# xuanvinh1997/llm-fp8

Measured on AMD Instinct MI355X. Metric: train tokens/sec + FP8 GEMM % of MFMA peak, Llama-3.2-3B seq512 b16, higher is better.
Workload: dtype fp8 (E4M3/E5M2 operands, fp32 accumulate, bf16 activations); 1 GPU; llama-3.2-3b (28 layers) full fine-tuning step, batch 16/GPU x seq 512, fp8_scenario=default (te_llama counterpart, lm_head FP8 under the outer recipe), random-init weights, synthetic tokens; route=fused, global_batch=16, seq_len=512, parallelism=single

## Files before the change

include/mi_fp8.h:

```cpp
#ifndef MI_FP8_H
#define MI_FP8_H

#include <stdint.h>

#ifdef __cplusplus
extern "C" {
#endif

#define MI_FMT_E4M3 0
#define MI_FMT_E5M2 1

#define MI_OK 0
#define MI_ERR_ARG (-1)
#define MI_ERR_SHAPE (-2)
#define MI_ERR_HIP (-3)

#define MI_OUT_BF16 0
#define MI_OUT_F32 1

#define MI_AMAX_ALGO_MAX 0
#define MI_AMAX_ALGO_MOST_RECENT 1

#define MI_ABI_VERSION 5
int mi_abi_version(void);
const char* mi_last_error(void);
int mi_device_supported(void);

int mi_cast_amax(const void* x_bf16, void* y_fp8, void* yT_fp8, const float* scale, float* amax,
                 int64_t rows, int64_t cols, int64_t ld_y, int64_t ld_yT, int fmt, void* stream);
int mi_transpose_u8(const void* y, void* yT, int64_t rows, int64_t cols, int64_t ld_y, int64_t ld_yT, void* stream);
int mi_cast_amax_colsum(const void* x_bf16, void* y_fp8, void* yT_fp8, const float* scale, float* amax,
                        float* colsum_partial, int64_t rows, int64_t cols, int64_t ld_y, int64_t ld_yT, int fmt, void* stream);
int mi_colsum_finish(const float* partial, int64_t P, int64_t C, void* out, int out_dtype, void* stream);
int mi_colsum_finish_multi(const void* const* partials, const int64_t* P, const int64_t* C, void* const* outs,
                           const int* out_dtypes, int n, void* stream);

int mi_scale_update(float* amax_history, float* scale, float* scale_inv, const float* fp8_max,
                    int H, int S, int64_t ld, int margin, int algo, void* stream);

int mi_gemm_fp8(const void* A, const void* B, void* D, const float* sa_inv, const float* sb_inv,
                const void* bias_bf16, int64_t M, int64_t N, int64_t K, int64_t lda, int64_t ldb,
                int64_t ldd, int fmt_a, int fmt_b, int out_dtype, int algo, void* stream);

int mi_gemm_fp8_clock(const void* A, const void* B, void* D, const float* sa_inv, const float* sb_inv, int64_t M, int64_t N,
                      int64_t K, int64_t lda, int64_t ldb, int64_t ldd, int algo, unsigned long long* stamps, void* stream);

typedef struct mi_gemm_problem {
  const void* A;
  const void* B;
  void* D;
  const float* sa_inv;
  const float* sb_inv;
  int64_t M, N, K, lda, ldb, ldd;
} mi_gemm_problem;
int mi_gemm_fp8_grouped(const mi_gemm_problem* problems, int n, int fmt_a, int fmt_b, int tile_cfg, void* stream);

int64_t mi_gemm_workspace_bytes(void);
int mi_gemm_set_workspace(void* workspace, int64_t bytes);

int mi_mxfp8_quantize(const void* x_bf16, void* y_row, void* s_row, void* y_colT, void* s_colT,
                      int64_t rows, int64_t cols, int fmt, void* stream);

int mi_mxfp8_quantize_ex(const void* x_bf16, void* y_row, void* s_row, void* y_colT, void* s_colT, float* colsum,
                         int64_t rows, int64_t cols, int64_t ld_rows, int fmt, void* stream);
int mi_mxfp8_norm_quantize(const void* x_bf16, const float* rstd, const void* gamma_bf16, void* y_row, void* s_row,
                           void* y_colT, void* s_colT, int64_t rows, int64_t cols, int fmt, void* stream);
int mi_mxfp8_swiglu_quantize(const void* h_bf16, void* y_row, void* s_row, void* y_colT, void* s_colT, int64_t rows,
                             int64_t F, int fmt, void* stream);
int mi_mxfp8_dswiglu_quantize(const void* h_bf16, const void* dact_bf16, void* y_row, void* s_row, void* y_colT,
                              void* s_colT, float* colsum, int64_t rows, int64_t F, int fmt, void* stream);
int mi_mxfp8_rope_bwd_quantize(const void* dq_bf16, const void* dk_bf16, const void* dv_bf16, const float* cos_tab,
                               const float* sin_tab, void* y_row, void* s_row, void* y_colT, void* s_colT, int64_t rows,
                               int64_t seq, int n_q_heads, int n_kv_heads, int head_dim, int fmt, void* stream);

int mi_gemm_mxfp8(const void* A, const void* SA, const void* B, const void* SB, void* D,
                  const void* bias_bf16, int64_t M, int64_t N, int64_t K, int fmt_a, int fmt_b,
                  int out_dtype, int algo, void* stream);

typedef struct mi_gemm_mx_problem {
  const void* A;
  const void* SA;
  const void* B;
  const void* SB;
  void* D;
  int64_t M, N, K;
} mi_gemm_mx_problem;
int mi_gemm_mxfp8_grouped(const mi_gemm_mx_problem* problems, int n, int fmt_a, int fmt_b, int tile_cfg, void* stream);

int mi_rope_qkv(void* fused_bf16, void* q_bf16, void* k_bf16, void* v_bf16, const float* cos_tab,
                const float* sin_tab, int64_t rows, int64_t seq, int n_q_heads, int n_kv_heads, int head_dim,
                int backward, void* stream);
int mi_rope_qkv_bwd_cast(const void* dq_bf16, const void* dk_bf16, const void* dv_bf16, const float* cos_tab, const float* sin_tab,
                         void* y_fp8, void* yT_fp8, const float* scale, float* amax, int64_t rows, int64_t seq, int n_q_heads,
                         int n_kv_heads, int head_dim, int fmt, void* stream);

int mi_swiglu_cast(const void* h_bf16, void* y_fp8, void* yT_fp8, const float* scale, float* amax,
                   int64_t rows, int64_t F, int fmt, void* stream);

int mi_dswiglu_cast(const void* h_bf16, const void* dact_bf16, void* y_fp8, void* yT_fp8, const float* scale,
                    float* amax, float* colsum, int64_t rows, int64_t F, int fmt, void* stream);
int mi_swiglu_cast_bias(const void* h_bf16, const void* bias_bf16, void* y_fp8, void* yT_fp8, const float* scale, float* amax,
                        int64_t rows, int64_t F, int fmt, void* stream);
int mi_dswiglu_cast_bias(const void* h_bf16, const void* bias_bf16, const void* dact_bf16, void* y_fp8, void* yT_fp8,
                         const float* scale, float* amax, float* colsum, int64_t rows, int64_t F, int fmt, void* stream);

int mi_rmsnorm_stats(const void* x_bf16, float* rstd, int64_t rows, int64_t cols, float eps, void* stream);
int mi_add_rmsnorm_stats(const void* a_bf16, const void* b_bf16, void* out_bf16, float* rstd, int64_t rows, int64_t cols,
                         float eps, void* stream);
int mi_add_bias_rmsnorm_stats(const void* a_bf16, const void* b_bf16, const void* bias_bf16, void* out_bf16, float* rstd,
                              int64_t rows, int64_t cols, float eps, void* stream);
int mi_norm_cast(const void* x_bf16, const float* rstd, const void* gamma_bf16, void* y_fp8, void* yT_fp8,
                 const float* scale, float* amax, int64_t rows, int64_t cols, int fmt, void* stream);
int mi_rmsnorm_bwd(const void* dy_bf16, const void* x_bf16, const float* rstd, const void* gamma_bf16,
                   const void* dres_bf16, void* dx_bf16, float* dgamma_partial, int n_partials, int64_t rows,
                   int64_t cols, void* stream);

int mi_ce_forward(const void* logits_bf16, const int64_t* labels, float* lse, float* loss_rows, int64_t rows,
                  int64_t cols, void* stream);
int mi_ce_backward(const void* logits_bf16, const int64_t* labels, const float* lse, const float* gscale,
                   void* dlogits_bf16, int64_t rows, int64_t cols, void* stream);
int mi_ce_backward_cast(const void* logits_bf16, const int64_t* labels, const float* lse, const float* gscale, void* y_fp8,
                        void* yT_fp8, const float* scale, float* amax, int64_t rows, int64_t cols, int fmt, void* stream);

int mi_sumsq_bf16(const void* g_bf16, int64_t n, float* partial, int n_partials, void* stream);
int mi_sumsq_bf16_multi(const int64_t* table, int n_tensors, const int32_t* chunks, int n_chunks, int chunk_elems,
                        double* partial, void* stream);
int mi_adamw_bf16_multi(const int64_t* table, int n_tensors, const int32_t* chunks, int n_chunks, int chunk_elems,
                        const float* grad_scale, float lr, float beta1, float beta2, float eps, float weight_decay,
                        int64_t step, void* stream);
int mi_adamw_cast_bf16_multi(const int64_t* table, int n_tensors, const int32_t* chunks, int n_chunks, int chunk_elems,
                             const float* grad_scale, float lr, float beta1, float beta2, float eps, float weight_decay,
                             int64_t step, void* stream);
int mi_adamw_mxcast_bf16_multi(const int64_t* table, int n_tensors, const int32_t* chunks, int n_chunks, int chunk_elems,
                               const float* grad_scale, float lr, float beta1, float beta2, float eps, float weight_decay,
                               int64_t step, void* stream);

int mi_embedding_grad_add(void* grad_bf16, const void* dy_bf16, const int64_t* sorted_ids, const int64_t* perm, int64_t tokens,
                          int64_t hidden, int64_t vocab, float alpha, int64_t padding_idx, void* stream);
int mi_adamw_bf16(void* p_bf16, const void* g_bf16, void* exp_avg_bf16, void* exp_avg_sq_bf16, int64_t n,
                  const float* grad_scale, float lr, float beta1, float beta2, float eps, float weight_decay,
                  int64_t step, void* stream);

int mi_attn_fwd(const void* q, const void* k, const void* v, void* o, float* lse, int B, int S, int H, int G, int D,
                int64_t q_ts, int64_t k_ts, int64_t v_ts, int64_t o_ts, float scale, int causal, void* stream);
#ifdef MI_DIAG
int mi_attn_fwd_diag(const void* q, const void* k, const void* v, void* o, float* lse, unsigned long long* dbg, int B, int S,
                     int H, int G, int D, int64_t q_ts, int64_t k_ts, int64_t v_ts, int64_t o_ts, float scale, void* stream);
#endif
int mi_attn_bwd(const void* q, const void* k, const void* v, const void* o, const void* dout, const float* lse,
                float* delta, void* dq, void* dk, void* dv, int B, int S, int H, int G, int D, int64_t q_ts,
                int64_t k_ts, int64_t v_ts, int64_t o_ts, int64_t do_ts, int64_t dq_ts, int64_t dk_ts, int64_t dv_ts,
                float scale, int causal, void* stream);

#ifdef __cplusplus
}
#endif
#endif
```

llm_fp8_amd/_lib.py:

```python
from __future__ import annotations

import ctypes
import os

_HERE = os.path.dirname(os.path.abspath(__file__))
LIB_PATH = os.environ.get("LLM_FP8_AMD_LIB") or os.path.join(_HERE, "libmi_fp8.so")
LAB_LIB_PATH = os.path.join(os.path.dirname(_HERE), "tools", "bin", "libmi_fp8_lab.so")

MI_FMT_E4M3 = 0
MI_FMT_E5M2 = 1
ABI_VERSION = 5

_c_i64 = ctypes.c_int64
_c_int = ctypes.c_int
_p = ctypes.c_void_p

class GemmProblem(ctypes.Structure):
    _fields_ = [("A", ctypes.c_void_p), ("B", ctypes.c_void_p), ("D", ctypes.c_void_p), ("sa_inv", ctypes.c_void_p),
                ("sb_inv", ctypes.c_void_p), ("M", ctypes.c_int64), ("N", ctypes.c_int64), ("K", ctypes.c_int64),
                ("lda", ctypes.c_int64), ("ldb", ctypes.c_int64), ("ldd", ctypes.c_int64)]


class GemmMxProblem(ctypes.Structure):
    _fields_ = [("A", ctypes.c_void_p), ("SA", ctypes.c_void_p), ("B", ctypes.c_void_p), ("SB", ctypes.c_void_p),
                ("D", ctypes.c_void_p), ("M", ctypes.c_int64), ("N", ctypes.c_int64), ("K", ctypes.c_int64)]

SIGNATURES = {
    "mi_abi_version": [],
    "mi_last_error": [],
    "mi_device_supported": [],
    "mi_cast_amax": [_p, _p, _p, _p, _p, _c_i64, _c_i64, _c_i64, _c_i64, _c_int, _p],
    "mi_transpose_u8": [_p, _p, _c_i64, _c_i64, _c_i64, _c_i64, _p],
    "mi_scale_update": [_p, _p, _p, _p, _c_int, _c_int, _c_i64, _c_int, _c_int, _p],
    "mi_gemm_fp8_grouped": [_p, _c_int, _c_int, _c_int, _c_int, _p],
    "mi_gemm_mxfp8_grouped": [_p, _c_int, _c_int, _c_int, _c_int, _p],
    "mi_gemm_fp8": [_p, _p, _p, _p, _p, _p, _c_i64, _c_i64, _c_i64, _c_i64, _c_i64, _c_i64,
                    _c_int, _c_int, _c_int, _c_int, _p],
    "mi_mxfp8_quantize": [_p, _p, _p, _p, _p, _c_i64, _c_i64, _c_int, _p],
    "mi_mxfp8_quantize_ex": [_p, _p, _p, _p, _p, _p, _c_i64, _c_i64, _c_i64, _c_int, _p],
    "mi_mxfp8_rope_bwd_quantize": [_p, _p, _p, _p, _p, _p, _p, _p, _p, _c_i64, _c_i64, _c_int, _c_int, _c_int, _c_int, _p],
    "mi_rope_qkv": [_p, _p, _p, _p, _p, _p, _c_i64, _c_i64, _c_int, _c_int, _c_int, _c_int, _p],
    "mi_rope_qkv_bwd_cast": [_p, _p, _p, _p, _p, _p, _p, _p, _p, _c_i64, _c_i64, _c_int, _c_int, _c_int, _c_int, _p],
    "mi_swiglu_cast": [_p, _p, _p, _p, _p, _c_i64, _c_i64, _c_int, _p],
    "mi_dswiglu_cast": [_p, _p, _p, _p, _p, _p, _p, _c_i64, _c_i64, _c_int, _p],
    "mi_rmsnorm_stats": [_p, _p, _c_i64, _c_i64, ctypes.c_float, _p],
    "mi_norm_cast": [_p, _p, _p, _p, _p, _p, _p, _c_i64, _c_i64, _c_int, _p],
    "mi_rmsnorm_bwd": [_p, _p, _p, _p, _p, _p, _p, _c_int, _c_i64, _c_i64, _p],
    "mi_ce_forward": [_p, _p, _p, _p, _c_i64, _c_i64, _p],
    "mi_ce_backward": [_p, _p, _p, _p, _p, _c_i64, _c_i64, _p],
    "mi_ce_backward_cast": [_p, _p, _p, _p, _p, _p, _p, _p, _c_i64, _c_i64, _c_int, _p],
    "mi_sumsq_bf16": [_p, _c_i64, _p, _c_int, _p],
    "mi_sumsq_bf16_multi": [_p, _c_int, _p, _c_int, _c_int, _p, _p],
    "mi_adamw_bf16_multi": [_p, _c_int, _p, _c_int, _c_int, _p, ctypes.c_float, ctypes.c_float, ctypes.c_float, ctypes.c_float,
                            ctypes.c_float, _c_i64, _p],
    "mi_adamw_cast_bf16_multi": [_p, _c_int, _p, _c_int, _c_int, _p, ctypes.c_float, ctypes.c_float, ctypes.c_float, ctypes.c_float,
                                 ctypes.c_float, _c_i64, _p],
    "mi_adamw_mxcast_bf16_multi": [_p, _c_int, _p, _c_int, _c_int, _p, ctypes.c_float, ctypes.c_float, ctypes.c_float, ctypes.c_float,
                                   ctypes.c_float, _c_i64, _p],
    "mi_embedding_grad_add": [_p, _p, _p, _p, _c_i64, _c_i64, _c_i64, ctypes.c_float, _c_i64, _p],
    "mi_adamw_bf16": [_p, _p, _p, _p, _c_i64, _p, ctypes.c_float, ctypes.c_float, ctypes.c_float, ctypes.c_float,
                      ctypes.c_float, _c_i64, _p],
    "mi_add_rmsnorm_stats": [_p, _p, _p, _p, _c_i64, _c_i64, ctypes.c_float, _p],
    "mi_cast_amax_colsum": [_p, _p, _p, _p, _p, _p, _c_i64, _c_i64, _c_i64, _c_i64, _c_int, _p],
    "mi_colsum_finish": [_p, _c_i64, _c_i64, _p, _c_int, _p],
    "mi_colsum_finish_multi": [_p, _p, _p, _p, _p, _c_int, _p],
    "mi_gemm_workspace_bytes": [],
    "mi_gemm_set_workspace": [_p, _c_i64],
    "mi_attn_fwd": [_p, _p, _p, _p, _p, _c_int, _c_int, _c_int, _c_int, _c_int, _c_i64, _c_i64, _c_i64, _c_i64, ctypes.c_float,
                    _c_int, _p],
    "mi_attn_bwd": [_p] * 10 + [_c_int] * 5 + [_c_i64] * 8 + [ctypes.c_float, _c_int, _p],
    "mi_mxfp8_norm_quantize": [_p, _p, _p, _p, _p, _p, _p, _c_i64, _c_i64, _c_int, _p],
    "mi_mxfp8_swiglu_quantize": [_p, _p, _p, _p, _p, _c_i64, _c_i64, _c_int, _p],
    "mi_mxfp8_dswiglu_quantize": [_p, _p, _p, _p, _p, _p, _p, _c_i64, _c_i64, _c_int, _p],
    "mi_gemm_mxfp8": [_p, _p, _p, _p, _p, _p, _c_i64, _c_i64, _c_i64, _c_int, _c_int, _c_int, _c_int, _p],
    "mi_swiglu_cast_bias": [_p, _p, _p, _p, _p, _p, _c_i64, _c_i64, _c_int, _p],
    "mi_dswiglu_cast_bias": [_p, _p, _p, _p, _p, _p, _p, _p, _c_i64, _c_i64, _c_int, _p],
    "mi_add_bias_rmsnorm_stats": [_p, _p, _p, _p, _p, _c_i64, _c_i64, ctypes.c_float, _p],
    "mi_gemm_fp8_clock": [_p, _p, _p, _p, _p, _c_i64, _c_i64, _c_i64, _c_i64, _c_i64, _c_i64, _c_int, _p, _p],
}
LAB_SIGNATURES = {
    "mi_attn_fwd_diag": [_p, _p, _p, _p, _p, _p, _c_int, _c_int, _c_int, _c_int, _c_int, _c_i64, _c_i64, _c_i64, _c_i64, ctypes.c_float, _p],
}

_lib = None


def _bind(path: str, signatures) -> ctypes.CDLL:
    lib = ctypes.CDLL(path)
    for name, argtypes in signatures.items():
        fn = getattr(lib, name)
        fn.argtypes = argtypes
        fn.restype = ctypes.c_char_p if name == "mi_last_error" else (_c_i64 if name == "mi_gemm_workspace_bytes" else _c_int)
    v = lib.mi_abi_version()
    if v != ABI_VERSION:
        raise ImportError(f"{os.path.basename(path)} ABI version {v} != expected {ABI_VERSION}; rebuild it")
    return lib


def load() -> ctypes.CDLL:
    global _lib
    if _lib is not None:
        return _lib
    if not os.path.exists(LIB_PATH):
        raise ImportError(
            f"{LIB_PATH} not found: the HIP extension is not built. Run "
            "`python -c 'import __graft_entry__ as g; g.build()'` or `make -C llm_fp8_amd/csrc`. "
            "llm_fp8_amd has no CPU/PyTorch fallback for the FP8 path.")
    _lib = _bind(LIB_PATH, SIGNATURES)
    return _lib


def use_lab_library() -> ctypes.CDLL:
    global _lib
    if _lib is not None and getattr(_lib, "_mi_is_lab", False):
        return _lib
    if _lib is not None:
        raise RuntimeError("use_lab_library(): the product library is already loaded in this process")
    if not os.path.exists(LAB_LIB_PATH):
        raise ImportError(f"{LAB_LIB_PATH} not found: run `make -C llm_fp8_amd/csrc lab`")
    _lib = _bind(LAB_LIB_PATH, {**SIGNATURES, **LAB_SIGNATURES})
    _lib._mi_is_lab = True
    return _lib


def check(rc: int, what: str = "") -> None:
    if rc != 0:
        msg = load().mi_last_error().decode("utf-8", "replace")
        raise RuntimeError(f"libmi_fp8 {what} failed (rc={rc}): {msg}")
```

llm_fp8_amd/csrc/mi_attn.hip:

```cpp
#include "mi_common.h"

namespace mi {

typedef __bf16 bf8 __attribute__((ext_vector_type(8)));
typedef short s4v __attribute__((ext_vector_type(4)));
typedef short s8v __attribute__((ext_vector_type(8)));
typedef float f16v __attribute__((ext_vector_type(16)));
typedef __attribute__((address_space(3))) s4v lds_s4v;

template <int D>
__device__ __forceinline__ int tile_off(int row, int ch) {
  if (D == 128) return 256 * row + 16 * (ch ^ (((row & 3) << 2) | ((row >> 2) & 3)));
  return 128 * row + 16 * (ch ^ (((row & 1) << 2) | ((row >> 1) & 3)));
}

__device__ __forceinline__ bf8 as_bf8(v4i v) { return __builtin_bit_cast(bf8, v); }

template <int D>
__device__ __forceinline__ bf8 row_frag(const char* tile, int r0, int t, int lane) {
  const int r = lane & 31, h = lane >> 5;
  return as_bf8(*reinterpret_cast<const v4i*>(tile + tile_off<D>(r0 + r, 2 * t + h)));
}

template <int D>
__device__ __forceinline__ bf8 tr_frag(const char* tile, int r0, int c0, int lane) {
  const int i16 = lane & 15, qq = i16 >> 2, pp = i16 & 3, half = (lane >> 4) & 1, h = lane >> 5;
  const int ch = (c0 >> 3) + 2 * half + (pp >> 1);
  const int rb = r0 + 4 * h + qq;
  const s4v lo = __builtin_amdgcn_ds_read_tr16_b64_v4i16((lds_s4v*)(tile + tile_off<D>(rb, ch) + 8 * (pp & 1)));
  const s4v hi = __builtin_amdgcn_ds_read_tr16_b64_v4i16((lds_s4v*)(tile + tile_off<D>(rb + 8, ch) + 8 * (pp & 1)));
  s8v v;
  v[0] = lo[0]; v[1] = lo[1]; v[2] = lo[2]; v[3] = lo[3]; v[4] = hi[0]; v[5] = hi[1]; v[6] = hi[2]; v[7] = hi[3];
  return __builtin_bit_cast(bf8, v);
}

__device__ __forceinline__ bf8 acc_frag(const f16v& a, int s) {
  v4i v;
#pragma unroll
  for (int j = 0; j < 4; ++j) v[j] = (int)pack_bf16x2(a[8 * s + 2 * j], a[8 * s + 2 * j + 1]);
  return as_bf8(v);
}

__device__ __forceinline__ int acc_row(int reg, int h) { return (reg & 3) + 8 * (reg >> 2) + 4 * h; }

__device__ __forceinline__ void retire(bf8& f) {
  v4i tmp = __builtin_bit_cast(v4i, f);
  asm volatile("" : "+v"(tmp));
  f = as_bf8(tmp);
}
__device__ __forceinline__ void retire(float& f) { asm volatile("" : "+v"(f)); }

constexpr int ATT_QB = 128;
constexpr int ATT_KB = 64;

typedef __amdgpu_buffer_rsrc_t rsrc_t;
#define MI_LDS_PTR(p) ((__attribute__((address_space(3))) void*)(p))
template <int D>
__device__ __forceinline__ void dma_voffsets(int* voff, int64_t tok_stride, int tid) {
  const int lane = tid & 63, w = tid >> 6;
#pragma unroll
  for (int i = 0; i < D / 32; ++i) {
    const int p = (4 * i + w) * 1024 + 16 * lane;
    const int row = p / (2 * D), slot = (p % (2 * D)) / 16;
    const int ch = D == 128 ? slot ^ (((row & 3) << 2) | ((row >> 2) & 3)) : slot ^ (((row & 1) << 2) | ((row >> 1) & 3));
    voff[i] = (int)((int64_t)row * tok_stride * 2) + 16 * ch;
  }
}
template <int D>
__device__ __forceinline__ void stage_dma(rsrc_t rs, const int* voff, int soff, char* tile, int w) {
#pragma unroll
  for (int i = 0; i < D / 32; ++i)
    __builtin_amdgcn_raw_ptr_buffer_load_lds(rs, MI_LDS_PTR(tile + (4 * i + w) * 1024), 16, voff[i], soff, 0, 0);
}
template <int D>
__device__ __forceinline__ void stage_dma_checked(rsrc_t rs, const int* voff, int adv, char* tile, int w) {
#pragma unroll
  for (int i = 0; i < D / 32; ++i)
    __builtin_amdgcn_raw_ptr_buffer_load_lds(rs, MI_LDS_PTR(tile + (4 * i + w) * 1024), 16, (int)((u32)voff[i] + (u32)adv), 0, 0, 0);
}
template <int D, bool TAIL>
__device__ __forceinline__ void stage_tile(rsrc_t rs, const int* voff, int adv, char* tile, int w) {
  if (TAIL) stage_dma_checked<D>(rs, voff, adv, tile, w);
  else stage_dma<D>(rs, voff, adv, tile, w);
}
__device__ __forceinline__ void dma_wait_all() { asm volatile("s_waitcnt vmcnt(0)" ::: "memory"); }

template <int D, bool CAUSAL, bool DIAG = false, bool TAIL = false>
__global__ __launch_bounds__(256, 2) void attn_fwd_kernel(const uint16_t* __restrict__ q, const uint16_t* __restrict__ k,
                                                          const uint16_t* __restrict__ v, uint16_t* __restrict__ o,
                                                          float* __restrict__ lse, int S, int H, int G, int64_t q_ts,
                                                          int64_t k_ts, int64_t v_ts, int64_t o_ts, float c,
                                                          unsigned long long* __restrict__ dbg = nullptr) {
  constexpr int TILE = ATT_KB * D * 2;
  constexpr int KT = D / 16, DB = D / 32;
  __shared__ __attribute__((aligned(16))) char lds[4 * TILE];
  const int tid = threadIdx.x, lane = tid & 63, w = tid >> 6, r = lane & 31, h = lane >> 5;
  const int qb = gridDim.x - 1 - blockIdx.x, head = blockIdx.y, b = blockIdx.z, g = head / (H / G);
  const int q_first = qb * ATT_QB + w * 32;
  const int qrow = q_first + r;
  int ntiles = CAUSAL ? (qb * ATT_QB + ATT_QB) / ATT_KB : S / ATT_KB;
  if (TAIL) {
    const int stiles = (S + ATT_KB - 1) / ATT_KB;
    ntiles = CAUSAL ? min(ntiles, stiles) : stiles;
  }
  const uint16_t* kbase = k + (int64_t)b * S * k_ts + (int64_t)g * D;
  const uint16_t* vbase = v + (int64_t)b * S * v_ts + (int64_t)g * D;

  bf8 qf[KT];
  {
    const uint16_t* qp = q + ((int64_t)b * S + (TAIL ? min(qrow, S - 1) : qrow)) * q_ts + (int64_t)head * D + 8 * h;
#pragma unroll
    for (int t = 0; t < KT; ++t) qf[t] = as_bf8(*reinterpret_cast<const v4i*>(qp + 16 * t));
  }
#pragma unroll
  for (int t = 0; t < KT; ++t) retire(qf[t]);
  f16v oacc[DB];
#pragma unroll
  for (int d = 0; d < DB; ++d)
#pragma unroll
    for (int i = 0; i < 16; ++i) oacc[d][i] = 0.0f;
  float m = -1.0e30f, l = 0.0f;

  const rsrc_t rsK = __builtin_amdgcn_make_buffer_rsrc((void*)kbase, 0, (int)((((int64_t)S - 1) * k_ts + D) * 2), 0x00020000);
  const rsrc_t rsV = __builtin_amdgcn_make_buffer_rsrc((void*)vbase, 0, (int)((((int64_t)S - 1) * v_ts + D) * 2), 0x00020000);
  int kvo[D / 32], vvo[D / 32];
  dma_voffsets<D>(kvo, k_ts, tid);
  dma_voffsets<D>(vvo, v_ts, tid);
  stage_tile<D, TAIL>(rsK, kvo, 0, lds, w);
  stage_tile<D, TAIL>(rsV, vvo, 0, lds + 2 * TILE, w);
  dma_wait_all();
  __syncthreads();

  unsigned long long tsum[5] = {0, 0, 0, 0, 0}, t_prev = 0;
#define MI_STAMP(k)                                                                       \
  if (DIAG) {                                                                             \
    __builtin_amdgcn_sched_barrier(0);                                                    \
    unsigned long long tn_;                                                               \
    asm volatile("s_memtime %0\n\ts_waitcnt lgkmcnt(0)" : "=s"(tn_)::"memory");          \
    if ((k) >= 0) tsum[(k) < 0 ? 0 : (k)] += tn_ - t_prev;                                  \
    t_prev = tn_;                                                                         \
    __builtin_amdgcn_sched_barrier(0);                                                    \
  }
  MI_STAMP(-1)
  for (int j = 0; j < ntiles; ++j) {
    const char* kt = lds + (j & 1) * TILE;
    const char* vt = lds + (2 + (j & 1)) * TILE;
    const bool more = j + 1 < ntiles;
    if (more) {
      stage_tile<D, TAIL>(rsK, kvo, (int)((int64_t)(j + 1) * ATT_KB * k_ts * 2), lds + ((j + 1) & 1) * TILE, w);
      stage_tile<D, TAIL>(rsV, vvo, (int)((int64_t)(j + 1) * ATT_KB * v_ts * 2), lds + (2 + ((j + 1) & 1)) * TILE, w);
    }
    const int key0 = j * ATT_KB;
    if ((!TAIL || q_first < S) && (!CAUSAL || key0 <= q_first + 31)) {
      f16v sacc[2];
#pragma unroll
      for (int kb = 0; kb < 2; ++kb) {
#pragma unroll
        for (int i = 0; i < 16; ++i) sacc[kb][i] = 0.0f;
        bf8 ka = row_frag<D>(kt, 32 * kb, 0, lane);
#pragma unroll
        for (int t = 0; t < KT; ++t) {
          bf8 kn = ka;
          if (t + 1 < KT) kn = row_frag<D>(kt, 32 * kb, t + 1, lane);
          __builtin_amdgcn_sched_barrier(0);
          sacc[kb] = __builtin_amdgcn_mfma_f32_32x32x16_bf16(ka, qf[t], sacc[kb], 0, 0, 0);
          __builtin_amdgcn_sched_barrier(0);
          ka = kn;
        }
      }
      if (DIAG) {
        asm volatile("" : "+v"(sacc[0][0]), "+v"(sacc[1][15]));
      }
      MI_STAMP(0)
      if (CAUSAL && key0 + ATT_KB - 1 > q_first) {
#pragma unroll
        for (int kb = 0; kb < 2; ++kb)
#pragma unroll
          for (int i = 0; i < 16; ++i)
            if (key0 + 32 * kb + acc_row(i, h) > qrow) sacc[kb][i] = -INFINITY;
      }
      if (TAIL && !CAUSAL && key0 + ATT_KB > S) {
#pragma unroll
        for (int kb = 0; kb < 2; ++kb)
#pragma unroll
          for (int i = 0; i < 16; ++i)
            if (key0 + 32 * kb + acc_row(i, h) >= S) sacc[kb][i] = -INFINITY;
      }
      float mx = sacc[0][0];
#pragma unroll
      for (int kb = 0; kb < 2; ++kb)
#pragma unroll
        for (int i = 0; i < 16; ++i) mx = fmaxf(mx, sacc[kb][i]);
      mx = fmaxf(mx, __shfl_xor(mx, 32));
      const float m_new = fmaxf(m, mx);
      const float alpha = __builtin_amdgcn_exp2f((m - m_new) * c);
      const float mc = m_new * c;
      m = m_new;
      float psum = 0.0f;
#pragma unroll
      for (int kb = 0; kb < 2; ++kb)
#pragma unroll
        for (int i = 0; i < 16; ++i) {
          const float p = __builtin_amdgcn_exp2f(__builtin_fmaf(sacc[kb][i], c, -mc));
          sacc[kb][i] = p;
          psum += p;
        }
      l = l * alpha + psum;
#pragma unroll
      for (int d = 0; d < DB; ++d) oacc[d] = oacc[d] * alpha;
      if (DIAG) {
        asm volatile("" : "+v"(oacc[0][0]), "+v"(sacc[1][15]), "+v"(l));
      }
      MI_STAMP(1)
#pragma unroll
      for (int kb = 0; kb < 2; ++kb)
#pragma unroll
        for (int s = 0; s < 2; ++s) {
          const bf8 pf = acc_frag(sacc[kb], s);
          bf8 fa = tr_frag<D>(vt, 32 * kb + 16 * s, 0, lane);
#pragma unroll
          for (int d = 0; d < DB; ++d) {
            bf8 fn = fa;
            if (d + 1 < DB) fn = tr_frag<D>(vt, 32 * kb + 16 * s, 32 * (d + 1), lane);
            __builtin_amdgcn_sched_barrier(0);
            oacc[d] = __builtin_amdgcn_mfma_f32_32x32x16_bf16(fa, pf, oacc[d], 0, 0, 0);
            __builtin_amdgcn_sched_barrier(0);
            fa = fn;
          }
        }
    }
    if (DIAG) {
      asm volatile("" : "+v"(oacc[0][0]), "+v"(oacc[DB - 1][15]));
    }
    MI_STAMP(2)
    dma_wait_all();
    MI_STAMP(3)
    __syncthreads();
    MI_STAMP(4)
  }
  if (DIAG && dbg != nullptr && lane == 0) {
    unsigned long long* dp = dbg + ((((int64_t)b * H + head) * gridDim.x + qb) * 4 + w) * 8;
    for (int i2 = 0; i2 < 5; ++i2) dp[i2] = tsum[i2];
    dp[5] = (unsigned long long)ntiles;
  }
#undef MI_STAMP

  l += __shfl_xor(l, 32);
  const float inv = 1.0f / l;
  if (h == 0 && (!TAIL || qrow < S)) lse[((int64_t)b * H + head) * S + qrow] = m * c + __builtin_amdgcn_logf(l);
  char* ot = lds + w * (32 * D * 2);
#pragma unroll
  for (int d = 0; d < DB; ++d)
#pragma unroll
    for (int i = 0; i < 4; ++i) {
      const int ch = 4 * d + i;
      uint2 pk;
      pk.x = pack_bf16x2(oacc[d][4 * i] * inv, oacc[d][4 * i + 1] * inv);
      pk.y = pack_bf16x2(oacc[d][4 * i + 2] * inv, oacc[d][4 * i + 3] * inv);
      *reinterpret_cast<uint2*>(ot + r * (D * 2) + 16 * (ch ^ (r & (D / 8 - 1))) + 8 * h) = pk;
    }
  __builtin_amdgcn_s_waitcnt(0xc07f);
  __builtin_amdgcn_wave_barrier();
  constexpr int CPR = D / 8;
#pragma unroll
  for (int it = 0; it < 32 * CPR / 64; ++it) {
    const int idx = it * 64 + lane, row = idx / CPR, ch = idx % CPR;
    const v4i val = *reinterpret_cast<const v4i*>(ot + row * (D * 2) + 16 * (ch ^ (row & (CPR - 1))));
    if (!TAIL || q_first + row < S) *reinterpret_cast<v4i*>(o + ((int64_t)b * S + q_first + row) * o_ts + (int64_t)head * D + ch * 8) = val;
  }
}


template <int D, bool TAIL = false>
__device__ __forceinline__ void store_rows_from_accT(const f16v (&acc)[D / 32], float mul, char* slice, uint16_t* out,
                                                     int64_t row_stride, int lane, int nrows = 32) {
  const int r = lane & 31, h = lane >> 5;
  constexpr int CPR = D / 8;
#pragma unroll
  for (int d = 0; d < D / 32; ++d)
#pragma unroll
    for (int i = 0; i < 4; ++i) {
      const int ch = 4 * d + i;
      uint2 pk;
      pk.x = pack_bf16x2(acc[d][4 * i] * mul, acc[d][4 * i + 1] * mul);
      pk.y = pack_bf16x2(acc[d][4 * i + 2] * mul, acc[d][4 * i + 3] * mul);
      *reinterpret_cast<uint2*>(slice + r * (D * 2) + 16 * (ch ^ (r & (CPR - 1))) + 8 * h) = pk;
    }
  __builtin_amdgcn_s_waitcnt(0xc07f);
  __builtin_amdgcn_wave_barrier();
#pragma unroll
  for (int it = 0; it < 32 * CPR / 64; ++it) {
    const int idx = it * 64 + lane, row = idx / CPR, ch = idx % CPR;
    const v4i val = *reinterpret_cast<const v4i*>(slice + row * (D * 2) + 16 * (ch ^ (row & (CPR - 1))));
    if (!TAIL || row < nrows) *reinterpret_cast<v4i*>(out + (int64_t)row * row_stride + ch * 8) = val;
  }
}

template <int D, bool CAUSAL, bool TAIL = false>
__global__ __launch_bounds__(256, 2) void attn_bwd_dq_kernel(const uint16_t* __restrict__ q, const uint16_t* __restrict__ k,
                                                             const uint16_t* __restrict__ v, const uint16_t* __restrict__ o,
                                                             const uint16_t* __restrict__ dout, const float* __restrict__ lse,
                                                             float* __restrict__ delta, uint16_t* __restrict__ dq, int S,
                                                             int H, int G, int64_t q_ts, int64_t k_ts, int64_t v_ts,
                                                             int64_t o_ts, int64_t do_ts, int64_t dq_ts, float c, float scale) {
  constexpr int TILE = ATT_KB * D * 2;
  constexpr int KT = D / 16, DB = D / 32;
  __shared__ __attribute__((aligned(16))) char lds[4 * TILE];
  const int tid = threadIdx.x, lane = tid & 63, w = tid >> 6, r = lane & 31, h = lane >> 5;
  const int qb = gridDim.x - 1 - blockIdx.x, head = blockIdx.y, b = blockIdx.z, g = head / (H / G);
  const int q_first = qb * ATT_QB + w * 32;
  const int qrow = q_first + r;
  int ntiles = CAUSAL ? (qb * ATT_QB + ATT_QB) / ATT_KB : S / ATT_KB;
  if (TAIL) {
    const int stiles = (S + ATT_KB - 1) / ATT_KB;
    ntiles = CAUSAL ? min(ntiles, stiles) : stiles;
  }
  const uint16_t* kbase = k + (int64_t)b * S * k_ts + (int64_t)g * D;
  const uint16_t* vbase = v + (int64_t)b * S * v_ts + (int64_t)g * D;

  bf8 qf[KT], dof[KT];
  float dl = 0.0f;
  {
    const int lrow = TAIL ? min(qrow, S - 1) : qrow;
    const uint16_t* qp = q + ((int64_t)b * S + lrow) * q_ts + (int64_t)head * D + 8 * h;
    const uint16_t* dp = dout + ((int64_t)b * S + lrow) * do_ts + (int64_t)head * D + 8 * h;
    const uint16_t* op = o + ((int64_t)b * S + lrow) * o_ts + (int64_t)head * D + 8 * h;
#pragma unroll
    for (int t = 0; t < KT; ++t) {
      qf[t] = as_bf8(*reinterpret_cast<const v4i*>(qp + 16 * t));
      const v4i dv4 = *reinterpret_cast<const v4i*>(dp + 16 * t);
      const v4i ov4 = *reinterpret_cast<const v4i*>(op + 16 * t);
      dof[t] = as_bf8(dv4);
#pragma unroll
      for (int j = 0; j < 4; ++j) {
        const u32 a = (u32)dv4[j], bb = (u32)ov4[j];
        dl += __uint_as_float(a << 16) * __uint_as_float(bb << 16) + __uint_as_float(a & 0xFFFF0000u) * __uint_as_float(bb & 0xFFFF0000u);
      }
    }
  }
  dl += __shfl_xor(dl, 32);
  const int64_t stat = ((int64_t)b * H + head) * S + qrow;
  if (h == 0 && (!TAIL || qrow < S)) delta[stat] = dl;
  float my_lse = lse[TAIL ? ((int64_t)b * H + head) * S + min(qrow, S - 1) : stat];
#pragma unroll
  for (int t = 0; t < KT; ++t) {
    retire(qf[t]);
    retire(dof[t]);
  }
  retire(my_lse);
  retire(dl);

  f16v acc[DB];
#pragma unroll
  for (int d = 0; d < DB; ++d)
#pragma unroll
    for (int i = 0; i < 16; ++i) acc[d][i] = 0.0f;

  const rsrc_t rsK = __builtin_amdgcn_make_buffer_rsrc((void*)kbase, 0, (int)((((int64_t)S - 1) * k_ts + D) * 2), 0x00020000);
  const rsrc_t rsV = __builtin_amdgcn_make_buffer_rsrc((void*)vbase, 0, (int)((((int64_t)S - 1) * v_ts + D) * 2), 0x00020000);
  int kvo[D / 32], vvo[D / 32];
  dma_voffsets<D>(kvo, k_ts, tid);
  dma_voffsets<D>(vvo, v_ts, tid);
  stage_tile<D, TAIL>(rsK, kvo, 0, lds, w);
  stage_tile<D, TAIL>(rsV, vvo, 0, lds + 2 * TILE, w);
  dma_wait_all();
  __syncthreads();

  for (int j = 0; j < ntiles; ++j) {
    const char* kt = lds + (j & 1) * TILE;
    const char* vt = lds + (2 + (j & 1)) * TILE;
    const bool more = j + 1 < ntiles;
    if (more) {
      stage_tile<D, TAIL>(rsK, kvo, (int)((int64_t)(j + 1) * ATT_KB * k_ts * 2), lds + ((j + 1) & 1) * TILE, w);
      stage_tile<D, TAIL>(rsV, vvo, (int)((int64_t)(j + 1) * ATT_KB * v_ts * 2), lds + (2 + ((j + 1) & 1)) * TILE, w);
    }
    const int key0 = j * ATT_KB;
    auto block = [&](const int kb) {
      f16v sacc, pacc;
#pragma unroll
      for (int i = 0; i < 16; ++i) { sacc[i] = 0.0f; pacc[i] = 0.0f; }
      constexpr int PF = 1;
      bf8 kr[KT], vr[KT];
#pragma unroll
      for (int t = 0; t < PF; ++t) {
        kr[t] = row_frag<D>(kt, 32 * kb, t, lane);
        vr[t] = row_frag<D>(vt, 32 * kb, t, lane);
      }
#pragma unroll
      for (int t = 0; t < KT; ++t) {
        if (t + PF < KT) {
          kr[t + PF] = row_frag<D>(kt, 32 * kb, t + PF, lane);
          vr[t + PF] = row_frag<D>(vt, 32 * kb, t + PF, lane);
        }
        __builtin_amdgcn_sched_barrier(0);
        sacc = __builtin_amdgcn_mfma_f32_32x32x16_bf16(kr[t], qf[t], sacc, 0, 0, 0);
        pacc = __builtin_amdgcn_mfma_f32_32x32x16_bf16(vr[t], dof[t], pacc, 0, 0, 0);
        __builtin_amdgcn_sched_barrier(0);
      }
      const bool diag = CAUSAL && key0 + 32 * kb + 31 > q_first;
#pragma unroll
      for (int i = 0; i < 16; ++i) {
        float p = __builtin_amdgcn_exp2f(__builtin_fmaf(sacc[i], c, -my_lse));
        if (diag && key0 + 32 * kb + acc_row(i, h) > qrow) p = 0.0f;
        if (TAIL && !CAUSAL && key0 + 32 * kb + acc_row(i, h) >= S) p = 0.0f;
        sacc[i] = p * (pacc[i] - dl);
      }
#pragma unroll
      for (int s = 0; s < 2; ++s) {
        const bf8 dsf = acc_frag(sacc, s);
        bf8 fa = tr_frag<D>(kt, 32 * kb + 16 * s, 0, lane);
#pragma unroll
        for (int d = 0; d < DB; ++d) {
          bf8 fn = fa;
          if (d + 1 < DB) fn = tr_frag<D>(kt, 32 * kb + 16 * s, 32 * (d + 1), lane);
          __builtin_amdgcn_sched_barrier(0);
          acc[d] = __builtin_amdgcn_mfma_f32_32x32x16_bf16(fa, dsf, acc[d], 0, 0, 0);
          __builtin_amdgcn_sched_barrier(0);
          fa = fn;
        }
      }
    };
    if ((!TAIL || q_first < S) && (!CAUSAL || key0 <= q_first + 31)) block(0);
    if ((!TAIL || (q_first < S && key0 + 32 < S)) && (!CAUSAL || key0 + 32 <= q_first + 31)) block(1);
    dma_wait_all();
    __syncthreads();
  }
  store_rows_from_accT<D, TAIL>(acc, scale, lds + w * (32 * D * 2), dq + ((int64_t)b * S + q_first) * dq_ts + (int64_t)head * D, dq_ts, lane,
                                S - q_first);
}

template <int D, bool CAUSAL, bool TAIL = false>
__global__ __launch_bounds__(256, D == 128 ? 1 : 2) void attn_bwd_dkdv_kernel(const uint16_t* __restrict__ q, const uint16_t* __restrict__ k,
                                                               const uint16_t* __restrict__ v, const uint16_t* __restrict__ dout,
                                                               const float* __restrict__ lse, const float* __restrict__ delta,
                                                               uint16_t* __restrict__ dk, uint16_t* __restrict__ dv, int S, int H,
                                                               int G, int B, int64_t q_ts, int64_t k_ts, int64_t v_ts,
                                                               int64_t do_ts, int64_t dk_ts, int64_t dv_ts, float c, float scale) {
  constexpr int SL = 32 * D * 2;
  constexpr int KT = D / 16, DB = D / 32;
  constexpr int BUF = 2 * SL + 256;
  __shared__ __attribute__((aligned(16))) char lds[(2 * BUF > 4 * SL) ? 2 * BUF : 4 * SL];
  const int tid = threadIdx.x, lane = tid & 63, w = tid >> 6, r = lane & 31, h = lane >> 5;
  const int lin = blockIdx.x, nkb = TAIL ? (S + 127) / 128 : S / 128;
  const int kbi = CAUSAL ? lin / (G * B) : nkb - 1 - lin / (G * B);
  const int g = (lin / B) % G, b = lin % B;
  const int rep = H / G;
  const int key_first = kbi * 128 + w * 32;
  const int key = key_first + r;

  bf8 kf[KT], vf[KT];
  {
    const int lkey = TAIL ? min(key, S - 1) : key;
    const uint16_t* kp = k + ((int64_t)b * S + lkey) * k_ts + (int64_t)g * D + 8 * h;
    const uint16_t* vp = v + ((int64_t)b * S + lkey) * v_ts + (int64_t)g * D + 8 * h;
#pragma unroll
    for (int t = 0; t < KT; ++t) {
      kf[t] = as_bf8(*reinterpret_cast<const v4i*>(kp + 16 * t));
      vf[t] = as_bf8(*reinterpret_cast<const v4i*>(vp + 16 * t));
    }
  }
#pragma unroll
  for (int t = 0; t < KT; ++t) {
    retire(kf[t]);
    retire(vf[t]);
  }
  f16v dka[DB], dva[DB];
#pragma unroll
  for (int d = 0; d < DB; ++d)
#pragma unroll
    for (int i = 0; i < 16; ++i) { dka[d][i] = 0.0f; dva[d][i] = 0.0f; }

  const int sl0 = CAUSAL ? (kbi * 128) / 32 : 0;
  const int nsl = (TAIL ? (S + 31) / 32 : S / 32) - sl0;
  const int nsteps = rep * nsl;
  v4i qreg[2], dreg[2];
  float sreg = 0.0f;
  auto load_step = [&](int step) {
    const int head = g * rep + step / nsl, q0 = (sl0 + step % nsl) * 32;
    const uint16_t* qp = q + ((int64_t)b * S + q0) * q_ts + (int64_t)head * D;
    const uint16_t* dp = dout + ((int64_t)b * S + q0) * do_ts + (int64_t)head * D;
#pragma unroll
    for (int i = 0; i < 2; ++i) {
      const int cidx = tid + 256 * i, row = cidx / (D / 8), ch = cidx % (D / 8);
      if (D == 128 || cidx < 32 * (D / 8)) {
        if (TAIL && q0 + row >= S) {
          qreg[i] = v4i{0, 0, 0, 0};
          dreg[i] = v4i{0, 0, 0, 0};
        } else {
          qreg[i] = *reinterpret_cast<const v4i*>(qp + (int64_t)row * q_ts + ch * 8);
          dreg[i] = *reinterpret_cast<const v4i*>(dp + (int64_t)row * do_ts + ch * 8);
        }
      }
    }
    if (tid < 64) {
      if (TAIL && q0 + (tid & 31) >= S) sreg = 0.0f;
      else sreg = (tid < 32 ? lse : delta)[((int64_t)b * H + head) * S + q0 + (tid & 31)];
    }
  };
  auto store_step = [&](char* buf) {
#pragma unroll
    for (int i = 0; i < 2; ++i) {
      const int cidx = tid + 256 * i, row = cidx / (D / 8), ch = cidx % (D / 8);
      if (D == 128 || cidx < 32 * (D / 8)) {
        *reinterpret_cast<v4i*>(buf + tile_off<D>(row, ch)) = qreg[i];
        *reinterpret_cast<v4i*>(buf + SL + tile_off<D>(row, ch)) = dreg[i];
      }
    }
    if (tid < 64) reinterpret_cast<float*>(buf + 2 * SL)[tid] = sreg;
  };
  load_step(0);
  store_step(lds);
  __syncthreads();

  for (int step = 0; step < nsteps; ++step) {
    const char* buf = lds + (step & 1) * BUF;
    const bool more = step + 1 < nsteps;
    if (more) load_step(step + 1);
    const int q0 = (sl0 + step % nsl) * 32;
    if ((!TAIL || key_first < S) && (!CAUSAL || q0 + 31 >= key_first)) {
      const char* qt = buf;
      const char* dt = buf + SL;
      const float* st = reinterpret_cast<const float*>(buf + 2 * SL);
      f16v sacc, pacc;
#pragma unroll
      for (int i = 0; i < 16; ++i) { sacc[i] = 0.0f; pacc[i] = 0.0f; }
#pragma unroll
      for (int t = 0; t < KT; ++t) {
        sacc = __builtin_amdgcn_mfma_f32_32x32x16_bf16(row_frag<D>(qt, 0, t, lane), kf[t], sacc, 0, 0, 0);
        pacc = __builtin_amdgcn_mfma_f32_32x32x16_bf16(row_frag<D>(dt, 0, t, lane), vf[t], pacc, 0, 0, 0);
      }
      const bool diag = CAUSAL && q0 < key_first + 31;
      f16v dsacc;
#pragma unroll
      for (int a = 0; a < 4; ++a) {
        const v4f ls = *reinterpret_cast<const v4f*>(st + 8 * a + 4 * h);
        const v4f dl = *reinterpret_cast<const v4f*>(st + 32 + 8 * a + 4 * h);
#pragma unroll
        for (int e = 0; e < 4; ++e) {
          const int i = 4 * a + e;
          float p = __builtin_amdgcn_exp2f(__builtin_fmaf(sacc[i], c, -ls[e]));
          if (diag && key > q0 + acc_row(i, h)) p = 0.0f;
          if (TAIL && q0 + acc_row(i, h) >= S) p = 0.0f;
          sacc[i] = p;
          dsacc[i] = p * (pacc[i] - dl[e]);
        }
      }
#pragma unroll
      for (int s = 0; s < 2; ++s) {
        const bf8 pf = acc_frag(sacc, s), dsf = acc_frag(dsacc, s);
#pragma unroll
        for (int d = 0; d < DB; ++d) {
          dva[d] = __builtin_amdgcn_mfma_f32_32x32x16_bf16(tr_frag<D>(dt, 16 * s, 32 * d, lane), pf, dva[d], 0, 0, 0);
          dka[d] = __builtin_amdgcn_mfma_f32_32x32x16_bf16(tr_frag<D>(qt, 16 * s, 32 * d, lane), dsf, dka[d], 0, 0, 0);
        }
      }
    }
    if (D == 128) {
#pragma unroll
      for (int d = 0; d < DB; ++d) asm volatile("" : "+a"(dka[d]), "+a"(dva[d]));
    }
    if (more) store_step(lds + ((step + 1) & 1) * BUF);
    __syncthreads();
  }
  char* slice = lds + w * SL;
  store_rows_from_accT<D, TAIL>(dka, scale, slice, dk + ((int64_t)b * S + key_first) * dk_ts + (int64_t)g * D, dk_ts, lane, S - key_first);
  __builtin_amdgcn_wave_barrier();
  store_rows_from_accT<D, TAIL>(dva, 1.0f, slice, dv + ((int64_t)b * S + key_first) * dv_ts + (int64_t)g * D, dv_ts, lane, S - key_first);
}

}

extern "C" int mi_attn_fwd(const void* q, const void* k, const void* v, void* o, float* lse, int B, int S, int H, int G,
                           int D, int64_t q_ts, int64_t k_ts, int64_t v_ts, int64_t o_ts, float scale, int causal,
                           void* stream) {
  MI_CHECK_ARG(q && k && v && o && lse, "mi_attn_fwd: null pointer");
  MI_CHECK_ARG(B >= 1 && H >= 1 && G >= 1 && H % G == 0, "mi_attn_fwd: bad B/H/G (%d, %d, %d)", B, H, G);
  MI_CHECK_ARG(D == 128 || D == 64, "mi_attn_fwd: head_dim %d not supported (64, 128)", D);
  MI_CHECK_ARG(S >= 128 && S % 16 == 0, "mi_attn_fwd: seq %d must be a multiple of 16 and at least 128", S);
  MI_CHECK_ARG(q_ts % 8 == 0 && k_ts % 8 == 0 && v_ts % 8 == 0 && o_ts % 8 == 0, "mi_attn_fwd: token strides must be multiples of 8");
  MI_CHECK_ARG((int64_t)S * k_ts * 2 < (1LL << 31) && (int64_t)S * v_ts * 2 < (1LL << 31) && ((uintptr_t)k % 16) == 0 && ((uintptr_t)v % 16) == 0,
               "mi_attn_fwd: one batch of K / V must span < 2 GiB and be 16-byte aligned (32-bit buffer offsets of the LDS DMA)");
  MI_CHECK_ARG(((uintptr_t)q % 16) == 0 && ((uintptr_t)o % 16) == 0, "mi_attn_fwd: q and o must be 16-byte aligned (16-byte row accesses)");
  MI_CHECK_ARG(H <= 65535 && B <= 65535, "mi_attn_fwd: grid too large");
  const float c = scale * 1.4426950408889634f;
  const bool tail = S % mi::ATT_QB != 0;
  dim3 grid((S + mi::ATT_QB - 1) / mi::ATT_QB, H, B), block(256);
  hipStream_t st = (hipStream_t)stream;
#define MI_ATTN_FWD_T(DD, CC, TT)                                                                                      \
  hipLaunchKernelGGL((mi::attn_fwd_kernel<DD, CC, false, TT>), grid, block, 0, st, (const uint16_t*)q, (const uint16_t*)k, \
                     (const uint16_t*)v, (uint16_t*)o, lse, S, H, G, q_ts, k_ts, v_ts, o_ts, c, (unsigned long long*)nullptr)
#define MI_ATTN_FWD(DD, CC)                                                                                            \
  do {                                                                                                                 \
    if (tail) MI_ATTN_FWD_T(DD, CC, true); else MI_ATTN_FWD_T(DD, CC, false);                                          \
  } while (0)
  if (D == 128) {
    if (causal) MI_ATTN_FWD(128, true); else MI_ATTN_FWD(128, false);
  } else {
    if (causal) MI_ATTN_FWD(64, true); else MI_ATTN_FWD(64, false);
  }
#undef MI_ATTN_FWD_T
#undef MI_ATTN_FWD
  MI_CHECK_LAUNCH("mi_attn_fwd launch");
  return MI_OK;
}

#ifdef MI_DIAG
extern "C" int mi_attn_fwd_diag(const void* q, const void* k, const void* v, void* o, float* lse, unsigned long long* dbg, int B,
                                int S, int H, int G, int D, int64_t q_ts, int64_t k_ts, int64_t v_ts, int64_t o_ts, float scale,
                                void* stream) {
  MI_CHECK_ARG(q && k && v && o && lse && dbg, "mi_attn_fwd_diag: null pointer");
  MI_CHECK_ARG(D == 128 && S % 128 == 0 && H % G == 0, "mi_attn_fwd_diag: unsupported shape");
  dim3 grid(S / mi::ATT_QB, H, B), block(256);
  hipLaunchKernelGGL((mi::attn_fwd_kernel<128, true, true>), grid, block, 0, (hipStream_t)stream, (const uint16_t*)q,
                     (const uint16_t*)k, (const uint16_t*)v, (uint16_t*)o, lse, S, H, G, q_ts, k_ts, v_ts, o_ts,
                     scale * 1.4426950408889634f, dbg);
  MI_CHECK_LAUNCH("mi_attn_fwd_diag launch");
  return MI_OK;
}
#endif

extern "C" int mi_attn_bwd(const void* q, const void* k, const void* v, const void* o, const void* dout, const float* lse,
                           float* delta, void* dq, void* dk, void* dv, int B, int S, int H, int G, int D, int64_t q_ts,
                           int64_t k_ts, int64_t v_ts, int64_t o_ts, int64_t do_ts, int64_t dq_ts, int64_t dk_ts,
                           int64_t dv_ts, float scale, int causal, void* stream) {
  MI_CHECK_ARG(q && k && v && o && dout && lse && delta && dq && dk && dv, "mi_attn_bwd: null pointer");
  MI_CHECK_ARG(B >= 1 && H >= 1 && G >= 1 && H % G == 0, "mi_attn_bwd: bad B/H/G (%d, %d, %d)", B, H, G);
  MI_CHECK_ARG(D == 128 || D == 64, "mi_attn_bwd: head_dim %d not supported (64, 128)", D);
  MI_CHECK_ARG(S >= 128 && S % 16 == 0, "mi_attn_bwd: seq %d must be a multiple of 16 and at least 128", S);
  MI_CHECK_ARG((q_ts | k_ts | v_ts | o_ts | do_ts | dq_ts | dk_ts | dv_ts) % 8 == 0, "mi_attn_bwd: token strides must be multiples of 8");
  MI_CHECK_ARG((int64_t)S * k_ts * 2 < (1LL << 31) && (int64_t)S * v_ts * 2 < (1LL << 31) && ((uintptr_t)k % 16) == 0 && ((uintptr_t)v % 16) == 0,
               "mi_attn_bwd: one batch of K / V must span < 2 GiB and be 16-byte aligned (32-bit buffer offsets of the LDS DMA)");
  MI_CHECK_ARG((((uintptr_t)q | (uintptr_t)o | (uintptr_t)dout | (uintptr_t)dq | (uintptr_t)dk | (uintptr_t)dv) % 16) == 0,
               "mi_attn_bwd: q, o, dout, dq, dk and dv must be 16-byte aligned (16-byte row accesses)");
  MI_CHECK_ARG(H <= 65535 && B <= 65535, "mi_attn_bwd: grid too large");
  const float c = scale * 1.4426950408889634f;
  hipStream_t st = (hipStream_t)stream;
  const bool tail = S % mi::ATT_QB != 0;
  const int nblk = (S + mi::ATT_QB - 1) / mi::ATT_QB;
  dim3 grid_q(nblk, H, B), grid_kv((unsigned)((int64_t)nblk * G * B)), block(256);
#define MI_ATTN_BWD_T(DD, CC, TT)                                                                                      \
  do {                                                                                                                 \
    hipLaunchKernelGGL((mi::attn_bwd_dq_kernel<DD, CC, TT>), grid_q, block, 0, st, (const uint16_t*)q, (const uint16_t*)k, \
                       (const uint16_t*)v, (const uint16_t*)o, (const uint16_t*)dout, lse, delta, (uint16_t*)dq, S, H,  \
                       G, q_ts, k_ts, v_ts, o_ts, do_ts, dq_ts, c, scale);                                               \
    hipLaunchKernelGGL((mi::attn_bwd_dkdv_kernel<DD, CC, TT>), grid_kv, block, 0, st, (const uint16_t*)q,                \
                       (const uint16_t*)k, (const uint16_t*)v, (const uint16_t*)dout, lse, delta, (uint16_t*)dk,        \
                       (uint16_t*)dv, S, H, G, B, q_ts, k_ts, v_ts, do_ts, dk_ts, dv_ts, c, scale);                      \
  } while (0)
#define MI_ATTN_BWD(DD, CC)                                                                                            \
  do {                                                                                                                 \
    if (tail) MI_ATTN_BWD_T(DD, CC, true); else MI_ATTN_BWD_T(DD, CC, false);                                          \
  } while (0)
  if (D == 128) {
    if (causal) MI_ATTN_BWD(128, true); else MI_ATTN_BWD(128, false);
  } else {
    if (causal) MI_ATTN_BWD(64, true); else MI_ATTN_BWD(64, false);
  }
#undef MI_ATTN_BWD
#undef MI_ATTN_BWD_T
  MI_CHECK_LAUNCH("mi_attn_bwd launch");
  return MI_OK;
}
```

llm_fp8_amd/csrc/mi_fused.hip:

```cpp
#include "mi_common.h"

namespace mi {

template <int DIR>
__global__ __launch_bounds__(256) void rope_qkv_kernel(uint16_t* __restrict__ fused, uint16_t* __restrict__ q,
                                                       uint16_t* __restrict__ k, uint16_t* __restrict__ v,
                                                       const float* __restrict__ cosT, const float* __restrict__ sinT,
                                                       int rows, int seq, int nq, int nk, int D) {
  const int half = D >> 1;
  const int vph = half >> 3;
  const int W = (nq + 2 * nk) * D;
  const int rot_items = (nq + nk) * vph;
  const int cpy_items = (nk * D) >> 3;
  const int per_row = rot_items + cpy_items;
  const int64_t items = (int64_t)rows * per_row;
  const float sgn = DIR == 0 ? 1.0f : -1.0f;
  for (int64_t it = (int64_t)blockIdx.x * blockDim.x + threadIdx.x; it < items; it += (int64_t)gridDim.x * blockDim.x) {
    const int64_t r = it / per_row;
    const int w = (int)(it - r * per_row);
    uint16_t* frow = fused + r * W;
    if (w < rot_items) {
      const int hd = w / vph, vv = w - hd * vph;
      uint16_t* sep = hd < nq ? q + (r * nq + hd) * D : k + (r * nk + (hd - nq)) * D;
      uint16_t* f1 = frow + hd * D + vv * 8;
      uint16_t* s1 = sep + vv * 8;
      const uint16_t* in1 = DIR == 0 ? f1 : s1;
      uint16_t* out1 = DIR == 0 ? s1 : f1;
      const v4i a = *reinterpret_cast<const v4i*>(in1), b = *reinterpret_cast<const v4i*>(in1 + half);
      const int pos = (int)(r % seq);
      const float* cp = cosT + (int64_t)pos * half + vv * 8;
      const float* sp = sinT + (int64_t)pos * half + vv * 8;
      float c[8], sn[8];
      *reinterpret_cast<v4f*>(c) = *reinterpret_cast<const v4f*>(cp);
      *reinterpret_cast<v4f*>(c + 4) = *reinterpret_cast<const v4f*>(cp + 4);
      *reinterpret_cast<v4f*>(sn) = *reinterpret_cast<const v4f*>(sp);
      *reinterpret_cast<v4f*>(sn + 4) = *reinterpret_cast<const v4f*>(sp + 4);
      v4i o1, o2;
#pragma unroll
      for (int j = 0; j < 4; ++j) {
        const u32 wa = (u32)a[j], wb = (u32)b[j];
        const float x1l = __uint_as_float(wa << 16), x1h = __uint_as_float(wa & 0xFFFF0000u);
        const float x2l = __uint_as_float(wb << 16), x2h = __uint_as_float(wb & 0xFFFF0000u);
        const float cl = c[2 * j], ch = c[2 * j + 1], sl = sgn * sn[2 * j], sh = sgn * sn[2 * j + 1];
        o1[j] = (int)pack_bf16x2(x1l * cl - x2l * sl, x1h * ch - x2h * sh);
        o2[j] = (int)pack_bf16x2(x2l * cl + x1l * sl, x2h * ch + x1h * sh);
      }
      *reinterpret_cast<v4i*>(out1) = o1;
      *reinterpret_cast<v4i*>(out1 + half) = o2;
    } else {
      const int cv = w - rot_items;
      uint16_t* fp = frow + (nq + nk) * D + cv * 8;
      uint16_t* sp2 = v + r * (int64_t)(nk * D) + cv * 8;
      if (DIR == 0) *reinterpret_cast<v4i*>(sp2) = *reinterpret_cast<const v4i*>(fp);
      else *reinterpret_cast<v4i*>(fp) = *reinterpret_cast<const v4i*>(sp2);
    }
  }
}

template <int FMT, bool WRITE_Y, bool WRITE_T>
__global__ __launch_bounds__(256) void rope_bwd_cast_kernel(const uint16_t* __restrict__ dq, const uint16_t* __restrict__ dk,
                                                            const uint16_t* __restrict__ dv, const float* __restrict__ cosT,
                                                            const float* __restrict__ sinT, uint8_t* __restrict__ y,
                                                            uint8_t* __restrict__ yT, const float* __restrict__ scale_p,
                                                            float* amax_out, int rows, int seq, int nq, int nk) {
  constexpr int D = 128, half = 64;
  __shared__ float s_amax[4];
  const int tid = threadIdx.x, lane = tid & 63, wave = tid >> 6;
  const int W = (nq + 2 * nk) * D;
  const int units = (nq + nk) + 2 * nk;
  const int64_t u_all = (int64_t)blockIdx.x * 4 + wave;
  const int rb = (int)(u_all / units), u = (int)(u_all % units);
  const int r0 = rb * 64 + (lane >> 3) * 8, lc = (lane & 7) * 8;
  const float scale = *scale_p;
  float amax = 0.0f;
  auto emit = [&](const float (&f)[8][8], int c0) {
    u32 lo[8], hi[8];
#pragma unroll
    for (int i = 0; i < 8; ++i) {
#pragma unroll
      for (int j = 0; j < 8; ++j) amax = fmaxf(amax, (f[i][j] != f[i][j]) ? 0.0f : fabsf(f[i][j]));
      lo[i] = cvt4_fp8<FMT>(f[i][0] * scale, f[i][1] * scale, f[i][2] * scale, f[i][3] * scale);
      hi[i] = cvt4_fp8<FMT>(f[i][4] * scale, f[i][5] * scale, f[i][6] * scale, f[i][7] * scale);
    }
    if (WRITE_Y) {
      uint8_t* dst = y + (int64_t)r0 * W + c0;
#pragma unroll
      for (int i = 0; i < 8; ++i) mi::st8<MI_NT_Y>(dst + (int64_t)i * W, lo[i], hi[i]);
    }
    if (WRITE_T) {
      u32 a[4], b[4], c[4], d[4];
      transpose4x4(lo[0], lo[1], lo[2], lo[3], a[0], a[1], a[2], a[3]);
      transpose4x4(lo[4], lo[5], lo[6], lo[7], b[0], b[1], b[2], b[3]);
      transpose4x4(hi[0], hi[1], hi[2], hi[3], c[0], c[1], c[2], c[3]);
      transpose4x4(hi[4], hi[5], hi[6], hi[7], d[0], d[1], d[2], d[3]);
      uint8_t* dst = yT + (int64_t)c0 * rows + r0;
#pragma unroll
      for (int j = 0; j < 4; ++j) {
        mi::st8<MI_NT_YT>(dst + (int64_t)j * rows, a[j], b[j]);
        mi::st8<MI_NT_YT>(dst + (int64_t)(j + 4) * rows, c[j], d[j]);
      }
    }
  };
  auto bf16_round = [](float v) { return __uint_as_float(float_to_bf16_bits(v) << 16); };
  if (r0 < rows) {
    if (u < nq + nk) {
      const int hd = u;
      const uint16_t* src = hd < nq ? dq + ((int64_t)r0 * nq + hd) * D : dk + ((int64_t)r0 * nk + (hd - nq)) * D;
      const int64_t rstride = (int64_t)(hd < nq ? nq : nk) * D;
      float f1[8][8], f2[8][8];
#pragma unroll
      for (int i = 0; i < 8; ++i) {
        const v4i a = *reinterpret_cast<const v4i*>(src + i * rstride + lc);
        const v4i b = *reinterpret_cast<const v4i*>(src + i * rstride + half + lc);
        const int pos = (r0 + i) % seq;
        float c[8], sn[8];
        *reinterpret_cast<v4f*>(c) = *reinterpret_cast<const v4f*>(cosT + (int64_t)pos * half + lc);
        *reinterpret_cast<v4f*>(c + 4) = *reinterpret_cast<const v4f*>(cosT + (int64_t)pos * half + lc + 4);
        *reinterpret_cast<v4f*>(sn) = *reinterpret_cast<const v4f*>(sinT + (int64_t)pos * half + lc);
        *reinterpret_cast<v4f*>(sn + 4) = *reinterpret_cast<const v4f*>(sinT + (int64_t)pos * half + lc + 4);
#pragma unroll
        for (int j = 0; j < 4; ++j) {
          const u32 wa = (u32)a[j], wb = (u32)b[j];
          const float x1l = __uint_as_float(wa << 16), x1h = __uint_as_float(wa & 0xFFFF0000u);
          const float x2l = __uint_as_float(wb << 16), x2h = __uint_as_float(wb & 0xFFFF0000u);
          const float cl = c[2 * j], ch = c[2 * j + 1], sl = -1.0f * sn[2 * j], sh = -1.0f * sn[2 * j + 1];
          f1[i][2 * j] = bf16_round(x1l * cl - x2l * sl);
          f1[i][2 * j + 1] = bf16_round(x1h * ch - x2h * sh);
          f2[i][2 * j] = bf16_round(x2l * cl + x1l * sl);
          f2[i][2 * j + 1] = bf16_round(x2h * ch + x1h * sh);
        }
      }
      emit(f1, hd * D + lc);
      emit(f2, hd * D + half + lc);
    } else {
      const int tc = u - (nq + nk);
      float f[8][8];
#pragma unroll
      for (int i = 0; i < 8; ++i) {
        const v4i a = *reinterpret_cast<const v4i*>(dv + (int64_t)(r0 + i) * (nk * D) + tc * 64 + lc);
#pragma unroll
        for (int j = 0; j < 4; ++j) {
          f[i][2 * j] = __uint_as_float((u32)a[j] << 16);
          f[i][2 * j + 1] = __uint_as_float((u32)a[j] & 0xFFFF0000u);
        }
      }
      emit(f, (nq + nk) * D + tc * 64 + lc);
    }
  }
  if (amax_out != nullptr) {
    amax = wave_max(amax);
    if (lane == 0) s_amax[wave] = amax;
    __syncthreads();
    if (tid == 0) {
      const float m = fmaxf(fmaxf(s_amax[0], s_amax[1]), fmaxf(s_amax[2], s_amax[3]));
      if (m > 0.0f && m > __builtin_nontemporal_load(amax_out)) atomicMax(reinterpret_cast<unsigned int*>(amax_out), __float_as_uint(m));
    }
  }
}

__device__ __forceinline__ float sigmoidf_(float g) { return 1.0f / (1.0f + __expf(-g)); }

template <int FMT, int MODE, bool WRITE_Y, bool WRITE_T>
__global__ __launch_bounds__(256) void swiglu_cast_kernel(const uint16_t* __restrict__ h, const uint16_t* __restrict__ d,
                                                          uint8_t* __restrict__ y, uint8_t* __restrict__ yT,
                                                          const float* __restrict__ scale_p, float* amax_out,
                                                          float* __restrict__ colsum, int rows, int F, int tiles_c,
                                                          const uint16_t* __restrict__ bias) {
  __shared__ float s_amax[4];
  __shared__ float s_col[MODE == 1 ? 2 : 1][2][128];
  constexpr int NOUT = MODE == 0 ? 1 : 2;
  const int ocols = MODE == 0 ? F : 2 * F;
  const int tid = threadIdx.x, lane = tid & 63, wave = tid >> 6;
  const int tile_r = blockIdx.x / tiles_c, tile_c = blockIdx.x % tiles_c;
  const int r0 = tile_r * 128 + (wave >> 1) * 64 + (lane >> 3) * 8;
  const int cg = tile_c * 128 + (wave & 1) * 64 + (lane & 7) * 8;
  const float scale = *scale_p;
  float amax = 0.0f;
  float csum[NOUT][8];
#pragma unroll
  for (int o = 0; o < NOUT; ++o)
#pragma unroll
    for (int j = 0; j < 8; ++j) csum[o][j] = 0.0f;
  const bool active = (r0 < rows) && (cg < F);
  if (active) {
    u32 lo[NOUT][8], hi[NOUT][8];
    float bg[8] = {0.f, 0.f, 0.f, 0.f, 0.f, 0.f, 0.f, 0.f}, bu[8] = {0.f, 0.f, 0.f, 0.f, 0.f, 0.f, 0.f, 0.f};
    if (bias != nullptr) {
      const v4i vg = *reinterpret_cast<const v4i*>(bias + cg), vu = *reinterpret_cast<const v4i*>(bias + F + cg);
#pragma unroll
      for (int j = 0; j < 4; ++j) {
        bg[2 * j] = __uint_as_float((u32)vg[j] << 16);
        bg[2 * j + 1] = __uint_as_float((u32)vg[j] & 0xFFFF0000u);
        bu[2 * j] = __uint_as_float((u32)vu[j] << 16);
        bu[2 * j + 1] = __uint_as_float((u32)vu[j] & 0xFFFF0000u);
      }
    }
#pragma unroll
    for (int pass = 0; pass < 2; ++pass) {
      v4i gv[4], uv[4], dv[4];
#pragma unroll
      for (int i = 0; i < 4; ++i) {
        const int64_t r = r0 + 4 * pass + i;
        gv[i] = __builtin_nontemporal_load(reinterpret_cast<const v4i*>(h + r * 2 * F + cg));
        uv[i] = __builtin_nontemporal_load(reinterpret_cast<const v4i*>(h + r * 2 * F + F + cg));
        dv[i] = MODE == 1 ? __builtin_nontemporal_load(reinterpret_cast<const v4i*>(d + r * F + cg)) : (v4i){0, 0, 0, 0};
      }
#pragma unroll
      for (int i = 0; i < 4; ++i) {
        float f[NOUT][8];
#pragma unroll
        for (int j = 0; j < 4; ++j) {
          const u32 wg = (u32)gv[i][j], wu = (u32)uv[i][j], wd = (u32)dv[i][j];
          float g2[2] = {__uint_as_float(wg << 16), __uint_as_float(wg & 0xFFFF0000u)};
          float u2[2] = {__uint_as_float(wu << 16), __uint_as_float(wu & 0xFFFF0000u)};
          const float d2[2] = {__uint_as_float(wd << 16), __uint_as_float(wd & 0xFFFF0000u)};
          if (bias != nullptr) {
            g2[0] += bg[2 * j];
            g2[1] += bg[2 * j + 1];
            u2[0] += bu[2 * j];
            u2[1] += bu[2 * j + 1];
          }
#pragma unroll
          for (int e = 0; e < 2; ++e) {
            const float sg = sigmoidf_(g2[e]);
            if (MODE == 0) {
              f[0][2 * j + e] = g2[e] * sg * u2[e];
            } else {
              f[0][2 * j + e] = d2[e] * u2[e] * (sg * (1.0f + g2[e] * (1.0f - sg)));
              f[NOUT - 1][2 * j + e] = d2[e] * (g2[e] * sg);
            }
          }
        }
#pragma unroll
        for (int o = 0; o < NOUT; ++o) {
#pragma unroll
          for (int j = 0; j < 8; ++j) {
            amax = fmaxf(amax, (f[o][j] != f[o][j]) ? 0.0f : fabsf(f[o][j]));
            if (MODE == 1) csum[o][j] += f[o][j];
          }
          lo[o][4 * pass + i] = cvt4_fp8<FMT>(f[o][0] * scale, f[o][1] * scale, f[o][2] * scale, f[o][3] * scale);
          hi[o][4 * pass + i] = cvt4_fp8<FMT>(f[o][4] * scale, f[o][5] * scale, f[o][6] * scale, f[o][7] * scale);
        }
      }
      if (MODE == 1) __builtin_amdgcn_sched_barrier(0);
    }
#pragma unroll
    for (int o = 0; o < NOUT; ++o) {
      const int c0 = cg + o * F;
      if (WRITE_Y) {
        uint8_t* dst = y + (int64_t)r0 * ocols + c0;
#pragma unroll
        for (int i = 0; i < 8; ++i) mi::st8<MI_NT_Y>(dst + (int64_t)i * ocols, lo[o][i], hi[o][i]);
      }
      if (WRITE_T) {
        u32 a[4], b[4], c[4], dd[4];
        transpose4x4(lo[o][0], lo[o][1], lo[o][2], lo[o][3], a[0], a[1], a[2], a[3]);
        transpose4x4(lo[o][4], lo[o][5], lo[o][6], lo[o][7], b[0], b[1], b[2], b[3]);
        transpose4x4(hi[o][0], hi[o][1], hi[o][2], hi[o][3], c[0], c[1], c[2], c[3]);
        transpose4x4(hi[o][4], hi[o][5], hi[o][6], hi[o][7], dd[0], dd[1], dd[2], dd[3]);
        uint8_t* dst = yT + (int64_t)c0 * rows + r0;
#pragma unroll
        for (int j = 0; j < 4; ++j) {
          mi::st8<MI_NT_YT>(dst + (int64_t)j * rows, a[j], b[j]);
          mi::st8<MI_NT_YT>(dst + (int64_t)(j + 4) * rows, c[j], dd[j]);
        }
      }
    }
  }
  if (MODE == 1 && colsum != nullptr) {
#pragma unroll
    for (int o = 0; o < NOUT; ++o)
#pragma unroll
      for (int j = 0; j < 8; ++j) {
        float v = csum[o][j];
        v += __shfl_xor(v, 8);
        v += __shfl_xor(v, 16);
        v += __shfl_xor(v, 32);
        if ((lane >> 3) == 0) s_col[o][wave >> 1][(wave & 1) * 64 + (lane & 7) * 8 + j] = v;
      }
    __syncthreads();
    const int c = tile_c * 128 + (tid & 127), o = tid >> 7;
    if (c < F) colsum[(int64_t)tile_r * ocols + o * F + c] = s_col[MODE == 1 ? o : 0][0][tid & 127] + s_col[MODE == 1 ? o : 0][1][tid & 127];
  }
  if (amax_out != nullptr) {
    amax = wave_max(amax);
    if (lane == 0) s_amax[wave] = amax;
    __syncthreads();
    if (tid == 0) {
      float m = fmaxf(fmaxf(s_amax[0], s_amax[1]), fmaxf(s_amax[2], s_amax[3]));
      if (m > 0.0f && m > __builtin_nontemporal_load(amax_out)) atomicMax(reinterpret_cast<unsigned int*>(amax_out), __float_as_uint(m));
    }
  }
}

template <int FMT, int MODE>
static int launch_swiglu(const void* h, const void* d, void* y, void* yT, const float* scale, float* amax, float* colsum,
                         int64_t rows, int64_t F, hipStream_t st, const void* bias = nullptr) {
  const int64_t ocols = MODE == 0 ? F : 2 * F;
  (void)ocols;
  const int tiles_r = (int)((rows + 127) / 128), tiles_c = (int)((F + 127) / 128);
  dim3 grid((unsigned)(tiles_r * tiles_c)), block(256);
  const uint16_t *hp = (const uint16_t*)h, *dp = (const uint16_t*)d, *bp = (const uint16_t*)bias;
  uint8_t *yp = (uint8_t*)y, *tp = (uint8_t*)yT;
  if (y && yT)
    hipLaunchKernelGGL((swiglu_cast_kernel<FMT, MODE, true, true>), grid, block, 0, st, hp, dp, yp, tp, scale, amax, colsum, (int)rows, (int)F, tiles_c, bp);
  else if (y)
    hipLaunchKernelGGL((swiglu_cast_kernel<FMT, MODE, true, false>), grid, block, 0, st, hp, dp, yp, tp, scale, amax, colsum, (int)rows, (int)F, tiles_c, bp);
  else
    hipLaunchKernelGGL((swiglu_cast_kernel<FMT, MODE, false, true>), grid, block, 0, st, hp, dp, yp, tp, scale, amax, colsum, (int)rows, (int)F, tiles_c, bp);
  MI_CHECK_LAUNCH("mi_swiglu_cast launch");
  return MI_OK;
}

__global__ __launch_bounds__(256) void rmsnorm_stats_kernel(const uint16_t* __restrict__ x, float* __restrict__ rstd, int rows,
                                                            int cols, float eps) {
  const int lane = threadIdx.x & 63;
  const int row = blockIdx.x * 4 + (threadIdx.x >> 6);
  if (row >= rows) return;
  const uint16_t* xr = x + (int64_t)row * cols;
  float acc = 0.0f;
  for (int c = lane * 8; c < cols; c += 512) {
    const v4i v = *reinterpret_cast<const v4i*>(xr + c);
#pragma unroll
    for (int j = 0; j < 4; ++j) {
      const u32 w = (u32)v[j];
      const float a = __uint_as_float(w << 16), b = __uint_as_float(w & 0xFFFF0000u);
      acc += a * a + b * b;
    }
  }
#pragma unroll
  for (int o = 32; o >= 1; o >>= 1) acc += __shfl_xor(acc, o);
  if (lane == 0) rstd[row] = rsqrtf(acc / (float)cols + eps);
}

template <int FMT, bool WRITE_Y, bool WRITE_T>
__global__ __launch_bounds__(256) void norm_cast_kernel(const uint16_t* __restrict__ x, const float* __restrict__ rstd,
                                                        const uint16_t* __restrict__ gamma, uint8_t* __restrict__ y,
                                                        uint8_t* __restrict__ yT, const float* __restrict__ scale_p,
                                                        float* amax_out, int rows, int cols, int tiles_c) {
  __shared__ float s_amax[4];
  const int tid = threadIdx.x, lane = tid & 63, wave = tid >> 6;
  const int ntiles = ((rows + 63) / 64) * tiles_c;
  const int stride = gridDim.x * 4;
  const int lr = (lane >> 3) * 8, lc = (lane & 7) * 8;
  const float scale = *scale_p;
  float amax = 0.0f;
  int t = blockIdx.x * 4 + wave;
  v4i nxt[8], nxt_g;
  v4f nxt_r[2];
  auto load_tile = [&](int tt, v4i (&raw)[8], v4i& gv, v4f (&rs)[2]) {
    const int r0 = (tt / tiles_c) * 64 + lr, c0 = (tt % tiles_c) * 64 + lc;
    if (r0 < rows && c0 < cols) {
      const uint16_t* src = x + (int64_t)r0 * cols + c0;
#pragma unroll
      for (int i = 0; i < 8; ++i) raw[i] = __builtin_nontemporal_load(reinterpret_cast<const v4i*>(src + (int64_t)i * cols));
      gv = *reinterpret_cast<const v4i*>(gamma + c0);
      rs[0] = *reinterpret_cast<const v4f*>(rstd + r0);
      rs[1] = *reinterpret_cast<const v4f*>(rstd + r0 + 4);
    } else {
#pragma unroll
      for (int i = 0; i < 8; ++i) raw[i] = (v4i){0, 0, 0, 0};
      gv = (v4i){0, 0, 0, 0};
      rs[0] = rs[1] = (v4f){0.f, 0.f, 0.f, 0.f};
    }
  };
  if (t < ntiles) load_tile(t, nxt, nxt_g, nxt_r);
  while (t < ntiles) {
    v4i raw[8];
#pragma unroll
    for (int i = 0; i < 8; ++i) raw[i] = nxt[i];
    const v4i gv = nxt_g;
    const v4f rs0 = nxt_r[0], rs1 = nxt_r[1];
    const int tn = t + stride;
    if (tn < ntiles) load_tile(tn, nxt, nxt_g, nxt_r);
    const int r0 = (t / tiles_c) * 64 + lr, c0 = (t % tiles_c) * 64 + lc;
    if ((r0 < rows) && (c0 < cols)) {
      float g[8];
#pragma unroll
      for (int j = 0; j < 4; ++j) {
        g[2 * j] = __uint_as_float((u32)gv[j] << 16);
        g[2 * j + 1] = __uint_as_float((u32)gv[j] & 0xFFFF0000u);
      }
      u32 lo[8], hi[8];
#pragma unroll
      for (int i = 0; i < 8; ++i) {
        const float rs = i < 4 ? rs0[i] : rs1[i - 4];
        float f[8];
#pragma unroll
        for (int j = 0; j < 4; ++j) {
          const u32 w = (u32)raw[i][j];
          f[2 * j] = (__uint_as_float(w << 16) * rs) * g[2 * j];
          f[2 * j + 1] = (__uint_as_float(w & 0xFFFF0000u) * rs) * g[2 * j + 1];
        }
#pragma unroll
        for (int j = 0; j < 8; ++j) amax = fmaxf(amax, (f[j] != f[j]) ? 0.0f : fabsf(f[j]));
        lo[i] = cvt4_fp8<FMT>(f[0] * scale, f[1] * scale, f[2] * scale, f[3] * scale);
        hi[i] = cvt4_fp8<FMT>(f[4] * scale, f[5] * scale, f[6] * scale, f[7] * scale);
      }
      if (WRITE_Y) {
        uint8_t* dst = y + (int64_t)r0 * cols + c0;
#pragma unroll
        for (int i = 0; i < 8; ++i) mi::st8<MI_NT_Y>(dst + (int64_t)i * cols, lo[i], hi[i]);
      }
      if (WRITE_T) {
        u32 a[4], b[4], c[4], d[4];
        transpose4x4(lo[0], lo[1], lo[2], lo[3], a[0], a[1], a[2], a[3]);
        transpose4x4(lo[4], lo[5], lo[6], lo[7], b[0], b[1], b[2], b[3]);
        transpose4x4(hi[0], hi[1], hi[2], hi[3], c[0], c[1], c[2], c[3]);
        transpose4x4(hi[4], hi[5], hi[6], hi[7], d[0], d[1], d[2], d[3]);
        uint8_t* dst = yT + (int64_t)c0 * rows + r0;
#pragma unroll
        for (int j = 0; j < 4; ++j) {
          mi::st8<MI_NT_YT>(dst + (int64_t)j * rows, a[j], b[j]);
          mi::st8<MI_NT_YT>(dst + (int64_t)(j + 4) * rows, c[j], d[j]);
        }
      }
    }
    t = tn;
  }
  if (amax_out != nullptr) {
    amax = wave_max(amax);
    if (lane == 0) s_amax[wave] = amax;
    __syncthreads();
    if (tid == 0) {
      float m = fmaxf(fmaxf(s_amax[0], s_amax[1]), fmaxf(s_amax[2], s_amax[3]));
      if (m > 0.0f && m > __builtin_nontemporal_load(amax_out)) atomicMax(reinterpret_cast<unsigned int*>(amax_out), __float_as_uint(m));
    }
  }
}

constexpr int kNormMaxVec = 16;
template <int NVEC, int WPR>
__global__ __launch_bounds__(256) void rmsnorm_bwd_kernel(const uint16_t* __restrict__ dy, const uint16_t* __restrict__ x,
                                                          const float* __restrict__ rstd, const uint16_t* __restrict__ gamma,
                                                          const uint16_t* __restrict__ dres, uint16_t* __restrict__ dx,
                                                          float* __restrict__ dgp, int rows, int rows_per_block) {
  static_assert(NVEC % WPR == 0 && (WPR == 1 || WPR == 2 || WPR == 4), "row split");
  extern __shared__ float s_dg[];
  __shared__ float s_dot[2][4];
  constexpr int cols = NVEC * 512;
  constexpr int NV = NVEC / WPR, R = 4 / WPR;
  const int lane = threadIdx.x & 63, wave = threadIdx.x >> 6;
  const int slot = wave / WPR, part = wave % WPR;
  const int col0 = part * NV * 512 + lane * 8;
  v4i gq[NV];
  float dgacc[NV][8];
#pragma unroll
  for (int v = 0; v < NV; ++v) {
    gq[v] = *reinterpret_cast<const v4i*>(gamma + col0 + v * 512);
#pragma unroll
    for (int j = 0; j < 8; ++j) dgacc[v][j] = 0.0f;
  }
  const int row_begin = blockIdx.x * rows_per_block;
  const int row_end = min(rows, row_begin + rows_per_block);
  const int iters = (row_end - row_begin + R - 1) / R;
  for (int it = 0; it < iters; ++it) {
    const int row = row_begin + it * R + slot;
    const bool valid = row < row_end;
    const float rs = valid ? rstd[row] : 0.0f;
    v4i dq[NV], xq[NV];
    float dot = 0.0f;
#pragma unroll
    for (int v = 0; v < NV; ++v) {
      dq[v] = (v4i){0, 0, 0, 0};
      xq[v] = (v4i){0, 0, 0, 0};
      if (valid) {
        const int64_t off = (int64_t)row * cols + col0 + v * 512;
        dq[v] = *reinterpret_cast<const v4i*>(dy + off);
        xq[v] = *reinterpret_cast<const v4i*>(x + off);
      }
    }
#pragma unroll
    for (int v = 0; v < NV; ++v)
#pragma unroll
      for (int j = 0; j < 4; ++j) {
        const float d0 = __uint_as_float((u32)dq[v][j] << 16), d1 = __uint_as_float((u32)dq[v][j] & 0xFFFF0000u);
        const float x0 = __uint_as_float((u32)xq[v][j] << 16) * rs, x1 = __uint_as_float((u32)xq[v][j] & 0xFFFF0000u) * rs;
        const float g0 = __uint_as_float((u32)gq[v][j] << 16), g1 = __uint_as_float((u32)gq[v][j] & 0xFFFF0000u);
        dgacc[v][2 * j] += d0 * x0;
        dgacc[v][2 * j + 1] += d1 * x1;
        dot += (d0 * g0) * x0 + (d1 * g1) * x1;
      }
#pragma unroll
    for (int o = 32; o >= 1; o >>= 1) dot += __shfl_xor(dot, o);
    if (WPR > 1) {
      if (lane == 0) s_dot[it & 1][wave] = dot;
      __syncthreads();
      dot = s_dot[it & 1][slot * WPR];
#pragma unroll
      for (int q = 1; q < WPR; ++q) dot += s_dot[it & 1][slot * WPR + q];
    }
    const float c = dot / (float)cols;
    if (valid) {
#pragma unroll
      for (int v = 0; v < NV; ++v) {
        const int64_t off = (int64_t)row * cols + col0 + v * 512;
        v4i rv = {0, 0, 0, 0};
        if (dres) rv = *reinterpret_cast<const v4i*>(dres + off);
        v4i ov;
#pragma unroll
        for (int j = 0; j < 4; ++j) {
          const float d0 = __uint_as_float((u32)dq[v][j] << 16), d1 = __uint_as_float((u32)dq[v][j] & 0xFFFF0000u);
          const float x0 = __uint_as_float((u32)xq[v][j] << 16) * rs, x1 = __uint_as_float((u32)xq[v][j] & 0xFFFF0000u) * rs;
          const float g0 = __uint_as_float((u32)gq[v][j] << 16), g1 = __uint_as_float((u32)gq[v][j] & 0xFFFF0000u);
          float o0 = rs * (d0 * g0 - x0 * c), o1 = rs * (d1 * g1 - x1 * c);
          if (dres) {
            o0 += __uint_as_float((u32)rv[j] << 16);
            o1 += __uint_as_float((u32)rv[j] & 0xFFFF0000u);
          }
          ov[j] = (int)pack_bf16x2(o0, o1);
        }
        *reinterpret_cast<v4i*>(dx + off) = ov;
      }
    }
  }
#pragma unroll
  for (int v = 0; v < NV; ++v)
#pragma unroll
    for (int j = 0; j < 8; ++j) s_dg[slot * cols + col0 + v * 512 + j] = dgacc[v][j];
  __syncthreads();
  for (int c = threadIdx.x; c < cols; c += 256) {
    float a = s_dg[c];
#pragma unroll
    for (int q = 1; q < R; ++q) a += s_dg[q * cols + c];
    dgp[(int64_t)blockIdx.x * cols + c] = a;
  }
}

__global__ __launch_bounds__(256) void ce_fwd_kernel(const uint16_t* __restrict__ x, const int64_t* __restrict__ labels,
                                                     float* __restrict__ lse, float* __restrict__ loss, int cols) {
  __shared__ float s_m[4], s_s[4];
  const int row = blockIdx.x, tid = threadIdx.x;
  const uint16_t* xr = x + (int64_t)row * cols;
  float m = -INFINITY, ssum = 0.0f;
  for (int c = tid * 8; c < cols; c += 2048) {
    const v4i v = *reinterpret_cast<const v4i*>(xr + c);
    float f[8];
#pragma unroll
    for (int j = 0; j < 4; ++j) {
      f[2 * j] = __uint_as_float((u32)v[j] << 16);
      f[2 * j + 1] = __uint_as_float((u32)v[j] & 0xFFFF0000u);
    }
    float vm = f[0];
#pragma unroll
    for (int j = 1; j < 8; ++j) vm = fmaxf(vm, f[j]);
    const float nm = fmaxf(m, vm);
    float add = 0.0f;
#pragma unroll
    for (int j = 0; j < 8; ++j) add += __expf(f[j] - nm);
    ssum = (nm == -INFINITY) ? 0.0f : ssum * __expf(m - nm) + add;
    m = nm;
  }
#pragma unroll
  for (int o = 32; o >= 1; o >>= 1) {
    const float om = __shfl_xor(m, o), os = __shfl_xor(ssum, o);
    const float nm = fmaxf(m, om);
    ssum = (nm == -INFINITY) ? 0.0f : ssum * __expf(m - nm) + os * __expf(om - nm);
    m = nm;
  }
  if ((tid & 63) == 0) { s_m[tid >> 6] = m; s_s[tid >> 6] = ssum; }
  __syncthreads();
  if (tid == 0) {
    float M = s_m[0], S = s_s[0];
#pragma unroll
    for (int w = 1; w < 4; ++w) {
      const float nm = fmaxf(M, s_m[w]);
      S = (nm == -INFINITY) ? 0.0f : S * __expf(M - nm) + s_s[w] * __expf(s_m[w] - nm);
      M = nm;
    }
    const float l = M + __logf(S);
    lse[row] = l;
    const int64_t lab = labels[row];
    loss[row] = (lab >= 0 && lab < cols) ? l - bf16_bits_to_float(xr[lab]) : 0.0f;
  }
}

__global__ __launch_bounds__(256) void ce_bwd_kernel(const uint16_t* __restrict__ x, const int64_t* __restrict__ labels,
                                                     const float* __restrict__ lse, const float* __restrict__ gscale,
                                                     uint16_t* __restrict__ dx, int cols) {
  const int row = blockIdx.x, tid = threadIdx.x;
  const int64_t lab = labels[row];
  const bool valid = lab >= 0 && lab < cols;
  const float gs = valid ? *gscale : 0.0f;
  const float l = lse[row];
  const uint16_t* xr = x + (int64_t)row * cols;
  uint16_t* dr = dx + (int64_t)row * cols;
  for (int c = tid * 8; c < cols; c += 2048) {
    const v4i v = *reinterpret_cast<const v4i*>(xr + c);
    v4i o;
#pragma unroll
    for (int j = 0; j < 4; ++j) {
      float p0 = __expf(__uint_as_float((u32)v[j] << 16) - l), p1 = __expf(__uint_as_float((u32)v[j] & 0xFFFF0000u) - l);
      if (c + 2 * j == lab) p0 -= 1.0f;
      if (c + 2 * j + 1 == lab) p1 -= 1.0f;
      o[j] = (int)pack_bf16x2(p0 * gs, p1 * gs);
    }
    *reinterpret_cast<v4i*>(dr + c) = o;
  }
}

template <int FMT, bool WRITE_Y, bool WRITE_T>
__global__ __launch_bounds__(256) void ce_bwd_cast_kernel(const uint16_t* __restrict__ x, const int64_t* __restrict__ labels,
                                                          const float* __restrict__ lse, const float* __restrict__ gscale,
                                                          uint8_t* __restrict__ y, uint8_t* __restrict__ yT,
                                                          const float* __restrict__ scale_p, float* amax_out, int rows, int cols,
                                                          int tiles_c) {
  __shared__ float s_amax[4];
  const int tid = threadIdx.x, lane = tid & 63, wave = tid >> 6;
  const int tile_r = blockIdx.x / tiles_c, tile_c = blockIdx.x % tiles_c;
  const int r0 = tile_r * 128 + (wave >> 1) * 64 + (lane >> 3) * 8;
  const int c0 = tile_c * 128 + (wave & 1) * 64 + (lane & 7) * 8;
  const float scale = *scale_p, g0 = *gscale;
  float amax = 0.0f;
  if ((r0 < rows) && (c0 < cols)) {
    u32 lo[8], hi[8];
#pragma unroll
    for (int i = 0; i < 8; ++i) {
      const int64_t lab = labels[r0 + i];
      const bool valid = lab >= 0 && lab < cols;
      const float gs = valid ? g0 : 0.0f;
      const float l = lse[r0 + i];
      const v4i raw = __builtin_nontemporal_load(reinterpret_cast<const v4i*>(x + (int64_t)(r0 + i) * cols + c0));
      float f[8];
#pragma unroll
      for (int j = 0; j < 4; ++j) {
        float p0 = __expf(__uint_as_float((u32)raw[j] << 16) - l), p1 = __expf(__uint_as_float((u32)raw[j] & 0xFFFF0000u) - l);
        if (c0 + 2 * j == lab) p0 -= 1.0f;
        if (c0 + 2 * j + 1 == lab) p1 -= 1.0f;
        f[2 * j] = __uint_as_float(float_to_bf16_bits(p0 * gs) << 16);
        f[2 * j + 1] = __uint_as_float(float_to_bf16_bits(p1 * gs) << 16);
      }
#pragma unroll
      for (int j = 0; j < 8; ++j) amax = fmaxf(amax, (f[j] != f[j]) ? 0.0f : fabsf(f[j]));
      lo[i] = cvt4_fp8<FMT>(f[0] * scale, f[1] * scale, f[2] * scale, f[3] * scale);
      hi[i] = cvt4_fp8<FMT>(f[4] * scale, f[5] * scale, f[6] * scale, f[7] * scale);
    }
    if (WRITE_Y) {
      uint8_t* dst = y + (int64_t)r0 * cols + c0;
#pragma unroll
      for (int i = 0; i < 8; ++i) mi::st8<MI_NT_Y>(dst + (int64_t)i * cols, lo[i], hi[i]);
    }
    if (WRITE_T) {
      u32 a[4], b[4], c[4], d[4];
      transpose4x4(lo[0], lo[1], lo[2], lo[3], a[0], a[1], a[2], a[3]);
      transpose4x4(lo[4], lo[5], lo[6], lo[7], b[0], b[1], b[2], b[3]);
      transpose4x4(hi[0], hi[1], hi[2], hi[3], c[0], c[1], c[2], c[3]);
      transpose4x4(hi[4], hi[5], hi[6], hi[7], d[0], d[1], d[2], d[3]);
      uint8_t* dst = yT + (int64_t)c0 * rows + r0;
#pragma unroll
      for (int j = 0; j < 4; ++j) {
        mi::st8<MI_NT_YT>(dst + (int64_t)j * rows, a[j], b[j]);
        mi::st8<MI_NT_YT>(dst + (int64_t)(j + 4) * rows, c[j], d[j]);
      }
    }
  }
  if (amax_out != nullptr) {
    amax = wave_max(amax);
    if (lane == 0) s_amax[wave] = amax;
    __syncthreads();
    if (tid == 0) {
      const float m = fmaxf(fmaxf(s_amax[0], s_amax[1]), fmaxf(s_amax[2], s_amax[3]));
      if (m > 0.0f && m > __builtin_nontemporal_load(amax_out)) atomicMax(reinterpret_cast<unsigned int*>(amax_out), __float_as_uint(m));
    }
  }
}

}

extern "C" int mi_rope_qkv(void* fused_bf16, void* q_bf16, void* k_bf16, void* v_bf16, const float* cos_tab,
                           const float* sin_tab, int64_t rows, int64_t seq, int n_q_heads, int n_kv_heads, int head_dim,
                           int backward, void* stream) {
  MI_CHECK_ARG(fused_bf16 && q_bf16 && k_bf16 && v_bf16 && cos_tab && sin_tab, "mi_rope_qkv: null pointer");
  MI_CHECK_ARG(rows >= 0 && seq > 0 && n_q_heads > 0 && n_kv_heads > 0, "mi_rope_qkv: bad shape");
  MI_CHECK_ARG(head_dim > 0 && head_dim % 16 == 0, "mi_rope_qkv: head_dim must be a multiple of 16");
  MI_CHECK_ARG(((uintptr_t)fused_bf16 % 16) == 0 && ((uintptr_t)q_bf16 % 16) == 0 && ((uintptr_t)k_bf16 % 16) == 0 &&
                   ((uintptr_t)v_bf16 % 16) == 0 && ((uintptr_t)cos_tab % 16) == 0 && ((uintptr_t)sin_tab % 16) == 0,
               "mi_rope_qkv: pointers must be 16-byte aligned");
  MI_CHECK_ARG(rows < (1LL << 31), "mi_rope_qkv: too many rows");
  if (rows == 0) return MI_OK;
  const int64_t per_row = (int64_t)(n_q_heads + n_kv_heads) * (head_dim / 16) + (int64_t)n_kv_heads * head_dim / 8;
  int64_t blocks = (rows * per_row + 255) / 256;
  if (blocks > 8192) blocks = 8192;
  if (backward)
    hipLaunchKernelGGL(mi::rope_qkv_kernel<1>, dim3((unsigned)blocks), dim3(256), 0, (hipStream_t)stream, (uint16_t*)fused_bf16,
                       (uint16_t*)q_bf16, (uint16_t*)k_bf16, (uint16_t*)v_bf16, cos_tab, sin_tab, (int)rows, (int)seq, n_q_heads,
                       n_kv_heads, head_dim);
  else
    hipLaunchKernelGGL(mi::rope_qkv_kernel<0>, dim3((unsigned)blocks), dim3(256), 0, (hipStream_t)stream, (uint16_t*)fused_bf16,
                       (uint16_t*)q_bf16, (uint16_t*)k_bf16, (uint16_t*)v_bf16, cos_tab, sin_tab, (int)rows, (int)seq, n_q_heads,
                       n_kv_heads, head_dim);
  MI_CHECK_LAUNCH("mi_rope_qkv launch");
  return MI_OK;
}

extern "C" int mi_rope_qkv_bwd_cast(const void* dq_bf16, const void* dk_bf16, const void* dv_bf16, const float* cos_tab,
                                    const float* sin_tab, void* y_fp8, void* yT_fp8, const float* scale, float* amax, int64_t rows,
                                    int64_t seq, int n_q_heads, int n_kv_heads, int head_dim, int fmt, void* stream) {
  MI_CHECK_ARG(dq_bf16 && dk_bf16 && dv_bf16 && cos_tab && sin_tab && scale, "mi_rope_qkv_bwd_cast: null pointer");
  MI_CHECK_ARG(y_fp8 || yT_fp8, "mi_rope_qkv_bwd_cast: at least one of y, yT must be non-null");
  MI_CHECK_ARG(head_dim == 128, "mi_rope_qkv_bwd_cast: head_dim %d not supported (128)", head_dim);
  MI_CHECK_ARG(n_q_heads >= 1 && n_kv_heads >= 1 && seq >= 1 && rows >= 0 && rows % 8 == 0 && rows < (1LL << 31),
               "mi_rope_qkv_bwd_cast: bad shape (rows a multiple of 8)");
  MI_CHECK_ARG(((uintptr_t)dq_bf16 % 16) == 0 && ((uintptr_t)dk_bf16 % 16) == 0 && ((uintptr_t)dv_bf16 % 16) == 0 &&
                   ((uintptr_t)cos_tab % 16) == 0 && ((uintptr_t)sin_tab % 16) == 0 && ((uintptr_t)y_fp8 % 8) == 0 &&
                   ((uintptr_t)yT_fp8 % 8) == 0, "mi_rope_qkv_bwd_cast: misaligned pointer");
  MI_CHECK_ARG(fmt == MI_FMT_E4M3 || fmt == MI_FMT_E5M2, "mi_rope_qkv_bwd_cast: bad fmt %d", fmt);
  if (rows == 0) return MI_OK;
  const int64_t units = ((rows + 63) / 64) * (int64_t)(n_q_heads + 3 * n_kv_heads);
  dim3 grid((unsigned)((units + 3) / 4)), block(256);
  hipStream_t st = (hipStream_t)stream;
#define MI_RC(FMTv)                                                                                                          \
  if (y_fp8 && yT_fp8)                                                                                                       \
    hipLaunchKernelGGL((mi::rope_bwd_cast_kernel<FMTv, true, true>), grid, block, 0, st, (const uint16_t*)dq_bf16,           \
                       (const uint16_t*)dk_bf16, (const uint16_t*)dv_bf16, cos_tab, sin_tab, (uint8_t*)y_fp8, (uint8_t*)yT_fp8, \
                       scale, amax, (int)rows, (int)seq, n_q_heads, n_kv_heads);                                             \
  else if (y_fp8)                                                                                                            \
    hipLaunchKernelGGL((mi::rope_bwd_cast_kernel<FMTv, true, false>), grid, block, 0, st, (const uint16_t*)dq_bf16,          \
                       (const uint16_t*)dk_bf16, (const uint16_t*)dv_bf16, cos_tab, sin_tab, (uint8_t*)y_fp8, (uint8_t*)yT_fp8, \
                       scale, amax, (int)rows, (int)seq, n_q_heads, n_kv_heads);                                             \
  else                                                                                                                       \
    hipLaunchKernelGGL((mi::rope_bwd_cast_kernel<FMTv, false, true>), grid, block, 0, st, (const uint16_t*)dq_bf16,          \
                       (const uint16_t*)dk_bf16, (const uint16_t*)dv_bf16, cos_tab, sin_tab, (uint8_t*)y_fp8, (uint8_t*)yT_fp8, \
                       scale, amax, (int)rows, (int)seq, n_q_heads, n_kv_heads);
  if (fmt == MI_FMT_E4M3) { MI_RC(MI_FMT_E4M3) } else { MI_RC(MI_FMT_E5M2) }
#undef MI_RC
  MI_CHECK_LAUNCH("mi_rope_qkv_bwd_cast launch");
  return MI_OK;
}

static int swiglu_common_check(const char* who, const void* h, const void* y, const void* yT, const float* scale,
                               int64_t rows, int64_t F, int fmt) {
  MI_CHECK_ARG(h && scale, "%s: null input", who);
  MI_CHECK_ARG(y || yT, "%s: at least one of y, yT must be non-null", who);
  MI_CHECK_ARG(rows >= 0 && F >= 0 && rows % 8 == 0 && F % 8 == 0, "%s: rows and F must be multiples of 8", who);
  MI_CHECK_ARG(rows < (1LL << 31) && 2 * F < (1LL << 31), "%s: shape too large", who);
  MI_CHECK_ARG(((uintptr_t)h % 16) == 0 && ((uintptr_t)y % 8) == 0 && ((uintptr_t)yT % 8) == 0, "%s: misaligned pointer", who);
  MI_CHECK_ARG(fmt == MI_FMT_E4M3 || fmt == MI_FMT_E5M2, "%s: bad fmt %d", who, fmt);
  return MI_OK;
}

extern "C" int mi_swiglu_cast(const void* h_bf16, void* y_fp8, void* yT_fp8, const float* scale, float* amax,
                              int64_t rows, int64_t F, int fmt, void* stream) {
  int rc = swiglu_common_check("mi_swiglu_cast", h_bf16, y_fp8, yT_fp8, scale, rows, F, fmt);
  if (rc != MI_OK) return rc;
  if (rows == 0 || F == 0) return MI_OK;
  hipStream_t st = (hipStream_t)stream;
  if (fmt == MI_FMT_E4M3) return mi::launch_swiglu<MI_FMT_E4M3, 0>(h_bf16, nullptr, y_fp8, yT_fp8, scale, amax, nullptr, rows, F, st);
  return mi::launch_swiglu<MI_FMT_E5M2, 0>(h_bf16, nullptr, y_fp8, yT_fp8, scale, amax, nullptr, rows, F, st);
}

extern "C" int mi_dswiglu_cast(const void* h_bf16, const void* dact_bf16, void* y_fp8, void* yT_fp8, const float* scale,
                               float* amax, float* colsum, int64_t rows, int64_t F, int fmt, void* stream) {
  int rc = swiglu_common_check("mi_dswiglu_cast", h_bf16, y_fp8, yT_fp8, scale, rows, F, fmt);
  if (rc != MI_OK) return rc;
  MI_CHECK_ARG(dact_bf16 && ((uintptr_t)dact_bf16 % 16) == 0, "mi_dswiglu_cast: dact must be non-null and 16-byte aligned");
  if (rows == 0 || F == 0) return MI_OK;
  hipStream_t st = (hipStream_t)stream;
  if (fmt == MI_FMT_E4M3)
    return mi::launch_swiglu<MI_FMT_E4M3, 1>(h_bf16, dact_bf16, y_fp8, yT_fp8, scale, amax, colsum, rows, F, st);
  return mi::launch_swiglu<MI_FMT_E5M2, 1>(h_bf16, dact_bf16, y_fp8, yT_fp8, scale, amax, colsum, rows, F, st);
}

extern "C" int mi_swiglu_cast_bias(const void* h_bf16, const void* bias_bf16, void* y_fp8, void* yT_fp8, const float* scale, float* amax,
                                   int64_t rows, int64_t F, int fmt, void* stream) {
  int rc = swiglu_common_check("mi_swiglu_cast_bias", h_bf16, y_fp8, yT_fp8, scale, rows, F, fmt);
  if (rc != MI_OK) return rc;
  MI_CHECK_ARG(bias_bf16 && ((uintptr_t)bias_bf16 % 16) == 0, "mi_swiglu_cast_bias: bias must be non-null and 16-byte aligned");
  if (rows == 0 || F == 0) return MI_OK;
  hipStream_t st = (hipStream_t)stream;
  if (fmt == MI_FMT_E4M3) return mi::launch_swiglu<MI_FMT_E4M3, 0>(h_bf16, nullptr, y_fp8, yT_fp8, scale, amax, nullptr, rows, F, st, bias_bf16);
  return mi::launch_swiglu<MI_FMT_E5M2, 0>(h_bf16, nullptr, y_fp8, yT_fp8, scale, amax, nullptr, rows, F, st, bias_bf16);
}

extern "C" int mi_dswiglu_cast_bias(const void* h_bf16, const void* bias_bf16, const void* dact_bf16, void* y_fp8, void* yT_fp8,
                                    const float* scale, float* amax, float* colsum, int64_t rows, int64_t F, int fmt, void* stream) {
  int rc = swiglu_common_check("mi_dswiglu_cast_bias", h_bf16, y_fp8, yT_fp8, scale, rows, F, fmt);
  if (rc != MI_OK) return rc;
  MI_CHECK_ARG(dact_bf16 && ((uintptr_t)dact_bf16 % 16) == 0, "mi_dswiglu_cast_bias: dact must be non-null and 16-byte aligned");
  MI_CHECK_ARG(bias_bf16 && ((uintptr_t)bias_bf16 % 16) == 0, "mi_dswiglu_cast_bias: bias must be non-null and 16-byte aligned");
  if (rows == 0 || F == 0) return MI_OK;
  hipStream_t st = (hipStream_t)stream;
  if (fmt == MI_FMT_E4M3)
    return mi::launch_swiglu<MI_FMT_E4M3, 1>(h_bf16, dact_bf16, y_fp8, yT_fp8, scale, amax, colsum, rows, F, st, bias_bf16);
  return mi::launch_swiglu<MI_FMT_E5M2, 1>(h_bf16, dact_bf16, y_fp8, yT_fp8, scale, amax, colsum, rows, F, st, bias_bf16);
}

namespace mi {
__global__ __launch_bounds__(256) void add_rmsnorm_stats_kernel(const uint16_t* __restrict__ a, const uint16_t* __restrict__ b,
                                                                uint16_t* __restrict__ out, float* __restrict__ rstd, int rows,
                                                                int cols, float eps, const uint16_t* __restrict__ bias) {
  const int lane = threadIdx.x & 63;
  const int row = blockIdx.x * 4 + (threadIdx.x >> 6);
  if (row >= rows) return;
  const int64_t off = (int64_t)row * cols;
  float acc = 0.0f;
  for (int c = lane * 8; c < cols; c += 512) {
    const v4i va = __builtin_nontemporal_load(reinterpret_cast<const v4i*>(a + off + c));
    const v4i vb = __builtin_nontemporal_load(reinterpret_cast<const v4i*>(b + off + c));
    v4i vbias = {0, 0, 0, 0};
    if (bias != nullptr) vbias = *reinterpret_cast<const v4i*>(bias + c);
    v4i vo;
#pragma unroll
    for (int j = 0; j < 4; ++j) {
      const u32 wa = (u32)va[j], wb = (u32)vb[j];
      float b0 = __uint_as_float(wb << 16), b1 = __uint_as_float(wb & 0xFFFF0000u);
      if (bias != nullptr) {
        b0 += __uint_as_float((u32)vbias[j] << 16);
        b1 += __uint_as_float((u32)vbias[j] & 0xFFFF0000u);
      }
      const u32 o = pack_bf16x2(__uint_as_float(wa << 16) + b0, __uint_as_float(wa & 0xFFFF0000u) + b1);
      const float lo = __uint_as_float(o << 16), hi = __uint_as_float(o & 0xFFFF0000u);
      acc += lo * lo + hi * hi;
      vo[j] = (int)o;
    }
    *reinterpret_cast<v4i*>(out + off + c) = vo;
  }
#pragma unroll
  for (int o = 32; o >= 1; o >>= 1) acc += __shfl_xor(acc, o);
  if (lane == 0) rstd[row] = rsqrtf(acc / (float)cols + eps);
}
}

extern "C" int mi_add_rmsnorm_stats(const void* a_bf16, const void* b_bf16, void* out_bf16, float* rstd, int64_t rows, int64_t cols,
                                    float eps, void* stream) {
  MI_CHECK_ARG(a_bf16 && b_bf16 && out_bf16 && rstd, "mi_add_rmsnorm_stats: null pointer");
  MI_CHECK_ARG(rows >= 0 && cols > 0 && cols % 8 == 0 && rows < (1LL << 31) && cols < (1LL << 31), "mi_add_rmsnorm_stats: bad shape");
  MI_CHECK_ARG((((uintptr_t)a_bf16 | (uintptr_t)b_bf16 | (uintptr_t)out_bf16) % 16) == 0, "mi_add_rmsnorm_stats: operands must be 16-byte aligned");
  if (rows == 0) return MI_OK;
  hipLaunchKernelGGL(mi::add_rmsnorm_stats_kernel, dim3((unsigned)((rows + 3) / 4)), dim3(256), 0, (hipStream_t)stream,
                     (const uint16_t*)a_bf16, (const uint16_t*)b_bf16, (uint16_t*)out_bf16, rstd, (int)rows, (int)cols, eps,
                     (const uint16_t*)nullptr);
  MI_CHECK_LAUNCH("mi_add_rmsnorm_stats launch");
  return MI_OK;
}

extern "C" int mi_add_bias_rmsnorm_stats(const void* a_bf16, const void* b_bf16, const void* bias_bf16, void* out_bf16, float* rstd,
                                         int64_t rows, int64_t cols, float eps, void* stream) {
  MI_CHECK_ARG(a_bf16 && b_bf16 && bias_bf16 && out_bf16 && rstd, "mi_add_bias_rmsnorm_stats: null pointer");
  MI_CHECK_ARG(rows >= 0 && cols > 0 && cols % 8 == 0 && rows < (1LL << 31) && cols < (1LL << 31), "mi_add_bias_rmsnorm_stats: bad shape");
  MI_CHECK_ARG((((uintptr_t)a_bf16 | (uintptr_t)b_bf16 | (uintptr_t)out_bf16 | (uintptr_t)bias_bf16) % 16) == 0,
               "mi_add_bias_rmsnorm_stats: operands must be 16-byte aligned");
  if (rows == 0) return MI_OK;
  hipLaunchKernelGGL(mi::add_rmsnorm_stats_kernel, dim3((unsigned)((rows + 3) / 4)), dim3(256), 0, (hipStream_t)stream,
                     (const uint16_t*)a_bf16, (const uint16_t*)b_bf16, (uint16_t*)out_bf16, rstd, (int)rows, (int)cols, eps,
                     (const uint16_t*)bias_bf16);
  MI_CHECK_LAUNCH("mi_add_bias_rmsnorm_stats launch");
  return MI_OK;
}

extern "C" int mi_rmsnorm_stats(const void* x_bf16, float* rstd, int64_t rows, int64_t cols, float eps, void* stream) {
  MI_CHECK_ARG(x_bf16 && rstd, "mi_rmsnorm_stats: null pointer");
  MI_CHECK_ARG(rows >= 0 && cols > 0 && cols % 8 == 0 && rows < (1LL << 31) && cols < (1LL << 31), "mi_rmsnorm_stats: bad shape");
  MI_CHECK_ARG(((uintptr_t)x_bf16 % 16) == 0, "mi_rmsnorm_stats: x must be 16-byte aligned");
  if (rows == 0) return MI_OK;
  hipLaunchKernelGGL(mi::rmsnorm_stats_kernel, dim3((unsigned)((rows + 3) / 4)), dim3(256), 0, (hipStream_t)stream,
                     (const uint16_t*)x_bf16, rstd, (int)rows, (int)cols, eps);
  MI_CHECK_LAUNCH("mi_rmsnorm_stats launch");
  return MI_OK;
}

extern "C" int mi_norm_cast(const void* x_bf16, const float* rstd, const void* gamma_bf16, void* y_fp8, void* yT_fp8,
                            const float* scale, float* amax, int64_t rows, int64_t cols, int fmt, void* stream) {
  MI_CHECK_ARG(x_bf16 && rstd && gamma_bf16 && scale, "mi_norm_cast: null input");
  MI_CHECK_ARG(y_fp8 || yT_fp8, "mi_norm_cast: at least one of y, yT must be non-null");
  MI_CHECK_ARG(rows >= 0 && cols >= 0 && rows % 8 == 0 && cols % 8 == 0, "mi_norm_cast: rows and cols must be multiples of 8");
  MI_CHECK_ARG(rows < (1LL << 31) && cols < (1LL << 31), "mi_norm_cast: shape too large");
  MI_CHECK_ARG(((uintptr_t)x_bf16 % 16) == 0 && ((uintptr_t)gamma_bf16 % 16) == 0 && ((uintptr_t)rstd % 16) == 0 &&
                   ((uintptr_t)y_fp8 % 8) == 0 && ((uintptr_t)yT_fp8 % 8) == 0, "mi_norm_cast: misaligned pointer");
  MI_CHECK_ARG(fmt == MI_FMT_E4M3 || fmt == MI_FMT_E5M2, "mi_norm_cast: bad fmt %d", fmt);
  if (rows == 0 || cols == 0) return MI_OK;
  MI_CHECK_ARG(((rows + 63) / 64) * ((cols + 63) / 64) < (1LL << 31), "mi_norm_cast: shape too large");
  const int tiles_r = (int)((rows + 63) / 64), tiles_c = (int)((cols + 63) / 64);
  const int64_t wgs = ((int64_t)tiles_r * tiles_c + 3) / 4;
  int ncu = 256, devid = 0;
  if (hipGetDevice(&devid) != hipSuccess || hipDeviceGetAttribute(&ncu, hipDeviceAttributeMultiprocessorCount, devid) != hipSuccess || ncu <= 0) ncu = 256;
  const int64_t cap = (int64_t)ncu * 2;
  dim3 grid((unsigned)(wgs < cap ? wgs : cap)), block(256);
  hipStream_t st = (hipStream_t)stream;
  const uint16_t *xp = (const uint16_t*)x_bf16, *gp = (const uint16_t*)gamma_bf16;
  uint8_t *yp = (uint8_t*)y_fp8, *tp = (uint8_t*)yT_fp8;
#define MI_NC(FMTv)                                                                                                        \
  if (y_fp8 && yT_fp8)                                                                                                     \
    hipLaunchKernelGGL((mi::norm_cast_kernel<FMTv, true, true>), grid, block, 0, st, xp, rstd, gp, yp, tp, scale, amax, (int)rows, (int)cols, tiles_c); \
  else if (y_fp8)                                                                                                          \
    hipLaunchKernelGGL((mi::norm_cast_kernel<FMTv, true, false>), grid, block, 0, st, xp, rstd, gp, yp, tp, scale, amax, (int)rows, (int)cols, tiles_c); \
  else                                                                                                                     \
    hipLaunchKernelGGL((mi::norm_cast_kernel<FMTv, false, true>), grid, block, 0, st, xp, rstd, gp, yp, tp, scale, amax, (int)rows, (int)cols, tiles_c);
  if (fmt == MI_FMT_E4M3) { MI_NC(MI_FMT_E4M3) } else { MI_NC(MI_FMT_E5M2) }
#undef MI_NC
  MI_CHECK_LAUNCH("mi_norm_cast launch");
  return MI_OK;
}

extern "C" int mi_rmsnorm_bwd(const void* dy_bf16, const void* x_bf16, const float* rstd, const void* gamma_bf16,
                              const void* dres_bf16, void* dx_bf16, float* dgamma_partial, int n_partials, int64_t rows,
                              int64_t cols, void* stream) {
  MI_CHECK_ARG(dy_bf16 && x_bf16 && rstd && gamma_bf16 && dx_bf16 && dgamma_partial, "mi_rmsnorm_bwd: null pointer");
  MI_CHECK_ARG(rows >= 0 && cols > 0 && cols % 512 == 0 && cols <= 512 * mi::kNormMaxVec, "mi_rmsnorm_bwd: cols must be a multiple of 512, at most %d", 512 * mi::kNormMaxVec);
  MI_CHECK_ARG(n_partials >= 1 && rows < (1LL << 31), "mi_rmsnorm_bwd: bad sizes");
  MI_CHECK_ARG(((uintptr_t)dy_bf16 % 16) == 0 && ((uintptr_t)x_bf16 % 16) == 0 && ((uintptr_t)gamma_bf16 % 16) == 0 &&
                   ((uintptr_t)dres_bf16 % 16) == 0 && ((uintptr_t)dx_bf16 % 16) == 0, "mi_rmsnorm_bwd: misaligned pointer");
  const int rows_per_block = (int)((rows + n_partials - 1) / n_partials);
  const int rpb = rows_per_block < 1 ? 1 : rows_per_block;
  const size_t shm = (size_t)(4 * cols * sizeof(float));
#define MI_RB(NV, WPRv)                                                                                                   \
  case NV:                                                                                                                \
    hipLaunchKernelGGL((mi::rmsnorm_bwd_kernel<NV, WPRv>), dim3(n_partials), dim3(256), shm, (hipStream_t)stream,         \
                       (const uint16_t*)dy_bf16, (const uint16_t*)x_bf16, rstd, (const uint16_t*)gamma_bf16,              \
                       (const uint16_t*)dres_bf16, (uint16_t*)dx_bf16, dgamma_partial, (int)rows, rpb);                   \
    break;
  switch ((int)(cols / 512)) {
    MI_RB(1, 1) MI_RB(2, 1) MI_RB(3, 1) MI_RB(4, 2) MI_RB(5, 1) MI_RB(6, 2) MI_RB(7, 1) MI_RB(8, 2) MI_RB(10, 2) MI_RB(12, 4)
    MI_RB(14, 2) MI_RB(16, 4)
    default:
      mi::set_error("mi_rmsnorm_bwd: unsupported width %lld (cols/512 must be 1-8, 10, 12, 14 or 16)", (long long)cols);
      return MI_ERR_SHAPE;
  }
#undef MI_RB
  MI_CHECK_LAUNCH("mi_rmsnorm_bwd launch");
  return MI_OK;
}

extern "C" int mi_ce_forward(const void* logits_bf16, const int64_t* labels, float* lse, float* loss_rows, int64_t rows,
                             int64_t cols, void* stream) {
  MI_CHECK_ARG(logits_bf16 && labels && lse && loss_rows, "mi_ce_forward: null pointer");
  MI_CHECK_ARG(rows >= 0 && cols > 0 && cols % 8 == 0 && rows < (1LL << 31) && cols < (1LL << 31), "mi_ce_forward: bad shape (cols % 8)");
  MI_CHECK_ARG(((uintptr_t)logits_bf16 % 16) == 0, "mi_ce_forward: logits must be 16-byte aligned");
  if (rows == 0) return MI_OK;
  hipLaunchKernelGGL(mi::ce_fwd_kernel, dim3((unsigned)rows), dim3(256), 0, (hipStream_t)stream, (const uint16_t*)logits_bf16, labels,
                     lse, loss_rows, (int)cols);
  MI_CHECK_LAUNCH("mi_ce_forward launch");
  return MI_OK;
}

extern "C" int mi_ce_backward(const void* logits_bf16, const int64_t* labels, const float* lse, const float* gscale,
                              void* dlogits_bf16, int64_t rows, int64_t cols, void* stream) {
  MI_CHECK_ARG(logits_bf16 && labels && lse && gscale && dlogits_bf16, "mi_ce_backward: null pointer");
  MI_CHECK_ARG(rows >= 0 && cols > 0 && cols % 8 == 0 && rows < (1LL << 31) && cols < (1LL << 31), "mi_ce_backward: bad shape (cols % 8)");
  MI_CHECK_ARG(((uintptr_t)logits_bf16 % 16) == 0 && ((uintptr_t)dlogits_bf16 % 16) == 0, "mi_ce_backward: misaligned pointer");
  if (rows == 0) return MI_OK;
  hipLaunchKernelGGL(mi::ce_bwd_kernel, dim3((unsigned)rows), dim3(256), 0, (hipStream_t)stream, (const uint16_t*)logits_bf16, labels,
                     lse, gscale, (uint16_t*)dlogits_bf16, (int)cols);
  MI_CHECK_LAUNCH("mi_ce_backward launch");
  return MI_OK;
}

extern "C" int mi_ce_backward_cast(const void* logits_bf16, const int64_t* labels, const float* lse, const float* gscale,
                                   void* y_fp8, void* yT_fp8, const float* scale, float* amax, int64_t rows, int64_t cols, int fmt,
                                   void* stream) {
  MI_CHECK_ARG(logits_bf16 && labels && lse && gscale && scale, "mi_ce_backward_cast: null pointer");
  MI_CHECK_ARG(y_fp8 || yT_fp8, "mi_ce_backward_cast: at least one of y, yT must be non-null");
  MI_CHECK_ARG(rows >= 0 && cols > 0 && rows % 8 == 0 && cols % 8 == 0 && rows < (1LL << 31) && cols < (1LL << 31),
               "mi_ce_backward_cast: rows and cols must be multiples of 8");
  MI_CHECK_ARG(((uintptr_t)logits_bf16 % 16) == 0 && ((uintptr_t)y_fp8 % 8) == 0 && ((uintptr_t)yT_fp8 % 8) == 0,
               "mi_ce_backward_cast: misaligned pointer");
  MI_CHECK_ARG(fmt == MI_FMT_E4M3 || fmt == MI_FMT_E5M2, "mi_ce_backward_cast: bad fmt %d", fmt);
  if (rows == 0) return MI_OK;
  const int tiles_r = (int)((rows + 127) / 128), tiles_c = (int)((cols + 127) / 128);
  MI_CHECK_ARG((int64_t)tiles_r * tiles_c < (1LL << 31), "mi_ce_backward_cast: shape too large");
  dim3 grid((unsigned)(tiles_r * tiles_c)), block(256);
  hipStream_t st = (hipStream_t)stream;
#define MI_CC(FMTv, WY, WT)                                                                                              \
  hipLaunchKernelGGL((mi::ce_bwd_cast_kernel<FMTv, WY, WT>), grid, block, 0, st, (const uint16_t*)logits_bf16, labels, lse, \
                     gscale, (uint8_t*)y_fp8, (uint8_t*)yT_fp8, scale, amax, (int)rows, (int)cols, tiles_c)
#define MI_CC_F(FMTv)                                    \
  if (y_fp8 && yT_fp8) MI_CC(FMTv, true, true);          \
  else if (y_fp8) MI_CC(FMTv, true, false);              \
  else MI_CC(FMTv, false, true);
  if (fmt == MI_FMT_E4M3) { MI_CC_F(MI_FMT_E4M3) } else { MI_CC_F(MI_FMT_E5M2) }
#undef MI_CC_F
#undef MI_CC
  MI_CHECK_LAUNCH("mi_ce_backward_cast launch");
  return MI_OK;
}
```

llm_fp8_amd/pytorch/attention.py:

```python
from __future__ import annotations

import os
import weakref
from typing import Optional

import torch
import torch.nn.functional as F

from . import ops
from .module import DyHandoff, LayerNormLinear, Linear, handoff_readers

__all__ = ["RotaryPositionEmbedding", "apply_rotary_pos_emb", "DotProductAttention", "MultiheadAttention"]


class RotaryPositionEmbedding(torch.nn.Module):

    def __init__(self, dim: int, rotary_percent: float = 1.0, seq_len_interpolation_factor=None,
                 pretrained_max_position_embeddings=None, rotary_base: float = 10000.0):
        super().__init__()
        if rotary_percent < 1.0:
            dim = int(dim * rotary_percent)
        self.dim = dim
        self.seq_len_interpolation_factor = seq_len_interpolation_factor
        inv_freq = 1.0 / (rotary_base ** (torch.arange(0, dim, 2, dtype=torch.float32) / dim))
        self.register_buffer("inv_freq", inv_freq, persistent=False)

    def forward(self, max_seq_len: int, offset: int = 0) -> torch.Tensor:
        seq = torch.arange(max_seq_len, device=self.inv_freq.device, dtype=torch.float32) + offset
        if self.seq_len_interpolation_factor is not None:
            seq = seq / self.seq_len_interpolation_factor
        freqs = torch.outer(seq, self.inv_freq)
        emb = torch.cat((freqs, freqs), dim=-1)
        return emb.reshape(emb.size(0), 1, 1, emb.size(1))


def _rotate_half(x: torch.Tensor) -> torch.Tensor:
    x1, x2 = x.chunk(2, dim=-1)
    return torch.cat((-x2, x1), dim=-1)


def apply_rotary_pos_emb(t: torch.Tensor, freqs: torch.Tensor, tensor_format: str = "sbhd") -> torch.Tensor:
    s = t.shape[0] if tensor_format == "sbhd" else t.shape[1]
    f = freqs[:s]
    if tensor_format == "bshd":
        f = f.transpose(0, 1)
    cos, sin = torch.cos(f).to(t.dtype), torch.sin(f).to(t.dtype)
    rot = f.shape[-1]
    tr, tp = t[..., :rot], t[..., rot:]
    out = tr * cos + _rotate_half(tr) * sin
    return out if tp.shape[-1] == 0 else torch.cat((out, tp), dim=-1)


_COS_SIN_CACHE = {}


def _cos_sin_tables(freqs: torch.Tensor, seq: int):
    key = (freqs.data_ptr(), freqs.shape, seq, str(freqs.device))
    hit = _COS_SIN_CACHE.get(key)
    if hit is None:
        half = freqs.shape[-1] // 2
        f = freqs[:seq, 0, 0, :half].float()
        hit = (torch.cos(f).contiguous(), torch.sin(f).contiguous())
        if len(_COS_SIN_CACHE) > 16:
            _COS_SIN_CACHE.clear()
        _COS_SIN_CACHE[key] = hit
    return hit


class _RoPESplitFn(torch.autograd.Function):

    @staticmethod
    def forward(ctx, qkv, cos, sin, n_q, n_kv, d, handoff=None):
        B, S, W = qkv.shape
        x = qkv.reshape(B * S, W)
        x = x if x.is_contiguous() else x.contiguous()
        q, k, v = ops.rope_qkv_forward(x, cos, sin, n_q, n_kv, d, S)
        ctx.save_for_backward(cos, sin)
        ctx.meta = (B, S, n_q, n_kv, d)
        ctx.handoff = handoff
        ctx.act_ref = weakref.ref(qkv) if handoff is not None else None
        return q.view(B, S, n_q, d), k.view(B, S, n_kv, d), v.view(B, S, n_kv, d)

    @staticmethod
    def backward(ctx, dq, dk, dv):
        cos, sin = ctx.saved_tensors
        B, S, n_q, n_kv, d = ctx.meta
        T = B * S
        h = ctx.handoff
        if h is not None and h.offered() and handoff_readers(ctx.act_ref()):
            h = None
        if h is not None and h.offered() and d == 128 and T % (32 if h.mx else 8) == 0:
            args = (dq.reshape(T, n_q * d), dk.reshape(T, n_kv * d), dv.reshape(T, n_kv * d), cos, sin, n_q, n_kv, d, S)
            if h.mx:
                fp8 = ops.mxfp8_rope_bwd_quantize(*args, h.fmt, rowwise=h.want_y, colwise=h.want_t)
            else:
                fp8 = ops.rope_qkv_backward_cast(*args, h.scale, h.amax, h.fmt, want_y=h.want_y, want_t=h.want_t)
            g = torch.empty((B, S, (n_q + 2 * n_kv) * d), dtype=torch.bfloat16, device=dq.device)
            h.put(fp8, g)
            return g, None, None, None, None, None, None
        g = ops.rope_qkv_backward(dq.reshape(T, n_q * d), dk.reshape(T, n_kv * d), dv.reshape(T, n_kv * d), cos, sin,
                                  n_q, n_kv, d, S)
        return g.view(B, S, -1), None, None, None, None, None, None


class _FlashAttnFn(torch.autograd.Function):

    @staticmethod
    def forward(ctx, q, k, v, scale, causal):
        o, lse = ops.attn_fwd(q, k, v, scale, causal)
        ctx.save_for_backward(q, k, v, o, lse)
        ctx.scale, ctx.causal = scale, causal
        return o

    @staticmethod
    def backward(ctx, do):
        q, k, v, o, lse = ctx.saved_tensors
        ok = (do.stride(3) == 1 and do.stride(2) == do.shape[3] and do.stride(0) == do.shape[1] * do.stride(1)
              and do.stride(1) % 8 == 0 and do.data_ptr() % 16 == 0)
        do = do if ok else do.clone(memory_format=torch.contiguous_format)
        dq, dk, dv = ops.attn_bwd(do, q, k, v, o, lse, ctx.scale, ctx.causal)
        return dq, dk, dv, None, None


def _flash_ok(q, k, v, causal: bool, dropout: float) -> bool:
    if not (q.is_cuda and q.dtype == k.dtype == v.dtype == torch.bfloat16 and dropout == 0.0 and causal):
        return False
    B, S, H, D = q.shape
    if D not in (64, 128) or S % 16 or S < 128 or H % k.shape[2]:
        return False
    return all(t.stride(3) == 1 and t.stride(2) == D and t.stride(0) == S * t.stride(1) and t.stride(1) % 8 == 0
               and S * t.stride(1) * 2 < 2 ** 31 and t.data_ptr() % 16 == 0 for t in (q, k, v))


class DotProductAttention(torch.nn.Module):

    def __init__(self, num_attention_heads: int, kv_channels: int, num_gqa_groups: Optional[int] = None,
                 attention_dropout: float = 0.0, attn_mask_type: str = "causal", qkv_format: str = "bshd", **_ignored):
        super().__init__()
        self.h, self.d = num_attention_heads, kv_channels
        self.g = num_gqa_groups or num_attention_heads
        self.p, self.attn_mask_type, self.qkv_format = attention_dropout, attn_mask_type, qkv_format

    def forward(self, q, k, v, attention_mask=None):
        if self.qkv_format == "sbhd":
            q, k, v = (t.transpose(0, 1) for t in (q, k, v))
        causal = self.attn_mask_type in ("causal", "padding_causal")
        if _flash_ok(q, k, v, causal, self.p if self.training else 0.0):
            o = _FlashAttnFn.apply(q, k, v, self.d ** -0.5, True)
            if self.qkv_format == "sbhd":
                o = o.transpose(0, 1)
            return o.reshape(*o.shape[:2], self.h * self.d)
        q, k, v = (t.transpose(1, 2) for t in (q, k, v))
        mask = None
        if not causal and attention_mask is not None:
            mask = ~attention_mask if attention_mask.dtype == torch.bool else attention_mask
        o = F.scaled_dot_product_attention(q, k, v, attn_mask=mask, dropout_p=self.p if self.training else 0.0,
                                           is_causal=causal, enable_gqa=(self.g != self.h))
        o = o.transpose(1, 2)
        if self.qkv_format == "sbhd":
            o = o.transpose(0, 1)
        return o.reshape(*o.shape[:2], self.h * self.d)


class MultiheadAttention(torch.nn.Module):

    def __init__(self, hidden_size: int, num_attention_heads: int, kv_channels: Optional[int] = None,
                 attention_dropout: float = 0.1, layernorm_epsilon: float = 1e-5, init_method=None,
                 output_layer_init_method=None, attn_mask_type: str = "causal", num_gqa_groups: Optional[int] = None,
                 input_layernorm: bool = False, attention_type: str = "self", fuse_qkv_params: bool = False,
                 zero_centered_gamma: bool = False, qkv_weight_interleaved: bool = True, bias: bool = True,
                 normalization: str = "LayerNorm", qkv_format: str = "sbhd", params_dtype=None, device="cuda",
                 **_ignored):
        super().__init__()
        assert attention_type == "self", "only self-attention is on the reference path"
        assert qkv_format in ("sbhd", "bshd")
        self.hidden_size, self.h = hidden_size, num_attention_heads
        self.d = kv_channels or hidden_size // num_attention_heads
        self.g = num_gqa_groups or num_attention_heads
        self.qkv_format, self.input_layernorm = qkv_format, input_layernorm
        q_out, kv_out = self.h * self.d, self.g * self.d
        self.split = (q_out, kv_out, kv_out)
        if fuse_qkv_params:
            psplit = None
        else:
            psplit = {"query_": q_out, "key_": kv_out, "value_": kv_out}
        if input_layernorm:
            self.layernorm_qkv = LayerNormLinear(hidden_size, sum(self.split), eps=layernorm_epsilon, bias=bias,
                                                 normalization=normalization, parameters_split=psplit,
                                                 params_dtype=params_dtype, device=device,
                                                 zero_centered_gamma=zero_centered_gamma, init_method=init_method)
        else:
            self.qkv = Linear(hidden_size, sum(self.split), bias=bias, params_dtype=params_dtype, device=device,
                              init_method=init_method)
        self.core_attention = DotProductAttention(self.h, self.d, self.g, attention_dropout, attn_mask_type, qkv_format)
        self.proj = Linear(q_out, hidden_size, bias=bias, params_dtype=params_dtype, device=device,
                           init_method=output_layer_init_method or init_method)

    def forward(self, hidden_states: torch.Tensor, attention_mask: Optional[torch.Tensor] = None,
                rotary_pos_emb=None, _with_skip: bool = False, _rstd=None, **_ignored):
        if _with_skip:
            if not self.input_layernorm:
                return self._attend(self.qkv(hidden_states), attention_mask, rotary_pos_emb), hidden_states
            handoff = DyHandoff() if (rotary_pos_emb is not None and hidden_states.is_cuda and torch.is_grad_enabled()
                                      and os.environ.get("LLM_FP8_AMD_NO_DY_HANDOFF") != "1") else None
            qkv, skip = self.layernorm_qkv(hidden_states, _with_skip=True, _rstd=_rstd, _dy_handoff=handoff)
            return self._attend(qkv, attention_mask, rotary_pos_emb, handoff), skip
        qkv = self.layernorm_qkv(hidden_states) if self.input_layernorm else self.qkv(hidden_states)
        return self._attend(qkv, attention_mask, rotary_pos_emb)

    def _attend(self, qkv: torch.Tensor, attention_mask, rotary_pos_emb, handoff=None) -> torch.Tensor:
        if (rotary_pos_emb is not None and not isinstance(rotary_pos_emb, (tuple, list)) and qkv.is_cuda
                and qkv.dtype == torch.bfloat16 and self.qkv_format == "bshd" and self.d % 16 == 0
                and rotary_pos_emb.shape[-1] == self.d):
            cos, sin = _cos_sin_tables(rotary_pos_emb, qkv.shape[1])
            q, k, v = _RoPESplitFn.apply(qkv, cos, sin, self.h, self.g, self.d, handoff)
            return self.proj(self.core_attention(q, k, v, attention_mask))
        if handoff is not None:
            handoff.withdraw()
        q, k, v = torch.split(qkv, self.split, dim=-1)
        a, b = qkv.shape[0], qkv.shape[1]
        q = q.reshape(a, b, self.h, self.d)
        k = k.reshape(a, b, self.g, self.d)
        v = v.reshape(a, b, self.g, self.d)
        if rotary_pos_emb is not None:
            fq, fk = rotary_pos_emb if isinstance(rotary_pos_emb, (tuple, list)) else (rotary_pos_emb, rotary_pos_emb)
            q = apply_rotary_pos_emb(q, fq, self.qkv_format)
            k = apply_rotary_pos_emb(k, fk, self.qkv_format)
        ctx = self.core_attention(q, k, v, attention_mask)
        return self.proj(ctx)
```

llm_fp8_amd/pytorch/ops.py:

```python
from __future__ import annotations

import ctypes
import os
from typing import Optional, Tuple

import torch

from .. import _lib
from .profiler import KernelTimer

E4M3, E5M2 = _lib.MI_FMT_E4M3, _lib.MI_FMT_E5M2
FP8_MAX = {E4M3: 448.0, E5M2: 57344.0}


_SK_WORKSPACE = {}


def ensure_gemm_workspace(device: torch.device) -> None:
    idx = device.index if device.index is not None else torch.cuda.current_device()
    if idx in _SK_WORKSPACE:
        return
    lib = _lib.load()
    with torch.cuda.device(idx):
        nbytes = int(lib.mi_gemm_workspace_bytes())
        ws = torch.zeros(nbytes, dtype=torch.uint8, device=torch.device("cuda", idx))
        torch.cuda.synchronize(idx)
        _lib.check(lib.mi_gemm_set_workspace(ws.data_ptr(), nbytes), "mi_gemm_set_workspace")
    _SK_WORKSPACE[idx] = ws


def default_gemm_algo() -> int:
    env = os.environ.get("LLM_FP8_AMD_GEMM_ALGO")
    if env is not None:
        return int(env)
    d = torch.distributed
    if d.is_available() and d.is_initialized() and d.get_world_size() > 1:
        return 5
    return 47 if os.environ.get("LLM_FP8_AMD_GEMM_W4", "1") != "0" else 0


def _stream() -> int:
    return torch.cuda.current_stream().cuda_stream


def _dev(*ts):
    for t in ts:
        if t is not None and not t.is_cuda:
            raise RuntimeError("llm_fp8_amd ops need device (HIP) tensors; there is no CPU fallback")


def _ptr(t: Optional[torch.Tensor]) -> Optional[int]:
    return None if t is None else t.data_ptr()


def colsum_finish(partial: torch.Tensor, dtype: torch.dtype = torch.bfloat16) -> torch.Tensor:
    _dev(partial)
    assert partial.dtype == torch.float32 and partial.dim() == 2 and partial.is_contiguous()
    P, C = partial.shape
    if dtype not in (torch.bfloat16, torch.float32):
        return partial.sum(0).to(dtype)
    out = torch.empty(C, dtype=dtype, device=partial.device)
    _lib.check(_lib.load().mi_colsum_finish(partial.data_ptr(), P, C, out.data_ptr(), 0 if dtype == torch.bfloat16 else 1, _stream()),
               "mi_colsum_finish")
    return out


def colsum_finish_multi(items):
    import ctypes
    outs = [None] * len(items)
    todo = []
    for i, (partial, dtype) in enumerate(items):
        _dev(partial)
        assert partial.dtype == torch.float32 and partial.dim() == 2 and partial.is_contiguous()
        if dtype not in (torch.bfloat16, torch.float32):
            outs[i] = partial.sum(0).to(dtype)
        else:
            outs[i] = torch.empty(partial.shape[1], dtype=dtype, device=partial.device)
            todo.append(i)
    for k in range(0, len(todo), 4):
        grp = todo[k:k + 4]
        n = len(grp)
        parts = (ctypes.c_void_p * n)(*[items[i][0].data_ptr() for i in grp])
        Ps = (ctypes.c_int64 * n)(*[items[i][0].shape[0] for i in grp])
        Cs = (ctypes.c_int64 * n)(*[items[i][0].shape[1] for i in grp])
        os_ = (ctypes.c_void_p * n)(*[outs[i].data_ptr() for i in grp])
        dts = (ctypes.c_int * n)(*[0 if items[i][1] == torch.bfloat16 else 1 for i in grp])
        _lib.check(_lib.load().mi_colsum_finish_multi(parts, Ps, Cs, os_, dts, n, _stream()), "mi_colsum_finish_multi")
    return outs


def cast_amax(x: torch.Tensor, scale: torch.Tensor, amax: Optional[torch.Tensor], fmt: int,
              want_y: bool = True, want_t: bool = True,
              y: Optional[torch.Tensor] = None, yT: Optional[torch.Tensor] = None, want_colsum: bool = False):
    _dev(x, scale, amax, y, yT)
    assert x.dtype == torch.bfloat16 and x.dim() == 2 and x.is_contiguous()
    assert scale.dtype == torch.float32 and (amax is None or amax.dtype == torch.float32)
    R, C = x.shape
    if want_y and y is None:
        y = torch.empty((R, C), dtype=torch.uint8, device=x.device)
    if want_t and yT is None:
        yT = torch.empty((C, R), dtype=torch.uint8, device=x.device)
    if y is not None:
        assert y.dtype == torch.uint8 and y.shape == (R, C) and y.stride(1) == 1
    if yT is not None:
        assert yT.dtype == torch.uint8 and yT.shape == (C, R) and yT.stride(1) == 1
    cs = torch.empty(((R + 63) // 64, C), dtype=torch.float32, device=x.device) if want_colsum else None
    tail = (R, C, y.stride(0) if y is not None else C, yT.stride(0) if yT is not None else R, fmt, _stream())
    head = (x.data_ptr(), _ptr(y), _ptr(yT), scale.data_ptr(), _ptr(amax))
    fn = _lib.load().mi_cast_amax_colsum if want_colsum else _lib.load().mi_cast_amax
    args = head + ((cs.data_ptr(),) if want_colsum else ()) + tail
    t = KernelTimer.active
    if t is None:
        rc = fn(*args)
    else:
        nb = R * C * (2 + (y is not None) + (yT is not None))
        with t.span("cast_amax", f"{R}x{C}", float(R * C), float(nb)):
            rc = fn(*args)
    _lib.check(rc, "mi_cast_amax")
    return (y, yT, cs) if want_colsum else (y, yT)


def scale_update(amax_history: torch.Tensor, scale: torch.Tensor, scale_inv: torch.Tensor,
                 fp8_max: torch.Tensor, margin: int = 0, algo: str = "max") -> None:
    _dev(amax_history, scale, scale_inv, fp8_max)
    assert amax_history.dim() == 2 and amax_history.stride(1) == 1 and amax_history.dtype == torch.float32
    H, S = amax_history.shape
    assert scale.numel() == S and scale_inv.numel() == S and fp8_max.numel() == S
    assert scale.is_contiguous() and scale_inv.is_contiguous() and fp8_max.is_contiguous()
    rc = _lib.load().mi_scale_update(amax_history.data_ptr(), scale.data_ptr(), scale_inv.data_ptr(),
                                     fp8_max.data_ptr(), H, S, amax_history.stride(0), margin,
                                     0 if algo == "max" else 1, _stream())
    _lib.check(rc, "mi_scale_update")


def gemm_fp8(a8: torch.Tensor, b8: torch.Tensor, sa_inv: torch.Tensor, sb_inv: torch.Tensor,
             fmt_a: int, fmt_b: int, bias: Optional[torch.Tensor] = None,
             out: Optional[torch.Tensor] = None, out_dtype: torch.dtype = torch.bfloat16,
             algo: Optional[int] = None) -> torch.Tensor:
    if algo is None:
        algo = default_gemm_algo()
        M_, N_, K_ = a8.shape[0], b8.shape[0], a8.shape[1]
        if algo == 3 and (M_ % 256 or N_ % 256 or K_ % 128):
            algo = 0
        if algo == 47 and (out_dtype != torch.bfloat16 or (out is not None and out.dtype != torch.bfloat16)):
            algo = 0
        if algo == 5 and ((M_ % 256 and M_ % 192) or (N_ % 256 and N_ % 192) or K_ % 256 or out_dtype != torch.bfloat16
                          or (out is not None and out.dtype != torch.bfloat16)):
            algo = 0
    _dev(a8, b8, sa_inv, sb_inv, bias, out)
    if algo == 44:
        ensure_gemm_workspace(a8.device)
    assert a8.dtype == torch.uint8 and b8.dtype == torch.uint8 and a8.dim() == 2 and b8.dim() == 2
    assert a8.stride(1) == 1 and b8.stride(1) == 1
    M, K = a8.shape
    N, K2 = b8.shape
    assert K == K2, f"contraction mismatch {K} vs {K2}"
    if out is None:
        out = torch.empty((M, N), dtype=out_dtype, device=a8.device)
    assert out.shape == (M, N) and out.stride(1) == 1 and out.dtype in (torch.bfloat16, torch.float32)
    if bias is not None:
        assert bias.dtype == torch.bfloat16 and bias.numel() == N and bias.is_contiguous()
    args = (a8.data_ptr(), b8.data_ptr(), out.data_ptr(), sa_inv.data_ptr(), sb_inv.data_ptr(), _ptr(bias), M, N, K,
            a8.stride(0), b8.stride(0), out.stride(0), fmt_a, fmt_b, 0 if out.dtype == torch.bfloat16 else 1, algo,
            _stream())
    t = KernelTimer.active
    if t is None:
        rc = _lib.load().mi_gemm_fp8(*args)
    else:
        with t.span("gemm_fp8", f"{M}x{N}x{K}", 2.0 * M * N * K, M * K + N * K + out.element_size() * M * N):
            rc = _lib.load().mi_gemm_fp8(*args)
    _lib.check(rc, "mi_gemm_fp8")
    return out


def mxfp8_quantize(x: torch.Tensor, fmt: int = E4M3, rowwise: bool = True, colwise: bool = True, out=None,
                   want_colsum: bool = False):
    _dev(x)
    assert x.dtype == torch.bfloat16 and x.dim() == 2 and x.is_contiguous()
    R, C = x.shape
    y_row = s_row = y_colT = s_colT = None
    ld = R
    if out is not None:
        y_row, s_row, y_colT, s_colT = out
        _dev(y_row, s_row, y_colT, s_colT)
        assert (y_row is not None) == rowwise and (y_colT is not None) == colwise
        if rowwise:
            assert y_row.shape == (R, C) and y_row.is_contiguous() and s_row.shape == (C // 32, R) and s_row.stride(1) == 1
            ld = s_row.stride(0)
        if colwise:
            assert y_colT.shape == (C, R) and y_colT.stride(1) == 1 and s_colT.shape == (R // 32, C) and s_colT.is_contiguous()
            assert not rowwise or y_colT.stride(0) == ld
            ld = y_colT.stride(0)
    else:
        if rowwise:
            y_row = torch.empty((R, C), dtype=torch.uint8, device=x.device)
            s_row = torch.empty((C // 32, R), dtype=torch.uint8, device=x.device)
        if colwise:
            y_colT = torch.empty((C, R), dtype=torch.uint8, device=x.device)
            s_colT = torch.empty((R // 32, C), dtype=torch.uint8, device=x.device)
    cs = torch.empty(((R + 127) // 128, C), dtype=torch.float32, device=x.device) if want_colsum else None
    if out is None and not want_colsum:
        fn, args = _lib.load().mi_mxfp8_quantize, (x.data_ptr(), _ptr(y_row), _ptr(s_row), _ptr(y_colT), _ptr(s_colT), R, C, fmt, _stream())
    else:
        fn, args = _lib.load().mi_mxfp8_quantize_ex, (x.data_ptr(), _ptr(y_row), _ptr(s_row), _ptr(y_colT), _ptr(s_colT), _ptr(cs),
                                                      R, C, ld, fmt, _stream())
    t = KernelTimer.active
    if t is None:
        rc = fn(*args)
    else:
        nb = R * C * (2 + (1 + 1 / 32) * (int(rowwise) + int(colwise)))
        with t.span("mxfp8_quantize", f"{R}x{C}", float(R * C), float(nb)):
            rc = fn(*args)
    _lib.check(rc, "mi_mxfp8_quantize")
    return (y_row, s_row, y_colT, s_colT, cs) if want_colsum else (y_row, s_row, y_colT, s_colT)


def gemm_mxfp8(a8, sa, b8, sb, fmt_a: int = E4M3, fmt_b: int = E4M3, bias=None, out=None,
               out_dtype: torch.dtype = torch.bfloat16, algo: Optional[int] = None) -> torch.Tensor:
    _dev(a8, sa, b8, sb, bias, out)
    if algo is None:
        algo = default_gemm_algo()
        M_, N_, K_ = a8.shape[0], b8.shape[0], a8.shape[1]
        if algo not in (0, 1, 4, 5) or (algo == 5 and ((M_ % 256 and M_ % 192) or (N_ % 256 and N_ % 192) or K_ % 256
                                                      or out_dtype != torch.bfloat16 or (out is not None and out.dtype != torch.bfloat16))):
            algo = 0
    if algo == 44:
        ensure_gemm_workspace(a8.device)
    M, K = a8.shape
    N, K2 = b8.shape
    assert K == K2 and a8.is_contiguous() and b8.is_contiguous() and sa.is_contiguous() and sb.is_contiguous()
    assert sa.shape == (K // 32, M) and sb.shape == (K // 32, N), "scales must be block-major [K/32, rows]"
    if out is None:
        out = torch.empty((M, N), dtype=out_dtype, device=a8.device)
    assert out.is_contiguous() and out.shape == (M, N)
    args = (a8.data_ptr(), sa.data_ptr(), b8.data_ptr(), sb.data_ptr(), out.data_ptr(), _ptr(bias), M, N, K, fmt_a,
            fmt_b, 0 if out.dtype == torch.bfloat16 else 1, algo, _stream())
    t = KernelTimer.active
    if t is None:
        rc = _lib.load().mi_gemm_mxfp8(*args)
    else:
        with t.span("gemm_mxfp8", f"{M}x{N}x{K}", 2.0 * M * N * K, M * K + N * K + out.element_size() * M * N):
            rc = _lib.load().mi_gemm_mxfp8(*args)
    _lib.check(rc, "mi_gemm_mxfp8")
    return out


def rope_qkv_forward(qkv: torch.Tensor, cos: torch.Tensor, sin: torch.Tensor, n_q: int, n_kv: int, head_dim: int, seq: int):
    _dev(qkv, cos, sin)
    assert qkv.dtype == torch.bfloat16 and qkv.is_contiguous() and qkv.dim() == 2
    T, W = qkv.shape
    assert W == (n_q + 2 * n_kv) * head_dim and cos.dtype == torch.float32 and cos.shape[-1] == head_dim // 2 and cos.shape[0] >= seq
    q = torch.empty((T, n_q * head_dim), dtype=torch.bfloat16, device=qkv.device)
    k = torch.empty((T, n_kv * head_dim), dtype=torch.bfloat16, device=qkv.device)
    v = torch.empty((T, n_kv * head_dim), dtype=torch.bfloat16, device=qkv.device)
    rc = _lib.load().mi_rope_qkv(qkv.data_ptr(), q.data_ptr(), k.data_ptr(), v.data_ptr(), cos.data_ptr(), sin.data_ptr(),
                                 T, seq, n_q, n_kv, head_dim, 0, _stream())
    _lib.check(rc, "mi_rope_qkv")
    return q, k, v


def rope_qkv_backward(dq: torch.Tensor, dk: torch.Tensor, dv: torch.Tensor, cos: torch.Tensor, sin: torch.Tensor,
                      n_q: int, n_kv: int, head_dim: int, seq: int) -> torch.Tensor:
    _dev(dq, dk, dv, cos, sin)
    dq, dk, dv = (t.contiguous() for t in (dq, dk, dv))
    T = dq.shape[0]
    out = torch.empty((T, (n_q + 2 * n_kv) * head_dim), dtype=torch.bfloat16, device=dq.device)
    rc = _lib.load().mi_rope_qkv(out.data_ptr(), dq.data_ptr(), dk.data_ptr(), dv.data_ptr(), cos.data_ptr(), sin.data_ptr(),
                                 T, seq, n_q, n_kv, head_dim, 1, _stream())
    _lib.check(rc, "mi_rope_qkv")
    return out


def mxfp8_rope_bwd_quantize(dq: torch.Tensor, dk: torch.Tensor, dv: torch.Tensor, cos: torch.Tensor, sin: torch.Tensor, n_q: int,
                            n_kv: int, head_dim: int, seq: int, fmt: int, rowwise: bool = True, colwise: bool = True):
    _dev(dq, dk, dv, cos, sin)
    dq, dk, dv = (t.contiguous() for t in (dq, dk, dv))
    T, W = dq.shape[0], (n_q + 2 * n_kv) * head_dim
    y_row = s_row = y_colT = s_colT = None
    if rowwise:
        y_row = torch.empty((T, W), dtype=torch.uint8, device=dq.device)
        s_row = torch.empty((W // 32, T), dtype=torch.uint8, device=dq.device)
    if colwise:
        y_colT = torch.empty((W, T), dtype=torch.uint8, device=dq.device)
        s_colT = torch.empty((T // 32, W), dtype=torch.uint8, device=dq.device)
    args = (dq.data_ptr(), dk.data_ptr(), dv.data_ptr(), cos.data_ptr(), sin.data_ptr(), _ptr(y_row), _ptr(s_row), _ptr(y_colT),
            _ptr(s_colT), T, seq, n_q, n_kv, head_dim, fmt, _stream())
    t = KernelTimer.active
    if t is None:
        rc = _lib.load().mi_mxfp8_rope_bwd_quantize(*args)
    else:
        with t.span("mxfp8_quantize", f"rope {T}x{W}", float(T * W), float(T * W * (2 + (1 + 1 / 32) * (int(rowwise) + int(colwise))))):
            rc = _lib.load().mi_mxfp8_rope_bwd_quantize(*args)
    _lib.check(rc, "mi_mxfp8_rope_bwd_quantize")
    return y_row, s_row, y_colT, s_colT


def _group_shapes(problems, mx: bool):
    ib = 2 if mx else 1
    return tuple((p[0].shape[0], p[ib].shape[0], p[0].shape[1]) for p in problems)


def _grouped_launch(entry: str, span: str, arr, shapes, fmt_a: int, fmt_b: int, tile_cfg: int) -> None:
    fn = getattr(_lib.load(), entry)
    args = (ctypes.byref(arr), len(shapes), fmt_a, fmt_b, tile_cfg, _stream())
    t = KernelTimer.active
    if t is None:
        rc = fn(*args)
    else:
        work = sum(2.0 * M * N * K for M, N, K in shapes)
        nbytes = sum(M * K + N * K + 2 * M * N for M, N, K in shapes)
        with t.span(span, "+".join(f"{M}x{N}x{K}" for M, N, K in shapes), work, nbytes):
            rc = fn(*args)
    _lib.check(rc, entry)


def gemm_fp8_grouped(problems, fmt_a: int, fmt_b: int, tile_cfg: int = -1) -> None:
    arr = (_lib.GemmProblem * len(problems))()
    for i, (a8, b8, sa, sb, out) in enumerate(problems):
        _dev(a8, b8, sa, sb, out)
        assert a8.dtype == torch.uint8 and b8.dtype == torch.uint8 and out.dtype == torch.bfloat16
        assert a8.stride(1) == 1 and b8.stride(1) == 1 and out.stride(1) == 1 and a8.shape[1] == b8.shape[1]
        assert out.shape == (a8.shape[0], b8.shape[0])
        arr[i] = _lib.GemmProblem(a8.data_ptr(), b8.data_ptr(), out.data_ptr(), sa.data_ptr(), sb.data_ptr(), a8.shape[0], b8.shape[0],
                                  a8.shape[1], a8.stride(0), b8.stride(0), out.stride(0))
    _grouped_launch("mi_gemm_fp8_grouped", "gemm_fp8", arr, _group_shapes(problems, False), fmt_a, fmt_b, tile_cfg)


def gemm_mxfp8_grouped(problems, fmt_a: int, fmt_b: int, tile_cfg: int = -1) -> None:
    arr = (_lib.GemmMxProblem * len(problems))()
    for i, (a8, sa, b8, sb, out) in enumerate(problems):
        _dev(a8, sa, b8, sb, out)
        M, K = a8.shape
        N, K2 = b8.shape
        assert a8.dtype == torch.uint8 and b8.dtype == torch.uint8 and out.dtype == torch.bfloat16
        assert K == K2 and a8.is_contiguous() and b8.is_contiguous() and sa.is_contiguous() and sb.is_contiguous()
        assert sa.shape == (K // 32, M) and sb.shape == (K // 32, N), "scales must be block-major [K/32, rows]"
        assert out.is_contiguous() and out.shape == (M, N)
        arr[i] = _lib.GemmMxProblem(a8.data_ptr(), sa.data_ptr(), b8.data_ptr(), sb.data_ptr(), out.data_ptr(), M, N, K)
    _grouped_launch("mi_gemm_mxfp8_grouped", "gemm_mxfp8", arr, _group_shapes(problems, True), fmt_a, fmt_b, tile_cfg)


def grouped_gemm_ok(shapes, strides_ok: bool = True) -> bool:
    if not strides_ok or not shapes or len(shapes) > 4:
        return False
    if not any(all(M % bm == 0 and N % bn == 0 for M, N, K in shapes) for bm, bn in _TILE_CFGS):
        return False
    if any(K % 256 or M * K >= 2 ** 31 or N * K >= 2 ** 31 or M * N * 2 >= 2 ** 31 for M, N, K in shapes):
        return False
    return True


_TILE_CFGS = ((256, 256), (256, 192), (192, 256), (192, 192))
_TILE_EFF = (1.0, 0.90, 0.90, 0.80)
_GROUP_PLAN: dict = {}


def grouped_gemm_plan(shapes, n_cu: int = 256) -> int:
    key = (tuple(shapes), n_cu)
    if key in _GROUP_PLAN:
        return _GROUP_PLAN[key]
    import heapq
    best = -1
    if grouped_gemm_ok(shapes):
        fixed = 4.0
        sep = 0.0
        for M, N, K in shapes:
            c = min((-(-((M // bm) * (N // bn)) // n_cu)) * (K // 128) * (bm * bn / 65536.0) / eff
                    for (bm, bn), eff in zip(_TILE_CFGS, _TILE_EFF) if M % bm == 0 and N % bn == 0)
            sep += c + fixed
        best_cost = None
        for cfg, ((bm, bn), eff) in enumerate(zip(_TILE_CFGS, _TILE_EFF)):
            if any(M % bm or N % bn for M, N, K in shapes):
                continue
            probs = sorted(((K // 128, (M // bm) * (N // bn)) for M, N, K in shapes), reverse=True)
            total = sum(t for _, t in probs)
            g = min(total, n_cu)
            loads = [(0, v) for v in range(g)]
            heapq.heapify(loads)
            per_wg = [0] * g
            for nk, tiles in probs:
                for _ in range(tiles):
                    load, v = heapq.heappop(loads)
                    per_wg[v] += 1
                    heapq.heappush(loads, (load + nk, v))
            if max(per_wg) > 64:
                continue
            cost = max(l for l, _ in loads) * (bm * bn / 65536.0) / eff * 1.02 + fixed
            if best_cost is None or cost < best_cost:
                best_cost, best = cost, cfg
        if best_cost is None or best_cost >= 0.98 * sep:
            best = -1
    _GROUP_PLAN[key] = best
    return best


_GROUP_TUNED: dict = {}


def grouped_gemm_choice(problems, fmt_a: int, fmt_b: int, mx: bool = False) -> int:
    mode = os.environ.get("LLM_FP8_AMD_GROUPED_GEMM", "auto")
    if mode == "off":
        return -1
    if mode == "auto":
        import torch.distributed as dist
        mode = "plan" if (dist.is_available() and dist.is_initialized()) else "autotune"
    if mode == "plan":
        return grouped_gemm_plan(_group_shapes(problems, mx))
    if mode != "autotune":
        raise ValueError(f"LLM_FP8_AMD_GROUPED_GEMM={mode!r}: expected auto, plan, autotune or off")
    return grouped_gemm_autotune(problems, fmt_a, fmt_b, mx=mx)


def _tuned_key(shapes, fmt_a: int, fmt_b: int, mx: bool):
    return ("mx", tuple(shapes), fmt_a, fmt_b) if mx else (tuple(shapes), fmt_a, fmt_b)


def grouped_gemm_autotune(problems, fmt_a: int, fmt_b: int, iters: int = 5, mx: bool = False) -> int:
    shapes = _group_shapes(problems, mx)
    key = _tuned_key(shapes, fmt_a, fmt_b, mx)
    hit = _GROUP_TUNED.get(key)
    if hit is not None:
        return hit
    single, grouped = (gemm_mxfp8, gemm_mxfp8_grouped) if mx else (gemm_fp8, gemm_fp8_grouped)
    problems = [(*p[:4], torch.empty_like(p[4])) for p in problems]
    cands = [-1]
    if grouped_gemm_ok(shapes):
        cands += [cfg for cfg, (bm, bn) in enumerate(_TILE_CFGS) if all(M % bm == 0 and N % bn == 0 for M, N, K in shapes)]
        if (not mx and all(M % 256 == 0 and N % 256 == 0 and K >= 512 for M, N, K in shapes)
                and os.environ.get("LLM_FP8_AMD_GEMM_W4G", "1") != "0"):
            cands.append(4)

    def run(c):
        if c == -1:
            for p in problems:
                single(*p[:4], fmt_a, fmt_b, out=p[4])
        else:
            grouped(problems, fmt_a, fmt_b, tile_cfg=c)

    saved, KernelTimer.active = KernelTimer.active, None
    try:
        live = []
        for c in cands:
            try:
                run(c)
                live.append(c)
            except RuntimeError:
                continue
        total = {c: 0.0 for c in live}
        for r in range(iters):
            order = live[r % len(live):] + live[:r % len(live)]
            for c in order:
                e0, e1 = torch.cuda.Event(enable_timing=True), torch.cuda.Event(enable_timing=True)
                e0.record()
                run(c)
                run(c)
                e1.record()
                e1.synchronize()
                total[c] += e0.elapsed_time(e1)
        best, best_t = -1, total.get(-1)
        for c in live:
            if c == -1:
                continue
            t = total[c]
            if best_t is None or t < best_t * (0.98 if best == -1 else 1.0):
                best, best_t = c, t
        if 4 in total and best not in (-1, 4) and total[4] <= 1.01 * best_t:
            best, best_t = 4, total[4]
    finally:
        KernelTimer.active = saved
    _GROUP_TUNED[key] = best
    return best


def transpose_u8(y: torch.Tensor, out: Optional[torch.Tensor] = None) -> torch.Tensor:
    _dev(y)
    assert y.dtype == torch.uint8 and y.dim() == 2 and y.stride(1) == 1
    R, C = y.shape
    if out is None:
        out = torch.empty((C, R), dtype=torch.uint8, device=y.device)
    assert out.shape == (C, R) and out.dtype == torch.uint8 and out.stride(1) == 1
    if R == 0 or C == 0:
        return out
    _lib.check(_lib.load().mi_transpose_u8(y.data_ptr(), out.data_ptr(), R, C, y.stride(0), out.stride(0), _stream()), "mi_transpose_u8")
    return out


def embedding_grad_add_(grad: torch.Tensor, dy: torch.Tensor, ids: torch.Tensor, alpha: float = 1.0, padding_idx: int = -1) -> None:
    _dev(grad, dy, ids)
    assert grad.dtype == torch.bfloat16 and dy.dtype == torch.bfloat16 and grad.is_contiguous() and grad.dim() == 2
    dy = dy.reshape(-1, dy.shape[-1])
    dy = dy if dy.is_contiguous() else dy.contiguous()
    ids = ids.reshape(-1).to(torch.int64)
    assert dy.shape == (ids.numel(), grad.shape[1])
    sorted_ids, perm = torch.sort(ids, stable=True)
    rc = _lib.load().mi_embedding_grad_add(grad.data_ptr(), dy.data_ptr(), sorted_ids.data_ptr(), perm.data_ptr(), ids.numel(),
                                           grad.shape[1], grad.shape[0], float(alpha), int(padding_idx), _stream())
    _lib.check(rc, "mi_embedding_grad_add")


def rope_qkv_backward_cast(dq: torch.Tensor, dk: torch.Tensor, dv: torch.Tensor, cos: torch.Tensor, sin: torch.Tensor,
                           n_q: int, n_kv: int, head_dim: int, seq: int, scale: torch.Tensor, amax: Optional[torch.Tensor],
                           fmt: int, want_y: bool = True, want_t: bool = True):
    _dev(dq, dk, dv, cos, sin, scale, amax)
    dq, dk, dv = (t.contiguous() for t in (dq, dk, dv))
    T = dq.shape[0]
    W = (n_q + 2 * n_kv) * head_dim
    y = torch.empty((T, W), dtype=torch.uint8, device=dq.device) if want_y else None
    yT = torch.empty((W, T), dtype=torch.uint8, device=dq.device) if want_t else None
    args = (dq.data_ptr(), dk.data_ptr(), dv.data_ptr(), cos.data_ptr(), sin.data_ptr(), _ptr(y), _ptr(yT), scale.data_ptr(),
            _ptr(amax), T, seq, n_q, n_kv, head_dim, fmt, _stream())
    t = KernelTimer.active
    if t is None:
        rc = _lib.load().mi_rope_qkv_bwd_cast(*args)
    else:
        with t.span("cast_amax", f"rope {T}x{W}", float(T * W), float(T * W * (2 + (y is not None) + (yT is not None)))):
            rc = _lib.load().mi_rope_qkv_bwd_cast(*args)
    _lib.check(rc, "mi_rope_qkv_bwd_cast")
    return y, yT


def swiglu_cast(h: torch.Tensor, scale: torch.Tensor, amax: Optional[torch.Tensor], fmt: int, want_y: bool = True,
                want_t: bool = True, bias: Optional[torch.Tensor] = None):
    _dev(h, scale, amax, bias)
    assert h.dtype == torch.bfloat16 and h.dim() == 2 and h.is_contiguous() and h.shape[1] % 2 == 0
    R, F2 = h.shape
    F = F2 // 2
    y = torch.empty((R, F), dtype=torch.uint8, device=h.device) if want_y else None
    yT = torch.empty((F, R), dtype=torch.uint8, device=h.device) if want_t else None
    if bias is None:
        fn, args = _lib.load().mi_swiglu_cast, (h.data_ptr(), _ptr(y), _ptr(yT), scale.data_ptr(), _ptr(amax), R, F, fmt, _stream())
    else:
        assert bias.dtype == torch.bfloat16 and bias.numel() == F2 and bias.is_contiguous()
        fn, args = _lib.load().mi_swiglu_cast_bias, (h.data_ptr(), bias.data_ptr(), _ptr(y), _ptr(yT), scale.data_ptr(), _ptr(amax), R, F, fmt, _stream())
    t = KernelTimer.active
    if t is None:
        rc = fn(*args)
    else:
        with t.span("swiglu_cast", f"{R}x{F}", float(R * F), float(R * F * (4 + int(want_y) + int(want_t)))):
            rc = fn(*args)
    _lib.check(rc, "mi_swiglu_cast")
    return y, yT


def dswiglu_cast(h: torch.Tensor, dact: torch.Tensor, scale: torch.Tensor, amax: Optional[torch.Tensor], fmt: int,
                 want_y: bool = True, want_t: bool = True, want_colsum: bool = False, bias: Optional[torch.Tensor] = None):
    _dev(h, dact, scale, amax, bias)
    assert h.dtype == torch.bfloat16 and dact.dtype == torch.bfloat16 and h.is_contiguous() and dact.is_contiguous()
    R, F2 = h.shape
    F = F2 // 2
    assert dact.shape == (R, F)
    y = torch.empty((R, F2), dtype=torch.uint8, device=h.device) if want_y else None
    yT = torch.empty((F2, R), dtype=torch.uint8, device=h.device) if want_t else None
    cs = torch.empty(((R + 127) // 128, F2), dtype=torch.float32, device=h.device) if want_colsum else None
    if bias is None:
        fn = _lib.load().mi_dswiglu_cast
        args = (h.data_ptr(), dact.data_ptr(), _ptr(y), _ptr(yT), scale.data_ptr(), _ptr(amax), _ptr(cs), R, F, fmt, _stream())
    else:
        assert bias.dtype == torch.bfloat16 and bias.numel() == F2 and bias.is_contiguous()
        fn = _lib.load().mi_dswiglu_cast_bias
        args = (h.data_ptr(), bias.data_ptr(), dact.data_ptr(), _ptr(y), _ptr(yT), scale.data_ptr(), _ptr(amax), _ptr(cs), R, F, fmt, _stream())
    t = KernelTimer.active
    if t is None:
        rc = fn(*args)
    else:
        with t.span("dswiglu_cast", f"{R}x{F}", float(R * F2), float(R * F * (6 + 2 * int(want_y) + 2 * int(want_t)))):
            rc = fn(*args)
    _lib.check(rc, "mi_dswiglu_cast")
    return y, yT, cs


def rmsnorm_stats(x: torch.Tensor, eps: float) -> torch.Tensor:
    _dev(x)
    assert x.dtype == torch.bfloat16 and x.dim() == 2 and x.is_contiguous()
    R, C = x.shape
    rstd = torch.empty(R, dtype=torch.float32, device=x.device)
    _lib.check(_lib.load().mi_rmsnorm_stats(x.data_ptr(), rstd.data_ptr(), R, C, float(eps), _stream()), "mi_rmsnorm_stats")
    return rstd


def add_rmsnorm_stats(a: torch.Tensor, b: torch.Tensor, eps: float, bias: Optional[torch.Tensor] = None):
    _dev(a, b, bias)
    assert a.dtype == torch.bfloat16 and b.dtype == torch.bfloat16 and a.shape == b.shape and a.is_contiguous() and b.is_contiguous()
    C = a.shape[-1]
    R = a.numel() // C
    out = torch.empty_like(a)
    rstd = torch.empty(R, dtype=torch.float32, device=a.device)
    if bias is None:
        rc = _lib.load().mi_add_rmsnorm_stats(a.data_ptr(), b.data_ptr(), out.data_ptr(), rstd.data_ptr(), R, C, float(eps), _stream())
    else:
        assert bias.dtype == torch.bfloat16 and bias.numel() == C and bias.is_contiguous()
        rc = _lib.load().mi_add_bias_rmsnorm_stats(a.data_ptr(), b.data_ptr(), bias.data_ptr(), out.data_ptr(), rstd.data_ptr(), R, C,
                                                   float(eps), _stream())
    _lib.check(rc, "mi_add_rmsnorm_stats")
    return out, rstd


def norm_cast(x: torch.Tensor, rstd: torch.Tensor, gamma: torch.Tensor, scale: torch.Tensor, amax: Optional[torch.Tensor],
              fmt: int, want_y: bool = True, want_t: bool = True):
    _dev(x, rstd, gamma, scale, amax)
    assert x.dtype == torch.bfloat16 and gamma.dtype == torch.bfloat16 and x.is_contiguous() and gamma.is_contiguous()
    R, C = x.shape
    y = torch.empty((R, C), dtype=torch.uint8, device=x.device) if want_y else None
    yT = torch.empty((C, R), dtype=torch.uint8, device=x.device) if want_t else None
    args = (x.data_ptr(), rstd.data_ptr(), gamma.data_ptr(), _ptr(y), _ptr(yT), scale.data_ptr(), _ptr(amax), R, C, fmt, _stream())
    t = KernelTimer.active
    if t is None:
        rc = _lib.load().mi_norm_cast(*args)
    else:
        with t.span("norm_cast", f"{R}x{C}", float(R * C), float(R * C * (2 + int(want_y) + int(want_t)))):
            rc = _lib.load().mi_norm_cast(*args)
    _lib.check(rc, "mi_norm_cast")
    return y, yT


def rmsnorm_bwd(dy: torch.Tensor, x: torch.Tensor, rstd: torch.Tensor, gamma: torch.Tensor,
                dres: Optional[torch.Tensor] = None, n_partials: int = 512, dgamma_dtype: torch.dtype = torch.float32,
                finish: bool = True):
    _dev(dy, x, rstd, gamma, dres)
    assert dy.dtype == torch.bfloat16 and x.dtype == torch.bfloat16 and dy.is_contiguous() and x.is_contiguous()
    R, C = x.shape
    n_partials = max(1, min(n_partials, (R + 3) // 4))
    dx = torch.empty_like(x)
    part = torch.empty((n_partials, C), dtype=torch.float32, device=x.device)
    rc = _lib.load().mi_rmsnorm_bwd(dy.data_ptr(), x.data_ptr(), rstd.data_ptr(), gamma.data_ptr(), _ptr(dres), dx.data_ptr(),
                                    part.data_ptr(), n_partials, R, C, _stream())
    _lib.check(rc, "mi_rmsnorm_bwd")
    return (dx, colsum_finish(part, dgamma_dtype)) if finish else (dx, part)


def _mx_alloc(R: int, C: int, dev, rowwise: bool, colwise: bool):
    y_row = s_row = y_colT = s_colT = None
    if rowwise:
        y_row = torch.empty((R, C), dtype=torch.uint8, device=dev)
        s_row = torch.empty((C // 32, R), dtype=torch.uint8, device=dev)
    if colwise:
        y_colT = torch.empty((C, R), dtype=torch.uint8, device=dev)
        s_colT = torch.empty((R // 32, C), dtype=torch.uint8, device=dev)
    return y_row, s_row, y_colT, s_colT


def _mx_call(kind: str, fn, args, R: int, C: int, in_bytes: float, rowwise: bool, colwise: bool):
    t = KernelTimer.active
    if t is None:
        rc = fn(*args)
    else:
        with t.span("mxfp8_quantize", f"{kind} {R}x{C}", float(R * C), in_bytes + R * C * (1 + 1 / 32) * (int(rowwise) + int(colwise))):
            rc = fn(*args)
    _lib.check(rc, f"mi_mxfp8_{kind}_quantize")


def mxfp8_norm_quantize(x: torch.Tensor, rstd: torch.Tensor, gamma: torch.Tensor, fmt: int = E4M3, rowwise: bool = True,
                        colwise: bool = True):
    _dev(x, rstd, gamma)
    assert x.dtype == torch.bfloat16 and gamma.dtype == torch.bfloat16 and x.is_contiguous() and gamma.is_contiguous()
    R, C = x.shape
    out = _mx_alloc(R, C, x.device, rowwise, colwise)
    _mx_call("norm", _lib.load().mi_mxfp8_norm_quantize,
             (x.data_ptr(), rstd.data_ptr(), gamma.data_ptr(), *[_ptr(o) for o in out], R, C, fmt, _stream()), R, C, 2.0 * R * C,
             rowwise, colwise)
    return out


def mxfp8_swiglu_quantize(h: torch.Tensor, fmt: int = E4M3, rowwise: bool = True, colwise: bool = True):
    _dev(h)
    assert h.dtype == torch.bfloat16 and h.is_contiguous() and h.shape[1] % 2 == 0
    R, F = h.shape[0], h.shape[1] // 2
    out = _mx_alloc(R, F, h.device, rowwise, colwise)
    _mx_call("swiglu", _lib.load().mi_mxfp8_swiglu_quantize, (h.data_ptr(), *[_ptr(o) for o in out], R, F, fmt, _stream()), R, F,
             4.0 * R * F, rowwise, colwise)
    return out


def mxfp8_dswiglu_quantize(h: torch.Tensor, dact: torch.Tensor, fmt: int = E4M3, rowwise: bool = True, colwise: bool = True,
                           want_colsum: bool = False):
    _dev(h, dact)
    assert h.dtype == torch.bfloat16 and dact.dtype == torch.bfloat16 and h.is_contiguous() and dact.is_contiguous()
    R, F2 = h.shape
    F = F2 // 2
    assert dact.shape == (R, F)
    out = _mx_alloc(R, F2, h.device, rowwise, colwise)
    cs = torch.empty(((R + 127) // 128, F2), dtype=torch.float32, device=h.device) if want_colsum else None
    _mx_call("dswiglu", _lib.load().mi_mxfp8_dswiglu_quantize,
             (h.data_ptr(), dact.data_ptr(), *[_ptr(o) for o in out], _ptr(cs), R, F, fmt, _stream()), R, F2, 6.0 * R * F,
             rowwise, colwise)
    return (*out, cs)


def _bshd_ok(t: torch.Tensor, D: int):
    assert t.dtype == torch.bfloat16 and t.dim() == 4 and t.shape[3] == D and t.stride(3) == 1 and t.stride(2) == D
    assert t.stride(0) == t.shape[1] * t.stride(1), "batch and sequence must collapse to one token stride"


def attn_fwd(q: torch.Tensor, k: torch.Tensor, v: torch.Tensor, scale: float, causal: bool = True, out=None):
    _dev(q, k, v)
    B, S, H, D = q.shape
    G = k.shape[2]
    for t in (q, k, v):
        _bshd_ok(t, D)
    if out is None:
        o = torch.empty((B, S, H, D), dtype=torch.bfloat16, device=q.device)
        lse = torch.empty((B, H, S), dtype=torch.float32, device=q.device)
    else:
        o, lse = out
        _dev(o, lse)
        _bshd_ok(o, D)
        assert o.shape == q.shape and lse.shape == (B, H, S) and lse.dtype == torch.float32 and lse.is_contiguous()
    args = (q.data_ptr(), k.data_ptr(), v.data_ptr(), o.data_ptr(), lse.data_ptr(), B, S, H, G, D, q.stride(1), k.stride(1),
            v.stride(1), o.stride(1), float(scale), int(causal), _stream())
    t = KernelTimer.active
    flops = 4.0 * B * H * S * S * D * (0.5 if causal else 1.0)
    if t is None:
        rc = _lib.load().mi_attn_fwd(*args)
    else:
        with t.span("attn_fwd", f"{B}x{S}x{H}x{D}", flops, 2.0 * (q.numel() * 2 + k.numel() * 2)):
            rc = _lib.load().mi_attn_fwd(*args)
    _lib.check(rc, "mi_attn_fwd")
    return o, lse


def attn_bwd(do: torch.Tensor, q: torch.Tensor, k: torch.Tensor, v: torch.Tensor, o: torch.Tensor, lse: torch.Tensor,
             scale: float, causal: bool = True, out=None):
    _dev(do, q, k, v, o, lse)
    B, S, H, D = q.shape
    G = k.shape[2]
    for t in (q, k, v, o, do):
        _bshd_ok(t, D)
    assert o.shape == do.shape == q.shape and lse.shape == (B, H, S) and lse.dtype == torch.float32 and lse.is_contiguous()
    if out is None:
        dq = torch.empty((B, S, H, D), dtype=torch.bfloat16, device=q.device)
        dk = torch.empty((B, S, G, D), dtype=torch.bfloat16, device=q.device)
        dv = torch.empty((B, S, G, D), dtype=torch.bfloat16, device=q.device)
    else:
        dq, dk, dv = out
        _dev(dq, dk, dv)
        for t in out:
            _bshd_ok(t, D)
        assert dq.shape == q.shape and dk.shape == dv.shape == k.shape
    delta = torch.empty((B, H, S), dtype=torch.float32, device=q.device)
    args = (q.data_ptr(), k.data_ptr(), v.data_ptr(), o.data_ptr(), do.data_ptr(), lse.data_ptr(), delta.data_ptr(),
            dq.data_ptr(), dk.data_ptr(), dv.data_ptr(), B, S, H, G, D, q.stride(1), k.stride(1), v.stride(1), o.stride(1),
            do.stride(1), dq.stride(1), dk.stride(1), dv.stride(1), float(scale), int(causal), _stream())
    t = KernelTimer.active
    flops = 14.0 * B * H * S * S * D * (0.5 if causal else 1.0)
    if t is None:
        rc = _lib.load().mi_attn_bwd(*args)
    else:
        with t.span("attn_bwd", f"{B}x{S}x{H}x{D}", flops, 2.0 * (3 * q.numel() + 4 * k.numel())):
            rc = _lib.load().mi_attn_bwd(*args)
    _lib.check(rc, "mi_attn_bwd")
    return dq, dk, dv
```

Before: 89100 tokens/s.

## Fuse RoPE backward and FP8 cast into attention backward epilogues

```diff
diff --git a/include/mi_fp8.h b/include/mi_fp8.h
--- a/include/mi_fp8.h
+++ b/include/mi_fp8.h
@@ -151,6 +151,10 @@
                 float* delta, void* dq, void* dk, void* dv, int B, int S, int H, int G, int D, int64_t q_ts,
                 int64_t k_ts, int64_t v_ts, int64_t o_ts, int64_t do_ts, int64_t dq_ts, int64_t dk_ts, int64_t dv_ts,
                 float scale, int causal, void* stream);
+int mi_attn_bwd_rope_cast(const void* q, const void* k, const void* v, const void* o, const void* dout, const float* lse,
+                          float* delta, const float* cos_tab, const float* sin_tab, const float* scale_fp8, float* amax,
+                          void* y_fp8, void* yT_fp8, int B, int S, int H, int G, int D, int64_t q_ts, int64_t k_ts, int64_t v_ts,
+                          int64_t o_ts, int64_t do_ts, float scale, int causal, int fmt, void* stream);
 
 #ifdef __cplusplus
 }
diff --git a/llm_fp8_amd/_lib.py b/llm_fp8_amd/_lib.py
--- a/llm_fp8_amd/_lib.py
+++ b/llm_fp8_amd/_lib.py
@@ -69,6 +69,7 @@
     "mi_attn_fwd": [_p, _p, _p, _p, _p, _c_int, _c_int, _c_int, _c_int, _c_int, _c_i64, _c_i64, _c_i64, _c_i64, ctypes.c_float,
                     _c_int, _p],
     "mi_attn_bwd": [_p] * 10 + [_c_int] * 5 + [_c_i64] * 8 + [ctypes.c_float, _c_int, _p],
+    "mi_attn_bwd_rope_cast": [_p] * 13 + [_c_int] * 5 + [_c_i64] * 5 + [ctypes.c_float, _c_int, _c_int, _p],
     "mi_mxfp8_norm_quantize": [_p, _p, _p, _p, _p, _p, _p, _c_i64, _c_i64, _c_int, _p],
     "mi_mxfp8_swiglu_quantize": [_p, _p, _p, _p, _p, _c_i64, _c_i64, _c_int, _p],
     "mi_mxfp8_dswiglu_quantize": [_p, _p, _p, _p, _p, _p, _p, _c_i64, _c_i64, _c_int, _p],
diff --git a/llm_fp8_amd/csrc/mi_attn.hip b/llm_fp8_amd/csrc/mi_attn.hip
--- a/llm_fp8_amd/csrc/mi_attn.hip
+++ b/llm_fp8_amd/csrc/mi_attn.hip
@@ -1,4 +1,5 @@
 #include "mi_common.h"
+#include "mi_rope_cast_dev.h"
 
 namespace mi {
 
@@ -271,9 +272,8 @@
 }
 
 
-template <int D, bool TAIL = false>
-__device__ __forceinline__ void store_rows_from_accT(const f16v (&acc)[D / 32], float mul, char* slice, uint16_t* out,
-                                                     int64_t row_stride, int lane, int nrows = 32) {
+template <int D>
+__device__ __forceinline__ void acc_to_slice(const f16v (&acc)[D / 32], float mul, char* slice, int lane) {
   const int r = lane & 31, h = lane >> 5;
   constexpr int CPR = D / 8;
 #pragma unroll
@@ -286,6 +286,12 @@
       pk.y = pack_bf16x2(acc[d][4 * i + 2] * mul, acc[d][4 * i + 3] * mul);
       *reinterpret_cast<uint2*>(slice + r * (D * 2) + 16 * (ch ^ (r & (CPR - 1))) + 8 * h) = pk;
     }
+}
+template <int D, bool TAIL = false>
+__device__ __forceinline__ void store_rows_from_accT(const f16v (&acc)[D / 32], float mul, char* slice, uint16_t* out,
+                                                     int64_t row_stride, int lane, int nrows = 32) {
+  constexpr int CPR = D / 8;
+  acc_to_slice<D>(acc, mul, slice, lane);
   __builtin_amdgcn_s_waitcnt(0xc07f);
   __builtin_amdgcn_wave_barrier();
 #pragma unroll
@@ -296,13 +302,51 @@
   }
 }
 
-template <int D, bool CAUSAL, bool TAIL = false>
+struct CastEpi {
+  const float* cosT;
+  const float* sinT;
+  const float* scale;
+  float* amax;
+  uint8_t* y;
+  uint8_t* yT;
+};
+
+template <int CAST, bool ROTATE>
+__device__ __forceinline__ void cast_image(const char* img, const CastEpi& ce, float scale8, float& amax, int row0, int col0,
+                                           int S, int rows, int W, int tid) {
+  constexpr int FMT = (CAST & 4) ? MI_FMT_E5M2 : MI_FMT_E4M3;
+  const int lane = tid & 63, w = tid >> 6;
+  const int lr = (w >> 1) * 64 + (lane >> 3) * 8, ch = (w & 1) * 8 + (lane & 7);
+  auto chunk = [&](int row, int c) { return *reinterpret_cast<const v4i*>(img + 256 * row + 16 * (c ^ (row & 15))); };
+  float f[8][8];
+  if (!ROTATE) {
+#pragma unroll
+    for (int i = 0; i < 8; ++i) bf16_row8(chunk(lr + i, ch), f[i]);
+  } else if ((w & 1) == 0) {
+#pragma unroll
+    for (int i = 0; i < 8; ++i) {
+      const int64_t t = (int64_t)((row0 + lr + i) % S) * 64 + (ch & 7) * 8;
+      rope_bwd_row8<true, false>(chunk(lr + i, ch), chunk(lr + i, ch ^ 8), ce.cosT + t, ce.sinT + t, f[i], nullptr);
+    }
+  } else {
+#pragma unroll
+    for (int i = 0; i < 8; ++i) {
+      const int64_t t = (int64_t)((row0 + lr + i) % S) * 64 + (ch & 7) * 8;
+      rope_bwd_row8<false, true>(chunk(lr + i, ch ^ 8), chunk(lr + i, ch), ce.cosT + t, ce.sinT + t, nullptr, f[i]);
+    }
+  }
+  emit_fp8_block<FMT, (CAST & 1) != 0, (CAST & 2) != 0>(f, scale8, amax, ce.y, ce.yT, row0 + lr, col0 + 8 * ch, W, rows);
+}
+
+template <int D, bool CAUSAL, bool TAIL = false, int CAST = 0>
 __global__ __launch_bounds__(256, 2) void attn_bwd_dq_kernel(const uint16_t* __restrict__ q, const uint16_t* __restrict__ k,
                                                              const uint16_t* __restrict__ v, const uint16_t* __restrict__ o,
                                                              const uint16_t* __restrict__ dout, const float* __restrict__ lse,
                                                              float* __restrict__ delta, uint16_t* __restrict__ dq, int S,
                                                              int H, int G, int64_t q_ts, int64_t k_ts, int64_t v_ts,
-                                                             int64_t o_ts, int64_t do_ts, int64_t dq_ts, float c, float scale) {
+                                                             int64_t o_ts, int64_t do_ts, int64_t dq_ts, float c, float scale,
+                                                             CastEpi ce) {
+  static_assert(CAST == 0 || (D == 128 && !TAIL), "the CAST epilogue: head_dim 128, full blocks");
   constexpr int TILE = ATT_KB * D * 2;
   constexpr int KT = D / 16, DB = D / 32;
   __shared__ __attribute__((aligned(16))) char lds[4 * TILE];
@@ -425,17 +469,29 @@
     dma_wait_all();
     __syncthreads();
   }
-  store_rows_from_accT<D, TAIL>(acc, scale, lds + w * (32 * D * 2), dq + ((int64_t)b * S + q_first) * dq_ts + (int64_t)head * D, dq_ts, lane,
-                                S - q_first);
-}
-
-template <int D, bool CAUSAL, bool TAIL = false>
+  if constexpr (CAST == 0) {
+    store_rows_from_accT<D, TAIL>(acc, scale, lds + w * (32 * D * 2), dq + ((int64_t)b * S + q_first) * dq_ts + (int64_t)head * D, dq_ts, lane,
+                                  S - q_first);
+  } else {
+    __shared__ float s_amax[4];
+    const float scale8 = *ce.scale;
+    float amax = 0.0f;
+    acc_to_slice<D>(acc, scale, lds + w * (32 * D * 2), lane);
+    __syncthreads();
+    cast_image<CAST, true>(lds, ce, scale8, amax, b * S + qb * ATT_QB, head * D, S, (int)gridDim.z * S, (H + 2 * G) * D, tid);
+    if (ce.amax != nullptr) publish_amax(amax, s_amax, ce.amax, tid);
+  }
+}
+
+template <int D, bool CAUSAL, bool TAIL = false, int CAST = 0>
 __global__ __launch_bounds__(256, D == 128 ? 1 : 2) void attn_bwd_dkdv_kernel(const uint16_t* __restrict__ q, const uint16_t* __restrict__ k,
                                                                const uint16_t* __restrict__ v, const uint16_t* __restrict__ dout,
                                                                const float* __restrict__ lse, const float* __restrict__ delta,
                                                                uint16_t* __restrict__ dk, uint16_t* __restrict__ dv, int S, int H,
                                                                int G, int B, int64_t q_ts, int64_t k_ts, int64_t v_ts,
-                                                               int64_t do_ts, int64_t dk_ts, int64_t dv_ts, float c, float scale) {
+                                                               int64_t do_ts, int64_t dk_ts, int64_t dv_ts, float c, float scale,
+                                                               CastEpi ce) {
+  static_assert(CAST == 0 || (D == 128 && !TAIL), "the CAST epilogue: head_dim 128, full blocks");
   constexpr int SL = 32 * D * 2;
   constexpr int KT = D / 16, DB = D / 32;
   constexpr int BUF = 2 * SL + 256;
@@ -563,9 +619,24 @@
     __syncthreads();
   }
   char* slice = lds + w * SL;
-  store_rows_from_accT<D, TAIL>(dka, scale, slice, dk + ((int64_t)b * S + key_first) * dk_ts + (int64_t)g * D, dk_ts, lane, S - key_first);
-  __builtin_amdgcn_wave_barrier();
-  store_rows_from_accT<D, TAIL>(dva, 1.0f, slice, dv + ((int64_t)b * S + key_first) * dv_ts + (int64_t)g * D, dv_ts, lane, S - key_first);
+  if constexpr (CAST == 0) {
+    store_rows_from_accT<D, TAIL>(dka, scale, slice, dk + ((int64_t)b * S + key_first) * dk_ts + (int64_t)g * D, dk_ts, lane, S - key_first);
+    __builtin_amdgcn_wave_barrier();
+    store_rows_from_accT<D, TAIL>(dva, 1.0f, slice, dv + ((int64_t)b * S + key_first) * dv_ts + (int64_t)g * D, dv_ts, lane, S - key_first);
+  } else {
+    __shared__ float s_amax[4];
+    const float scale8 = *ce.scale;
+    float amax = 0.0f;
+    const int row0 = b * S + kbi * 128, rows = B * S, W = (H + 2 * G) * D;
+    acc_to_slice<D>(dka, scale, slice, lane);
+    __syncthreads();
+    cast_image<CAST, true>(lds, ce, scale8, amax, row0, (H + g) * D, S, rows, W, tid);
+    __syncthreads();
+    acc_to_slice<D>(dva, 1.0f, slice, lane);
+    __syncthreads();
+    cast_image<CAST, false>(lds, ce, scale8, amax, row0, (H + G + g) * D, S, rows, W, tid);
+    if (ce.amax != nullptr) publish_amax(amax, s_amax, ce.amax, tid);
+  }
 }
 
 }
@@ -642,10 +713,10 @@
   do {                                                                                                                 \
     hipLaunchKernelGGL((mi::attn_bwd_dq_kernel<DD, CC, TT>), grid_q, block, 0, st, (const uint16_t*)q, (const uint16_t*)k, \
                        (const uint16_t*)v, (const uint16_t*)o, (const uint16_t*)dout, lse, delta, (uint16_t*)dq, S, H,  \
-                       G, q_ts, k_ts, v_ts, o_ts, do_ts, dq_ts, c, scale);                                               \
+                       G, q_ts, k_ts, v_ts, o_ts, do_ts, dq_ts, c, scale, mi::CastEpi{});                                \
     hipLaunchKernelGGL((mi::attn_bwd_dkdv_kernel<DD, CC, TT>), grid_kv, block, 0, st, (const uint16_t*)q,                \
                        (const uint16_t*)k, (const uint16_t*)v, (const uint16_t*)dout, lse, delta, (uint16_t*)dk,        \
-                       (uint16_t*)dv, S, H, G, B, q_ts, k_ts, v_ts, do_ts, dk_ts, dv_ts, c, scale);                      \
+                       (uint16_t*)dv, S, H, G, B, q_ts, k_ts, v_ts, do_ts, dk_ts, dv_ts, c, scale, mi::CastEpi{});       \
   } while (0)
 #define MI_ATTN_BWD(DD, CC)                                                                                            \
   do {                                                                                                                 \
@@ -661,3 +732,49 @@
   MI_CHECK_LAUNCH("mi_attn_bwd launch");
   return MI_OK;
 }
+
+extern "C" int mi_attn_bwd_rope_cast(const void* q, const void* k, const void* v, const void* o, const void* dout, const float* lse,
+                                     float* delta, const float* cos_tab, const float* sin_tab, const float* scale_fp8, float* amax,
+                                     void* y_fp8, void* yT_fp8, int B, int S, int H, int G, int D, int64_t q_ts, int64_t k_ts,
+                                     int64_t v_ts, int64_t o_ts, int64_t do_ts, float scale, int causal, int fmt, void* stream) {
+  MI_CHECK_ARG(q && k && v && o && dout && lse && delta && cos_tab && sin_tab && scale_fp8, "mi_attn_bwd_rope_cast: null pointer");
+  MI_CHECK_ARG(y_fp8 || yT_fp8, "mi_attn_bwd_rope_cast: at least one of y, yT must be non-null");
+  MI_CHECK_ARG(B >= 1 && H >= 1 && G >= 1 && H % G == 0, "mi_attn_bwd_rope_cast: bad B/H/G (%d, %d, %d)", B, H, G);
+  MI_CHECK_ARG(D == 128, "mi_attn_bwd_rope_cast: head_dim %d not supported (128)", D);
+  MI_CHECK_ARG(causal, "mi_attn_bwd_rope_cast: causal attention only");
+  MI_CHECK_ARG(((int64_t)B * S) % 8 == 0 && (int64_t)B * S < (1LL << 31), "mi_attn_bwd_rope_cast: bad shape (rows a multiple of 8)");
+  MI_CHECK_ARG(S >= 128 && S % mi::ATT_QB == 0, "mi_attn_bwd_rope_cast: seq %d must be a multiple of 128", S);
+  MI_CHECK_ARG((q_ts | k_ts | v_ts | o_ts | do_ts) % 8 == 0, "mi_attn_bwd_rope_cast: token strides must be multiples of 8");
+  MI_CHECK_ARG((int64_t)S * k_ts * 2 < (1LL << 31) && (int64_t)S * v_ts * 2 < (1LL << 31) && ((uintptr_t)k % 16) == 0 && ((uintptr_t)v % 16) == 0,
+               "mi_attn_bwd_rope_cast: one batch of K / V must span < 2 GiB and be 16-byte aligned (32-bit buffer offsets of the LDS DMA)");
+  MI_CHECK_ARG((((uintptr_t)q | (uintptr_t)o | (uintptr_t)dout | (uintptr_t)cos_tab | (uintptr_t)sin_tab) % 16) == 0 &&
+                   ((uintptr_t)y_fp8 % 8) == 0 && ((uintptr_t)yT_fp8 % 8) == 0, "mi_attn_bwd_rope_cast: misaligned pointer");
+  MI_CHECK_ARG(fmt == MI_FMT_E4M3 || fmt == MI_FMT_E5M2, "mi_attn_bwd_rope_cast: bad fmt %d", fmt);
+  MI_CHECK_ARG(H <= 65535 && B <= 65535, "mi_attn_bwd_rope_cast: grid too large");
+  const float c = scale * 1.4426950408889634f;
+  hipStream_t st = (hipStream_t)stream;
+  const int nblk = S / mi::ATT_QB;
+  dim3 grid_q(nblk, H, B), grid_kv((unsigned)((int64_t)nblk * G * B)), block(256);
+  const mi::CastEpi ce{cos_tab, sin_tab, scale_fp8, amax, (uint8_t*)y_fp8, (uint8_t*)yT_fp8};
+#define MI_ATTN_BWD_CAST(CC)                                                                                            \
+  do {                                                                                                                  \
+    hipLaunchKernelGGL((mi::attn_bwd_dq_kernel<128, true, false, CC>), grid_q, block, 0, st, (const uint16_t*)q,          \
+                       (const uint16_t*)k, (const uint16_t*)v, (const uint16_t*)o, (const uint16_t*)dout, lse, delta,    \
+                       (uint16_t*)nullptr, S, H, G, q_ts, k_ts, v_ts, o_ts, do_ts, (int64_t)0, c, scale, ce);            \
+    hipLaunchKernelGGL((mi::attn_bwd_dkdv_kernel<128, true, false, CC>), grid_kv, block, 0, st, (const uint16_t*)q,       \
+                       (const uint16_t*)k, (const uint16_t*)v, (const uint16_t*)dout, lse, delta, (uint16_t*)nullptr,    \
+                       (uint16_t*)nullptr, S, H, G, B, q_ts, k_ts, v_ts, do_ts, (int64_t)0, (int64_t)0, c, scale, ce);   \
+  } while (0)
+  const int cast = (y_fp8 ? 1 : 0) | (yT_fp8 ? 2 : 0) | (fmt == MI_FMT_E5M2 ? 4 : 0);
+  switch (cast) {
+    case 1: MI_ATTN_BWD_CAST(1); break;
+    case 2: MI_ATTN_BWD_CAST(2); break;
+    case 3: MI_ATTN_BWD_CAST(3); break;
+    case 5: MI_ATTN_BWD_CAST(5); break;
+    case 6: MI_ATTN_BWD_CAST(6); break;
+    default: MI_ATTN_BWD_CAST(7); break;
+  }
+#undef MI_ATTN_BWD_CAST
+  MI_CHECK_LAUNCH("mi_attn_bwd_rope_cast launch");
+  return MI_OK;
+}
diff --git a/llm_fp8_amd/csrc/mi_fused.hip b/llm_fp8_amd/csrc/mi_fused.hip
--- a/llm_fp8_amd/csrc/mi_fused.hip
+++ b/llm_fp8_amd/csrc/mi_fused.hip
@@ -1,4 +1,5 @@
 #include "mi_common.h"
+#include "mi_rope_cast_dev.h"
 
 namespace mi {
 
@@ -74,34 +75,8 @@
   const float scale = *scale_p;
   float amax = 0.0f;
   auto emit = [&](const float (&f)[8][8], int c0) {
-    u32 lo[8], hi[8];
-#pragma unroll
-    for (int i = 0; i < 8; ++i) {
-#pragma unroll
-      for (int j = 0; j < 8; ++j) amax = fmaxf(amax, (f[i][j] != f[i][j]) ? 0.0f : fabsf(f[i][j]));
-      lo[i] = cvt4_fp8<FMT>(f[i][0] * scale, f[i][1] * scale, f[i][2] * scale, f[i][3] * scale);
-      hi[i] = cvt4_fp8<FMT>(f[i][4] * scale, f[i][5] * scale, f[i][6] * scale, f[i][7] * scale);
-    }
-    if (WRITE_Y) {
-      uint8_t* dst = y + (int64_t)r0 * W + c0;
-#pragma unroll
-      for (int i = 0; i < 8; ++i) mi::st8<MI_NT_Y>(dst + (int64_t)i * W, lo[i], hi[i]);
-    }
-    if (WRITE_T) {
-      u32 a[4], b[4], c[4], d[4];
-      transpose4x4(lo[0], lo[1], lo[2], lo[3], a[0], a[1], a[2], a[3]);
-      transpose4x4(lo[4], lo[5], lo[6], lo[7], b[0], b[1], b[2], b[3]);
-      transpose4x4(hi[0], hi[1], hi[2], hi[3], c[0], c[1], c[2], c[3]);
-      transpose4x4(hi[4], hi[5], hi[6], hi[7], d[0], d[1], d[2], d[3]);
-      uint8_t* dst = yT + (int64_t)c0 * rows + r0;
-#pragma unroll
-      for (int j = 0; j < 4; ++j) {
-        mi::st8<MI_NT_YT>(dst + (int64_t)j * rows, a[j], b[j]);
-        mi::st8<MI_NT_YT>(dst + (int64_t)(j + 4) * rows, c[j], d[j]);
-      }
-    }
+    emit_fp8_block<FMT, WRITE_Y, WRITE_T>(f, scale, amax, y, yT, r0, c0, W, rows);
   };
-  auto bf16_round = [](float v) { return __uint_as_float(float_to_bf16_bits(v) << 16); };
   if (r0 < rows) {
     if (u < nq + nk) {
       const int hd = u;
@@ -113,22 +88,7 @@
         const v4i a = *reinterpret_cast<const v4i*>(src + i * rstride + lc);
         const v4i b = *reinterpret_cast<const v4i*>(src + i * rstride + half + lc);
         const int pos = (r0 + i) % seq;
-        float c[8], sn[8];
-        *reinterpret_cast<v4f*>(c) = *reinterpret_cast<const v4f*>(cosT + (int64_t)pos * half + lc);
-        *reinterpret_cast<v4f*>(c + 4) = *reinterpret_cast<const v4f*>(cosT + (int64_t)pos * half + lc + 4);
-        *reinterpret_cast<v4f*>(sn) = *reinterpret_cast<const v4f*>(sinT + (int64_t)pos * half + lc);
-        *reinterpret_cast<v4f*>(sn + 4) = *reinterpret_cast<const v4f*>(sinT + (int64_t)pos * half + lc + 4);
-#pragma unroll
-        for (int j = 0; j < 4; ++j) {
-          const u32 wa = (u32)a[j], wb = (u32)b[j];
-          const float x1l = __uint_as_float(wa << 16), x1h = __uint_as_float(wa & 0xFFFF0000u);
-          const float x2l = __uint_as_float(wb << 16), x2h = __uint_as_float(wb & 0xFFFF0000u);
-          const float cl = c[2 * j], ch = c[2 * j + 1], sl = -1.0f * sn[2 * j], sh = -1.0f * sn[2 * j + 1];
-          f1[i][2 * j] = bf16_round(x1l * cl - x2l * sl);
-          f1[i][2 * j + 1] = bf16_round(x1h * ch - x2h * sh);
-          f2[i][2 * j] = bf16_round(x2l * cl + x1l * sl);
-          f2[i][2 * j + 1] = bf16_round(x2h * ch + x1h * sh);
-        }
+        rope_bwd_row8<true, true>(a, b, cosT + (int64_t)pos * half + lc, sinT + (int64_t)pos * half + lc, f1[i], f2[i]);
       }
       emit(f1, hd * D + lc);
       emit(f2, hd * D + half + lc);
@@ -137,25 +97,12 @@
       float f[8][8];
 #pragma unroll
       for (int i = 0; i < 8; ++i) {
-        const v4i a = *reinterpret_cast<const v4i*>(dv + (int64_t)(r0 + i) * (nk * D) + tc * 64 + lc);
-#pragma unroll
-        for (int j = 0; j < 4; ++j) {
-          f[i][2 * j] = __uint_as_float((u32)a[j] << 16);
-          f[i][2 * j + 1] = __uint_as_float((u32)a[j] & 0xFFFF0000u);
-        }
+        bf16_row8(*reinterpret_cast<const v4i*>(dv + (int64_t)(r0 + i) * (nk * D) + tc * 64 + lc), f[i]);
       }
       emit(f, (nq + nk) * D + tc * 64 + lc);
     }
   }
-  if (amax_out != nullptr) {
-    amax = wave_max(amax);
-    if (lane == 0) s_amax[wave] = amax;
-    __syncthreads();
-    if (tid == 0) {
-      const float m = fmaxf(fmaxf(s_amax[0], s_amax[1]), fmaxf(s_amax[2], s_amax[3]));
-      if (m > 0.0f && m > __builtin_nontemporal_load(amax_out)) atomicMax(reinterpret_cast<unsigned int*>(amax_out), __float_as_uint(m));
-    }
-  }
+  if (amax_out != nullptr) publish_amax(amax, s_amax, amax_out, tid);
 }
 
 __device__ __forceinline__ float sigmoidf_(float g) { return 1.0f / (1.0f + __expf(-g)); }
diff --git a/llm_fp8_amd/csrc/mi_rope_cast_dev.h b/llm_fp8_amd/csrc/mi_rope_cast_dev.h
--- /dev/null
+++ b/llm_fp8_amd/csrc/mi_rope_cast_dev.h
@@ -0,0 +1,82 @@
+#pragma once
+#include "mi_common.h"
+
+namespace mi {
+
+__device__ __forceinline__ float bf16_round(float v) { return __uint_as_float(float_to_bf16_bits(v) << 16); }
+
+template <bool LO, bool HI>
+__device__ __forceinline__ void rope_bwd_row8(const v4i a, const v4i b, const float* __restrict__ cp, const float* __restrict__ sp,
+                                              float* f1, float* f2) {
+  float c[8], sn[8];
+  *reinterpret_cast<v4f*>(c) = *reinterpret_cast<const v4f*>(cp);
+  *reinterpret_cast<v4f*>(c + 4) = *reinterpret_cast<const v4f*>(cp + 4);
+  *reinterpret_cast<v4f*>(sn) = *reinterpret_cast<const v4f*>(sp);
+  *reinterpret_cast<v4f*>(sn + 4) = *reinterpret_cast<const v4f*>(sp + 4);
+#pragma unroll
+  for (int j = 0; j < 4; ++j) {
+    const u32 wa = (u32)a[j], wb = (u32)b[j];
+    const float x1l = __uint_as_float(wa << 16), x1h = __uint_as_float(wa & 0xFFFF0000u);
+    const float x2l = __uint_as_float(wb << 16), x2h = __uint_as_float(wb & 0xFFFF0000u);
+    const float cl = c[2 * j], ch = c[2 * j + 1], sl = -1.0f * sn[2 * j], sh = -1.0f * sn[2 * j + 1];
+    if (LO) {
+      f1[2 * j] = bf16_round(x1l * cl - x2l * sl);
+      f1[2 * j + 1] = bf16_round(x1h * ch - x2h * sh);
+    }
+    if (HI) {
+      f2[2 * j] = bf16_round(x2l * cl + x1l * sl);
+      f2[2 * j + 1] = bf16_round(x2h * ch + x1h * sh);
+    }
+  }
+}
+
+__device__ __forceinline__ void bf16_row8(const v4i a, float* f) {
+#pragma unroll
+  for (int j = 0; j < 4; ++j) {
+    f[2 * j] = __uint_as_float((u32)a[j] << 16);
+    f[2 * j + 1] = __uint_as_float((u32)a[j] & 0xFFFF0000u);
+  }
+}
+
+template <int FMT, bool WRITE_Y, bool WRITE_T>
+__device__ __forceinline__ void emit_fp8_block(const float (&f)[8][8], float scale, float& amax, uint8_t* __restrict__ y,
+                                               uint8_t* __restrict__ yT, int r0, int c0, int W, int rows) {
+  u32 lo[8], hi[8];
+#pragma unroll
+  for (int i = 0; i < 8; ++i) {
+#pragma unroll
+    for (int j = 0; j < 8; ++j) amax = fmaxf(amax, (f[i][j] != f[i][j]) ? 0.0f : fabsf(f[i][j]));
+    lo[i] = cvt4_fp8<FMT>(f[i][0] * scale, f[i][1] * scale, f[i][2] * scale, f[i][3] * scale);
+    hi[i] = cvt4_fp8<FMT>(f[i][4] * scale, f[i][5] * scale, f[i][6] * scale, f[i][7] * scale);
+  }
+  if (WRITE_Y) {
+    uint8_t* dst = y + (int64_t)r0 * W + c0;
+#pragma unroll
+    for (int i = 0; i < 8; ++i) mi::st8<MI_NT_Y>(dst + (int64_t)i * W, lo[i], hi[i]);
+  }
+  if (WRITE_T) {
+    u32 a[4], b[4], c[4], d[4];
+    transpose4x4(lo[0], lo[1], lo[2], lo[3], a[0], a[1], a[2], a[3]);
+    transpose4x4(lo[4], lo[5], lo[6], lo[7], b[0], b[1], b[2], b[3]);
+    transpose4x4(hi[0], hi[1], hi[2], hi[3], c[0], c[1], c[2], c[3]);
+    transpose4x4(hi[4], hi[5], hi[6], hi[7], d[0], d[1], d[2], d[3]);
+    uint8_t* dst = yT + (int64_t)c0 * rows + r0;
+#pragma unroll
+    for (int j = 0; j < 4; ++j) {
+      mi::st8<MI_NT_YT>(dst + (int64_t)j * rows, a[j], b[j]);
+      mi::st8<MI_NT_YT>(dst + (int64_t)(j + 4) * rows, c[j], d[j]);
+    }
+  }
+}
+
+__device__ __forceinline__ void publish_amax(float amax, float* s_amax, float* amax_out, int tid) {
+  amax = wave_max(amax);
+  if ((tid & 63) == 0) s_amax[tid >> 6] = amax;
+  __syncthreads();
+  if (tid == 0) {
+    const float m = fmaxf(fmaxf(s_amax[0], s_amax[1]), fmaxf(s_amax[2], s_amax[3]));
+    if (m > 0.0f && m > __builtin_nontemporal_load(amax_out)) atomicMax(reinterpret_cast<unsigned int*>(amax_out), __float_as_uint(m));
+  }
+}
+
+}
diff --git a/llm_fp8_amd/pytorch/attention.py b/llm_fp8_amd/pytorch/attention.py
--- a/llm_fp8_amd/pytorch/attention.py
+++ b/llm_fp8_amd/pytorch/attention.py
@@ -79,6 +79,7 @@
         ctx.meta = (B, S, n_q, n_kv, d)
         ctx.handoff = handoff
         ctx.act_ref = weakref.ref(qkv) if handoff is not None else None
+        ctx.read_at_fwd = handoff is not None and handoff_readers(qkv)
         return q.view(B, S, n_q, d), k.view(B, S, n_kv, d), v.view(B, S, n_kv, d)
 
     @staticmethod
@@ -87,7 +88,7 @@
         B, S, n_q, n_kv, d = ctx.meta
         T = B * S
         h = ctx.handoff
-        if h is not None and h.offered() and handoff_readers(ctx.act_ref()):
+        if h is not None and h.offered() and (ctx.read_at_fwd or handoff_readers(ctx.act_ref())):
             h = None
         if h is not None and h.offered() and d == 128 and T % (32 if h.mx else 8) == 0:
             args = (dq.reshape(T, n_q * d), dk.reshape(T, n_kv * d), dv.reshape(T, n_kv * d), cos, sin, n_q, n_kv, d, S)
@@ -115,11 +116,57 @@
     @staticmethod
     def backward(ctx, do):
         q, k, v, o, lse = ctx.saved_tensors
-        ok = (do.stride(3) == 1 and do.stride(2) == do.shape[3] and do.stride(0) == do.shape[1] * do.stride(1)
-              and do.stride(1) % 8 == 0 and do.data_ptr() % 16 == 0)
-        do = do if ok else do.clone(memory_format=torch.contiguous_format)
-        dq, dk, dv = ops.attn_bwd(do, q, k, v, o, lse, ctx.scale, ctx.causal)
+        dq, dk, dv = ops.attn_bwd(_bshd_do(do), q, k, v, o, lse, ctx.scale, ctx.causal)
         return dq, dk, dv, None, None
+
+
+def _bshd_do(do):
+    ok = (do.stride(3) == 1 and do.stride(2) == do.shape[3] and do.stride(0) == do.shape[1] * do.stride(1)
+          and do.stride(1) % 8 == 0 and do.data_ptr() % 16 == 0)
+    return do if ok else do.clone(memory_format=torch.contiguous_format)
+
+
+class _RoPEAttnFn(torch.autograd.Function):
+
+    @staticmethod
+    def forward(ctx, qkv, cos, sin, n_q, n_kv, d, handoff):
+        B, S, W = qkv.shape
+        x = qkv.reshape(B * S, W)
+        x = x if x.is_contiguous() else x.contiguous()
+        q, k, v = ops.rope_qkv_forward(x, cos, sin, n_q, n_kv, d, S)
+        q, k, v = q.view(B, S, n_q, d), k.view(B, S, n_kv, d), v.view(B, S, n_kv, d)
+        scale = d ** -0.5
+        o, lse = ops.attn_fwd(q, k, v, scale, True)
+        ctx.save_for_backward(cos, sin, q, k, v, o, lse)
+        ctx.meta = (B, S, n_q, n_kv, d, scale)
+        ctx.handoff = handoff
+        ctx.act_ref = weakref.ref(qkv)
+        ctx.read_at_fwd = handoff_readers(qkv)
+        return o
+
+    @staticmethod
+    def backward(ctx, do):
+        cos, sin, q, k, v, o, lse = ctx.saved_tensors
+        B, S, n_q, n_kv, d, scale = ctx.meta
+        T = B * S
+        do = _bshd_do(do)
+        h = ctx.handoff
+        if h.offered() and (ctx.read_at_fwd or handoff_readers(ctx.act_ref())):
+            h = None
+        if h is not None and h.offered() and not h.mx:
+            fp8 = ops.rope_qkv_backward_cast(None, None, None, cos, sin, n_q, n_kv, d, S, h.scale, h.amax, h.fmt, want_y=h.want_y,
+                                             want_t=h.want_t, attn=(do, q, k, v, o, lse, scale))
+            g = torch.empty((B, S, (n_q + 2 * n_kv) * d), dtype=torch.bfloat16, device=do.device)
+            h.put(fp8, g)
+            return g, None, None, None, None, None, None
+        dq, dk, dv = ops.attn_bwd(do, q, k, v, o, lse, scale, True)
+        args = (dq.reshape(T, n_q * d), dk.reshape(T, n_kv * d), dv.reshape(T, n_kv * d), cos, sin, n_q, n_kv, d, S)
+        if h is not None and h.offered() and T % 32 == 0:
+            fp8 = ops.mxfp8_rope_bwd_quantize(*args, h.fmt, rowwise=h.want_y, colwise=h.want_t)
+            g = torch.empty((B, S, (n_q + 2 * n_kv) * d), dtype=torch.bfloat16, device=do.device)
+            h.put(fp8, g)
+            return g, None, None, None, None, None, None
+        return ops.rope_qkv_backward(*args).view(B, S, -1), None, None, None, None, None, None
 
 
 def _flash_ok(q, k, v, causal: bool, dropout: float) -> bool:
@@ -208,11 +255,21 @@
         qkv = self.layernorm_qkv(hidden_states) if self.input_layernorm else self.qkv(hidden_states)
         return self._attend(qkv, attention_mask, rotary_pos_emb)
 
+    def _one_node_ok(self, qkv: torch.Tensor) -> bool:
+        core = self.core_attention
+        B, S, W = qkv.shape
+        return (os.environ.get("LLM_FP8_AMD_NO_ATTN_BWD_CAST") != "1" and self.d == 128 and S % 128 == 0 and self.h % self.g == 0
+                and core.attn_mask_type in ("causal", "padding_causal") and core.qkv_format == "bshd"
+                and (core.p == 0.0 or not core.training) and S * self.h * self.d * 2 < 2 ** 31)
+
     def _attend(self, qkv: torch.Tensor, attention_mask, rotary_pos_emb, handoff=None) -> torch.Tensor:
         if (rotary_pos_emb is not None and not isinstance(rotary_pos_emb, (tuple, list)) and qkv.is_cuda
                 and qkv.dtype == torch.bfloat16 and self.qkv_format == "bshd" and self.d % 16 == 0
                 and rotary_pos_emb.shape[-1] == self.d):
             cos, sin = _cos_sin_tables(rotary_pos_emb, qkv.shape[1])
+            if handoff is not None and self._one_node_ok(qkv):
+                o = _RoPEAttnFn.apply(qkv, cos, sin, self.h, self.g, self.d, handoff)
+                return self.proj(o.reshape(*o.shape[:2], self.h * self.d))
             q, k, v = _RoPESplitFn.apply(qkv, cos, sin, self.h, self.g, self.d, handoff)
             return self.proj(self.core_attention(q, k, v, attention_mask))
         if handoff is not None:
diff --git a/llm_fp8_amd/pytorch/ops.py b/llm_fp8_amd/pytorch/ops.py
--- a/llm_fp8_amd/pytorch/ops.py
+++ b/llm_fp8_amd/pytorch/ops.py
@@ -500,7 +500,10 @@
 
 def rope_qkv_backward_cast(dq: torch.Tensor, dk: torch.Tensor, dv: torch.Tensor, cos: torch.Tensor, sin: torch.Tensor,
                            n_q: int, n_kv: int, head_dim: int, seq: int, scale: torch.Tensor, amax: Optional[torch.Tensor],
-                           fmt: int, want_y: bool = True, want_t: bool = True):
+                           fmt: int, want_y: bool = True, want_t: bool = True, attn=None):
+    if attn is not None:
+        assert dq is None and dk is None and dv is None and head_dim == 128 and attn[1].shape[1] == seq
+        return attn_bwd_rope_cast(*attn, cos, sin, scale, amax, fmt, want_y=want_y, want_t=want_t)
     _dev(dq, dk, dv, cos, sin, scale, amax)
     dq, dk, dv = (t.contiguous() for t in (dq, dk, dv))
     T = dq.shape[0]
@@ -749,3 +752,32 @@
             rc = _lib.load().mi_attn_bwd(*args)
     _lib.check(rc, "mi_attn_bwd")
     return dq, dk, dv
+
+
+def attn_bwd_rope_cast(do: torch.Tensor, q: torch.Tensor, k: torch.Tensor, v: torch.Tensor, o: torch.Tensor, lse: torch.Tensor,
+                       sm_scale: float, cos: torch.Tensor, sin: torch.Tensor, scale: torch.Tensor, amax: Optional[torch.Tensor],
+                       fmt: int, want_y: bool = True, want_t: bool = True):
+    _dev(do, q, k, v, o, lse, cos, sin, scale, amax)
+    B, S, H, D = q.shape
+    G = k.shape[2]
+    for t in (q, k, v, o, do):
+        _bshd_ok(t, D)
+    assert o.shape == do.shape == q.shape and lse.shape == (B, H, S) and lse.dtype == torch.float32 and lse.is_contiguous()
+    assert cos.dtype == sin.dtype == torch.float32 and cos.is_contiguous() and sin.is_contiguous() and cos.shape[0] >= S
+    T, W = B * S, (H + 2 * G) * D
+    y = torch.empty((T, W), dtype=torch.uint8, device=q.device) if want_y else None
+    yT = torch.empty((W, T), dtype=torch.uint8, device=q.device) if want_t else None
+    delta = torch.empty((B, H, S), dtype=torch.float32, device=q.device)
+    args = (q.data_ptr(), k.data_ptr(), v.data_ptr(), o.data_ptr(), do.data_ptr(), lse.data_ptr(), delta.data_ptr(),
+            cos.data_ptr(), sin.data_ptr(), scale.data_ptr(), _ptr(amax), _ptr(y), _ptr(yT), B, S, H, G, D, q.stride(1),
+            k.stride(1), v.stride(1), o.stride(1), do.stride(1), float(sm_scale), 1, fmt, _stream())
+    t = KernelTimer.active
+    flops = 14.0 * B * H * S * S * D * 0.5
+    if t is None:
+        rc = _lib.load().mi_attn_bwd_rope_cast(*args)
+    else:
+        with t.span("attn_bwd", f"{B}x{S}x{H}x{D} cast", flops,
+                    2.0 * (3 * q.numel() + 2 * k.numel()) + float(T * W * ((y is not None) + (yT is not None)))):
+            rc = _lib.load().mi_attn_bwd_rope_cast(*args)
+    _lib.check(rc, "mi_attn_bwd_rope_cast")
+    return y, yT
```

After: 89590 tokens/s (median of 6 runs). No clear change (+0.6%).
